# JuliaMeshless/WhatsThePoint.jl

Hardware: AMD Instinct MI355X
Metric: Mpoints/sec per repel iter (k=21 KNN+force) (higher is better)
Workload: dtype f32

## Files before the change

whatsthepoint.jl_amd/csrc/wtp_api.hip:

```cpp
#include <cmath>
#include <cstdlib>
#include <cstring>
#include <type_traits>

#include "wtp_internal.hpp"

namespace wtp {

static thread_local std::string g_create_err;

int fail(wtp_ctx* ctx, int code, const std::string& msg) {
    if (ctx)
        ctx->err = msg;
    else
        g_create_err = msg;
    return code;
}

int ensure(wtp_ctx* ctx, DevBuf& b, size_t bytes) {
    if (bytes == 0) bytes = 16;
    if (b.cap >= bytes) return WTP_OK;
    if (b.p) {
        hipFree(b.p);
        b.p = nullptr;
        b.cap = 0;
    }
    size_t want = bytes + bytes / 16 + 256;
    hipError_t e = hipMalloc(&b.p, want);
    if (e != hipSuccess) {
        (void)hipGetLastError();
        e = hipMalloc(&b.p, bytes);
        want = bytes;
    }
    if (e != hipSuccess) {
        (void)hipGetLastError();
        b.p = nullptr;
        return fail(ctx, WTP_ERR_OOM, "hipMalloc of " + std::to_string(bytes) + " bytes failed");
    }
    b.cap = want;
    return WTP_OK;
}

int launch_occupancy_of(wtp_ctx* ctx, const void* fn, int threads, size_t smem) {
    const auto key = std::make_pair(fn, smem);
    auto it = ctx->launch_cache.find(key);
    if (it != ctx->launch_cache.end()) return it->second;
    (void)hipFuncSetAttribute(fn, hipFuncAttributeMaxDynamicSharedMemorySize, (int)smem);
    int occ = 0;
    hipError_t e = hipOccupancyMaxActiveBlocksPerMultiprocessor(&occ, fn, threads, smem);
    if (e != hipSuccess || occ < 1) occ = 1;
    ctx->launch_cache[key] = occ;
    return occ;
}

int ensure_pinned(wtp_ctx* ctx, size_t bytes) {
    if (ctx->host_pinned_cap >= bytes) return WTP_OK;
    if (ctx->host_pinned) hipHostFree(ctx->host_pinned);
    ctx->host_pinned = nullptr;
    ctx->host_pinned_cap = 0;
    WTP_HIP(ctx, hipHostMalloc(&ctx->host_pinned, bytes, hipHostMallocDefault));
    ctx->host_pinned_cap = bytes;
    return WTP_OK;
}

static int take_event(wtp_ctx* ctx) {
    if (ctx->ev_used == (int)ctx->ev_pool.size()) {
        hipEvent_t e;
        if (hipEventCreate(&e) != hipSuccess) return -1;
        ctx->ev_pool.push_back(e);
    }
    return ctx->ev_used++;
}

int span_begin(wtp_ctx* ctx, int kind) {
    if (!ctx->timing) return -1;
    if (ctx->spans.size() > 8192) spans_collect(ctx);
    int a = ctx->ev_last_end;
    if (a < 0) {
        a = take_event(ctx);
        if (a < 0) return -1;
        hipEventRecord(ctx->ev_pool[a], ctx->stream);
    }
    const int b = take_event(ctx);
    if (b < 0) return -1;
    ctx->spans.push_back({a, b, kind});
    return (int)ctx->spans.size() - 1;
}

void span_end(wtp_ctx* ctx, int span) {
    if (span < 0) return;
    hipEventRecord(ctx->ev_pool[ctx->spans[span].b], ctx->stream);
    ctx->ev_last_end = ctx->spans[span].b;
}

void spans_collect(wtp_ctx* ctx) {
    ctx->ev_last_end = -1;
    if (ctx->spans.empty()) return;
    hipStreamSynchronize(ctx->stream);
    for (auto& s : ctx->spans) {
        float ms = 0.f;
        if (hipEventElapsedTime(&ms, ctx->ev_pool[s.a], ctx->ev_pool[s.b]) == hipSuccess) {
            if (s.kind == 0) ctx->t_hash += ms;
            else if (s.kind == 1) ctx->t_sweep += ms;
            else ctx->t_other += ms;
        }
    }
    ctx->spans.clear();
    ctx->ev_used = 0;
}

static int sync(wtp_ctx* ctx) {
    ctx->ev_last_end = -1;
    ctx->n_syncs += 1;
    WTP_HIP(ctx, hipStreamSynchronize(ctx->stream));
    return WTP_OK;
}

static size_t tsize(int dtype) { return dtype == WTP_F64 ? 8 : 4; }
static size_t pt_size(int dtype) { return by_dtype(dtype, [](auto t) { return sizeof(Pt<decltype(t)>); }); }

int need_session(wtp_ctx* ctx, const char* entry) {
    if (!ctx) return WTP_ERR_ARG;
    if (!ctx->relax.active) return fail(ctx, WTP_ERR_STATE, std::string(entry) + " before wtp_relax_init");
    return WTP_OK;
}

static double host_max(const void* v, int64_t n, int dtype) {
    double m = 0;
    if (dtype == WTP_F64) {
        const double* p = (const double*)v;
        for (int64_t i = 0; i < n; ++i) m = p[i] > m ? p[i] : m;
    } else {
        const float* p = (const float*)v;
        for (int64_t i = 0; i < n; ++i) m = p[i] > m ? p[i] : m;
    }
    return m;
}

static int check_cloud(wtp_ctx* ctx, const void* xyz, int64_t n, int dim, int dtype) {
    if (!ctx) return WTP_ERR_ARG;
    if (!xyz) return fail(ctx, WTP_ERR_ARG, "xyz is NULL");
    if (n < 1) return fail(ctx, WTP_ERR_ARG, "n must be >= 1");
    if (n > 2000000000LL) return fail(ctx, WTP_ERR_ARG, "n exceeds the int32 index space");
    if (dim != 2 && dim != 3) return fail(ctx, WTP_ERR_ARG, "dim must be 2 or 3");
    if (dtype != WTP_F32 && dtype != WTP_F64) return fail(ctx, WTP_ERR_ARG, "dtype must be WTP_F32 or WTP_F64");
    return WTP_OK;
}

static double hash_target_rho(const wtp_ctx* ctx, int dim, int k, double rho_direct) {
    if (rho_direct > 0) return rho_direct < 1.0 ? 1.0 : rho_direct;
    const double r = (dim == 3 ? 0.381 : 0.436) * (double)(k > 0 ? k : 21) * (ctx->rho / 8.0);
    return r < 1.0 ? 1.0 : r;
}

template <typename T>
static int find_robust_box(wtp_ctx* ctx, const Pt<T>* in, int64_t n, int dim, const Grid<T>& hg) {
    int rc;
    const size_t hist_bytes = sizeof(unsigned int) * 3 * 1024;
    if ((rc = ensure(ctx, ctx->box_dev, 64 + hist_bytes))) return rc;
    if ((rc = ensure_pinned(ctx, 64 + hist_bytes))) return rc;
    double box[6];
    for (int a = 0; a < 3; ++a) {
        box[a] = (double)hg.org[a];
        box[3 + a] = (double)hg.org[a] + (double)hg.n[a] * (double)hg.c;
    }
    const uint64_t tail = (uint64_t)(n / 2000) + 1;
    for (int round = 0; round < 4; ++round) {
        memcpy(ctx->host_pinned, box, sizeof(box));
        WTP_HIP(ctx, hipMemcpyAsync(ctx->box_dev.p, ctx->host_pinned, sizeof(box), hipMemcpyHostToDevice, ctx->stream));
        unsigned int* d_hist = (unsigned int*)((char*)ctx->box_dev.p + 64);
        if ((rc = launch_axis_hist<T>(ctx, in, n, dim, (const double*)ctx->box_dev.p, d_hist))) return rc;
        WTP_HIP(ctx, hipMemcpyAsync((char*)ctx->host_pinned + 64, d_hist, hist_bytes, hipMemcpyDeviceToHost, ctx->stream));
        if ((rc = sync(ctx))) return rc;
        const unsigned int* h = (const unsigned int*)((const char*)ctx->host_pinned + 64);
        bool shrunk = false;
        for (int a = 0; a < dim; ++a) {
            const double w = (box[3 + a] - box[a]) / 1024.0;
            if (!(w > 0)) continue;
            uint64_t run = 0;
            int b_lo = 0, b_hi = 1023;
            for (int b = 0; b < 1024; ++b) {
                run += h[a * 1024 + b];
                if (run >= tail) { b_lo = b; break; }
            }
            run = 0;
            for (int b = 1023; b >= 0; --b) {
                run += h[a * 1024 + b];
                if (run >= tail) { b_hi = b; break; }
            }
            if (b_hi < b_lo) b_hi = b_lo;
            const double nlo = box[a] + w * b_lo, nhi = box[a] + w * (b_hi + 1);
            if ((nhi - nlo) < 0.5 * (box[3 + a] - box[a])) shrunk = true;
            box[a] = nlo;
            box[3 + a] = nhi;
        }
        if (!shrunk) break;
    }
    memcpy(ctx->host_pinned, box, sizeof(box));
    WTP_HIP(ctx, hipMemcpyAsync(ctx->box_dev.p, ctx->host_pinned, sizeof(box), hipMemcpyHostToDevice, ctx->stream));
    return sync(ctx);
}

template <typename T>
static int build_hash_tuned(wtp_ctx* ctx, GridTune& t, HashBuild<T> b, Grid<T>* hg_out, double* rho_eff_out) {
    const double target = hash_target_rho(ctx, b.dim, b.k, b.rho_direct);
    double scale = 1.0;
    double prev_c = -1;
    int rc;
    if ((rc = ensure(ctx, ctx->occ, 64))) return rc;
    if ((rc = ensure_pinned(ctx, 16384))) return rc;
    t.clipped = false;
    b.keep_grid = false;
    for (int round = 0; round < 3; ++round) {
        b.cell_scale = scale;
        b.box = t.clipped ? (const double*)ctx->box_dev.p : nullptr;
        if ((rc = build_hash<T>(ctx, b))) return rc;
        if ((rc = launch_occupancy<T>(ctx, (const Grid<T>*)ctx->grid.p, (unsigned long long*)ctx->occ.p))) return rc;
        char* hp = (char*)ctx->host_pinned;
        WTP_HIP(ctx, hipMemcpyAsync(hp, ctx->occ.p, 24, hipMemcpyDeviceToHost, ctx->stream));
        WTP_HIP(ctx, hipMemcpyAsync(hp + 64, ctx->grid.p, sizeof(Grid<T>), hipMemcpyDeviceToHost, ctx->stream));
        if ((rc = sync(ctx))) return rc;
        const unsigned long long* o = (const unsigned long long*)hp;
        const double rho_eff = o[1] ? (double)o[0] / (double)o[1] : 1.0;
        Grid<T> hg;
        memcpy(&hg, hp + 64, sizeof(hg));
        *rho_eff_out = rho_eff;
        *hg_out = hg;
        const double excess = (rho_eff - 1.0) / target;
        const bool capped = hg.n[0] >= kMaxAxisCells || hg.n[1] >= kMaxAxisCells || hg.n[2] >= kMaxAxisCells ||
                            (double)hg.ncells > 6.0 * (double)b.n;
        if (excess > 4.0 && capped && !t.clipped) {
            if ((rc = find_robust_box<T>(ctx, b.in, b.n, b.dim, hg))) return rc;
            t.clipped = true;
            scale = 1.0;
            prev_c = -1;
            round = -1;
            continue;
        }
        if (!(excess > 1.6) || round == 2) break;
        if (prev_c > 0 && !((double)hg.c < prev_c * 0.999)) break;
        prev_c = (double)hg.c;
        double f = std::cbrt(1.15 / excess);
        if (f < 0.3) f = 0.3;
        scale *= f;
        if (scale < 0.02) scale = 0.02;
    }
    t.scale = scale;
    t.rho = b.rho_direct;
    return WTP_OK;
}

static double ksel_brick_cost(int cols, double rho_cell, int* bx_out = nullptr) {
    int bx = ksel_max_bx();
    double best = 1e300;
    for (int nbx = 1; nbx <= cols; ++nbx) {
        const int b = (cols + nbx - 1) / nbx;
        if (b > ksel_max_bx()) continue;
        const double q = 4.0 * rho_cell * b;
        const double p2 = 0.5 * std::erfc((256.0 - q) / std::sqrt(2.0 * (q > 1 ? q : 1)));
        const double cost = (1.0 + p2 + (q > 512.0 ? 100.0 : 0.0)) / q;
        if (cost < best) {
            best = cost;
            bx = b;
        }
        if (b < 8) break;
    }
// ... 168 lines not shown
    span_end(ctx, sp);
    sp = span_begin(ctx, 1);
    init_search(b, ctx, sorted32, sorted32, n, kc, 1);
    b.idx_out = (int32_t*)ctx->cand_idx.p;
    b.dist_out = (float*)ctx->cand_dist.p;
    if (ksel) {
        b.ksel_bx = t.bx;
        b.brick_hcap = t.hcap;
        b.cap_count = (float)ksel_cap_count(kc);
    }
    return launch_topology<float>(ctx, b);
}

static int knn_dev_f64(wtp_ctx* ctx, const double* d_xyz, int64_t n, int dim, int k, int include_self, int32_t* d_idx,
                       double* d_dist, bool* done) {
    *done = false;
    const int kq = include_self ? k : k + 1;
    int kc = kq + 2;
    if ((int64_t)kc > n) kc = (int)n;
    if (ctx->force_generic || kc > 31) return WTP_OK;
    int rc;
    if ((rc = ensure(ctx, ctx->pts[0], sizeof(double4) * (size_t)n))) return rc;
    if ((rc = ensure(ctx, ctx->pts[1], sizeof(double4) * (size_t)n))) return rc;
    if ((rc = ensure(ctx, ctx->fb_list, sizeof(int32_t) * (size_t)n))) return rc;
    if ((rc = ensure(ctx, ctx->fb_count, 64))) return rc;
    ctx->counters_clean = false;
    if ((rc = ensure(ctx, ctx->fb2_list, sizeof(int32_t) * (size_t)n))) return rc;
    if ((rc = ensure(ctx, ctx->fb2_count, 64))) return rc;
    double4* raw64 = (double4*)ctx->pts[0].p;
    int sp = span_begin(ctx, 0);
    if ((rc = load_points<double>(ctx, d_xyz, raw64, n, dim))) return rc;
    const bool slots = kc == 24;
    double4* slot64 = (double4*)ctx->pts[1].p;
    SearchArgs<float> a{};
    a.fb_list = (int32_t*)ctx->fb_list.p;
    a.fb_count = (int32_t*)ctx->fb_count.p;
    a.fb2_list = (int32_t*)ctx->fb2_list.p;
    a.fb2_count = (int32_t*)ctx->fb2_count.p;
    const double* org4 = nullptr;
    rc = f64_candidates(ctx, raw64, n, dim, kc, ctx->knn64_tune, a, sp, &org4, [&](float4* sorted32) {
        return slots ? launch_relabel_slots(ctx, raw64, sorted32, slot64, nullptr, n) : WTP_OK;
    });
    if (rc) return rc;
    ctx->knn_tune.valid = false;
    if (slots)
        rc = launch_refine_f64_slots(ctx, slot64, a.idx_out, a.dist_out, n, kc, k, include_self, org4, d_idx, d_dist,
                                     (int32_t*)ctx->fb_list.p, (int32_t*)ctx->fb_count.p);
    else
        rc = launch_refine_f64(ctx, raw64, a.idx_out, a.dist_out, n, kc, k, include_self, org4, d_idx, d_dist,
                               (int32_t*)ctx->fb_list.p, (int32_t*)ctx->fb_count.p);
    span_end(ctx, sp);
    if (rc) return rc;
    ctx->n_sweep_launches += 1;
    ctx->relax.have_tree = false;
    ctx->rad_valid = false;
    if ((rc = ensure_pinned(ctx, 64))) return rc;
    WTP_HIP(ctx, hipMemcpyAsync(ctx->host_pinned, ctx->fb_count.p, sizeof(int32_t), hipMemcpyDeviceToHost, ctx->stream));
    if ((rc = sync(ctx))) return rc;
    const int32_t n_fail = *(const int32_t*)ctx->host_pinned;
    if (n_fail > 0) {
        double4* sorted64 = (double4*)ctx->pts[1].p;
        HashBuild<double> hb(raw64, sorted64, n, dim, kq);
        hb.canonical = false;
        if ((rc = build_hash<double>(ctx, hb))) return rc;
        SearchArgs<double> b{};
        init_search(b, ctx, sorted64, raw64, n, k, include_self);
        b.idx_out = d_idx;
        b.dist_out = d_dist;
        b.fb_list = (int32_t*)ctx->fb_list.p;
        b.fb_count = (int32_t*)ctx->fb_count.p;
        b.fb2_list = (int32_t*)ctx->fb2_list.p;
        b.fb2_count = (int32_t*)ctx->fb2_count.p;
        if ((rc = launch_generic_topology<double>(ctx, b, false))) return rc;
    }
    *done = true;
    return WTP_OK;
}

static int check_idle(wtp_ctx* ctx) {
    if (ctx->relax.active)
        return fail(ctx, WTP_ERR_STATE,
                    "context holds a relax session (its buffers are live): call wtp_relax_end or use another context");
    return WTP_OK;
}

static int check_k(wtp_ctx* ctx, int64_t n, int k, int include_self) {
    if (k < 1) return fail(ctx, WTP_ERR_ARG, "k must be >= 1");
    if ((int64_t)k > n - (include_self ? 0 : 1))
        return fail(ctx, WTP_ERR_ARG, "k exceeds the number of available neighbours (k+1 > n)");
    if (k > kGenericKMax) return fail(ctx, WTP_ERR_ARG, "k > 128 is not supported");
    return WTP_OK;
}

}

using namespace wtp;

#define WTP_API extern "C"

WTP_API const char* wtp_version(void) { return "wtp-mi355x 0.1.0 (gfx950)"; }

WTP_API const char* wtp_last_error(const wtp_ctx* ctx) { return ctx ? ctx->err.c_str() : g_create_err.c_str(); }

WTP_API int wtp_create(const int* device_ordinals, int n_dev, wtp_ctx** out) {
    if (!out) return fail(nullptr, WTP_ERR_ARG, "out is NULL");
    *out = nullptr;
    if (n_dev != 1)
        return fail(nullptr, WTP_ERR_ARG, "one context drives one GPU: create one context per process/GPU");
    int count = 0;
    if (hipGetDeviceCount(&count) != hipSuccess || count < 1) {
        (void)hipGetLastError();
        return fail(nullptr, WTP_ERR_NO_DEVICE, "no HIP device visible (libwtp has no CPU path)");
    }
    int dev = device_ordinals ? device_ordinals[0] : 0;
    if (dev < 0 || dev >= count) return fail(nullptr, WTP_ERR_ARG, "device ordinal out of range");
    hipDeviceProp_t prop;
    if (hipGetDeviceProperties(&prop, dev) != hipSuccess)
        return fail(nullptr, WTP_ERR_HIP, "hipGetDeviceProperties failed");
    if (std::string(prop.gcnArchName).rfind("gfx950", 0) != 0)
        return fail(nullptr, WTP_ERR_NO_DEVICE,
                    std::string("device is ") + prop.gcnArchName + ", libwtp is built for gfx950 only");
    if (hipSetDevice(dev) != hipSuccess) return fail(nullptr, WTP_ERR_HIP, "hipSetDevice failed");
    wtp_ctx* ctx = new wtp_ctx();
    ctx->device = dev;
    ctx->sm_count = prop.multiProcessorCount > 0 ? prop.multiProcessorCount : 256;
    if (hipStreamCreateWithFlags(&ctx->own_stream, hipStreamNonBlocking) != hipSuccess) {
        delete ctx;
        return fail(nullptr, WTP_ERR_HIP, "hipStreamCreate failed");
    }
    ctx->stream = ctx->own_stream;
    if (const char* e = getenv("WTP_RHO")) ctx->rho = atof(e) > 0 ? atof(e) : ctx->rho;
    if (const char* e = getenv("WTP_FORCE_GENERIC")) ctx->force_generic = atoi(e);
    if (const char* e = getenv("WTP_FULL_SELECT")) ctx->full_select = atoi(e);
    if (const char* e = getenv("WTP_KSEL")) ctx->ksel = atoi(e);
    if (const char* e = getenv("WTP_BALL64")) ctx->ball64 = atoi(e);
    if (const char* e = getenv("WTP_F64_KSEL")) ctx->f64_ksel = atoi(e);
    if (const char* e = getenv("WTP_RADIUS_DENSE")) ctx->radius_dense = atoi(e);
    if (const char* e = getenv("WTP_BLOCK_OVERLAP")) ctx->block_overlap = atoi(e);
    ctx->debug = getenv("WTP_DEBUG") != nullptr;
    ctx->debug_kd = getenv("WTP_DEBUG_KD") != nullptr;
    if (const char* e = getenv("WTP_TIMING")) {
        ctx->timing = atoi(e) != 0;
        ctx->timing_forced = true;
    }
    *out = ctx;
    return WTP_OK;
}

WTP_API int wtp_destroy(wtp_ctx* ctx) {
    if (ctx) block_destroy(ctx);
    if (ctx) block_topo_destroy(ctx);
    if (!ctx) return WTP_OK;
    hipSetDevice(ctx->device);
    hipStreamSynchronize(ctx->stream);
    wtp_comm_finalize(ctx);
    if (ctx->host_pinned) hipHostFree(ctx->host_pinned);
    for (auto e : ctx->ev_pool) hipEventDestroy(e);
    if (ctx->ev_comm_a) hipEventDestroy(ctx->ev_comm_a);
    if (ctx->ev_comm_b) hipEventDestroy(ctx->ev_comm_b);
    if (ctx->comm_stream) hipStreamDestroy(ctx->comm_stream);
    hipStreamDestroy(ctx->own_stream);
    delete ctx;
    return WTP_OK;
}

static int knn_on_device(wtp_ctx* ctx, const void* d_xyz, int64_t n, int dim, int dtype, int k, int include_self,
                         int32_t* d_idx, void* d_dist) {
    bool done = false;
    int rc = dtype == WTP_F64 ? knn_dev_f64(ctx, (const double*)d_xyz, n, dim, k, include_self, d_idx, (double*)d_dist, &done)
                              : WTP_OK;
    if (rc || done) return rc;
    return by_dtype(dtype, [&](auto t) {
        using T = decltype(t);
        return knn_dev_t<T>(ctx, (const T*)d_xyz, n, dim, k, include_self, d_idx, (T*)d_dist);
    });
}

static int knn_rows_on_device(wtp_ctx* ctx, const void* xyz, int64_t n, int dim, int dtype, int k, int include_self,
                              bool want_dist) {
    const size_t ts = tsize(dtype);
    int rc;
    if ((rc = ensure(ctx, ctx->raw_in, ts * (size_t)n * dim))) return rc;
    if ((rc = ensure(ctx, ctx->idx_out, sizeof(int32_t) * (size_t)n * k))) return rc;
    if (want_dist && (rc = ensure(ctx, ctx->dist_out, ts * (size_t)n * k))) return rc;
    WTP_HIP(ctx, hipMemcpyAsync(ctx->raw_in.p, xyz, ts * (size_t)n * dim, hipMemcpyHostToDevice, ctx->stream));
    return knn_on_device(ctx, ctx->raw_in.p, n, dim, dtype, k, include_self, (int32_t*)ctx->idx_out.p,
                         want_dist ? ctx->dist_out.p : nullptr);
}

WTP_API int wtp_knn_dev(wtp_ctx* ctx, const void* d_xyz, int64_t n, int dim, int dtype, int k, int include_self,
                int32_t* d_idx_out, void* d_dist_out) {
    int rc = check_cloud(ctx, d_xyz, n, dim, dtype);
    if (rc) return rc;
    if ((rc = check_k(ctx, n, k, include_self))) return rc;
    if ((rc = check_idle(ctx))) return rc;
    if (!d_idx_out) return fail(ctx, WTP_ERR_ARG, "idx_out is NULL");
    WTP_HIP(ctx, hipSetDevice(ctx->device));
    if ((rc = knn_on_device(ctx, d_xyz, n, dim, dtype, k, include_self, d_idx_out, d_dist_out))) return rc;
    return sync(ctx);
}

WTP_API int wtp_knn(wtp_ctx* ctx, const void* xyz, int64_t n, int dim, int dtype, int k, int include_self,
            int32_t* idx_out, void* dist_out) {
    int rc = check_cloud(ctx, xyz, n, dim, dtype);
    if (rc) return rc;
    if ((rc = check_k(ctx, n, k, include_self))) return rc;
    if ((rc = check_idle(ctx))) return rc;
    if (!idx_out) return fail(ctx, WTP_ERR_ARG, "idx_out is NULL");
    WTP_HIP(ctx, hipSetDevice(ctx->device));
    const size_t ts = tsize(dtype);
    if ((rc = knn_rows_on_device(ctx, xyz, n, dim, dtype, k, include_self, dist_out != nullptr))) return rc;
    WTP_HIP(ctx, hipMemcpyAsync(idx_out, ctx->idx_out.p, sizeof(int32_t) * (size_t)n * k, hipMemcpyDeviceToHost,
                                ctx->stream));
    if (dist_out)
        WTP_HIP(ctx, hipMemcpyAsync(dist_out, ctx->dist_out.p, ts * (size_t)n * k, hipMemcpyDeviceToHost, ctx->stream));
    return sync(ctx);
}

WTP_API int wtp_pca_normals(wtp_ctx* ctx, const void* xyz, int64_t n, int dim, int dtype, int k, void* normals_out) {
    int rc = check_cloud(ctx, xyz, n, dim, dtype);
    if (rc) return rc;
    if (k < 2) return fail(ctx, WTP_ERR_ARG, "k must be >= 2 (a covariance needs two points)");
    if ((rc = check_k(ctx, n, k, 1))) return rc;
    if ((rc = check_idle(ctx))) return rc;
    if (!normals_out) return fail(ctx, WTP_ERR_ARG, "normals_out is NULL");
    WTP_HIP(ctx, hipSetDevice(ctx->device));
    const size_t ts = tsize(dtype);
    if ((rc = knn_rows_on_device(ctx, xyz, n, dim, dtype, k, 1, false))) return rc;
    if ((rc = ensure(ctx, ctx->scratch, ts * (size_t)n * dim))) return rc;
    int sp = span_begin(ctx, 2);
    rc = by_dtype(dtype, [&](auto t) {
        using T = decltype(t);
        return launch_pca_normals<T>(ctx, (const T*)ctx->raw_in.p, n, dim, (const int32_t*)ctx->idx_out.p, k, (T*)ctx->scratch.p);
    });
    span_end(ctx, sp);
    if (rc) return rc;
    WTP_HIP(ctx, hipMemcpyAsync(normals_out, ctx->scratch.p, ts * (size_t)n * dim, hipMemcpyDeviceToHost, ctx->stream));
    return sync(ctx);
}

WTP_API int wtp_gradient_limit(wtp_ctx* ctx, const void* centers, int64_t n, int dim, int dtype, int k, const void* h0,
                               double g, double tol, int max_sweeps, void* h_out, int* sweeps_out) {
    int rc = check_cloud(ctx, centers, n, dim, dtype);
    if (rc) return rc;
    if ((rc = check_k(ctx, n, k, 1))) return rc;
    if ((rc = check_idle(ctx))) return rc;
    if (!h0 || !h_out) return fail(ctx, WTP_ERR_ARG, "NULL array");
    if (max_sweeps < 0) return fail(ctx, WTP_ERR_ARG, "max_sweeps must be >= 0");
    WTP_HIP(ctx, hipSetDevice(ctx->device));
    const size_t ts = tsize(dtype);
    if ((rc = knn_rows_on_device(ctx, centers, n, dim, dtype, k, 1, true))) return rc;
    const size_t o1 = (ts * (size_t)n + 255) / 256 * 256;
    if ((rc = ensure(ctx, ctx->scratch, 2 * o1 + 64))) return rc;
    char* b = (char*)ctx->scratch.p;
    unsigned long long* st = (unsigned long long*)(b + 2 * o1);
    WTP_HIP(ctx, hipMemcpyAsync(b, h0, ts * (size_t)n, hipMemcpyHostToDevice, ctx->stream));
    WTP_HIP(ctx, hipMemsetAsync(st, 0, 64, ctx->stream));
    if ((rc = ensure_pinned(ctx, 64))) return rc;
    unsigned long long* hst = (unsigned long long*)ctx->host_pinned;
    hst[0] = hst[1] = 0;
    int sp = span_begin(ctx, 2);
    for (int first = 0; first < max_sweeps && !hst[0];) {
        const int batch = max_sweeps - first < 16 ? max_sweeps - first : 16;
        rc = by_dtype(dtype, [&](auto t) {
            using T = decltype(t);
            return launch_minplus_batch<T>(ctx, (const int32_t*)ctx->idx_out.p, (const T*)ctx->dist_out.p, n, k, g, tol, (T*)b,
                                           (T*)(b + o1), first, batch, st);
        });
        if (rc) return rc;
        WTP_HIP(ctx, hipMemcpyAsync(hst, st, 16, hipMemcpyDeviceToHost, ctx->stream));
        if ((rc = sync(ctx))) return rc;
        first += batch;
    }
    span_end(ctx, sp);
    const int applied = (int)hst[1];
    if (sweeps_out) *sweeps_out = applied;
    WTP_HIP(ctx, hipMemcpyAsync(h_out, b + ((applied & 1) ? o1 : 0), ts * (size_t)n, hipMemcpyDeviceToHost, ctx->stream));
    return sync(ctx);
}

template <typename T> static int radius_count_t(wtp_ctx* ctx, int64_t n, int dim, double r, int32_t* d_counts) {
    int rc;
    if ((rc = ensure(ctx, ctx->pts[0], sizeof(Pt<T>) * (size_t)n))) return rc;
    if ((rc = ensure(ctx, ctx->pts[1], sizeof(Pt<T>) * (size_t)n))) return rc;
    Pt<T>* raw = (Pt<T>*)ctx->pts[0].p;
    Pt<T>* sorted = (Pt<T>*)ctx->pts[1].p;
    int sp = span_begin(ctx, 0);
    if ((rc = load_points<T>(ctx, (const T*)ctx->raw_in.p, raw, n, dim))) return rc;
    HashBuild<T> b(raw, sorted, n, dim, 0);
    b.radius = r > 0 ? r : 1e-300;
    b.canonical = false;
    if ((rc = build_hash<T>(ctx, b))) return rc;
    span_end(ctx, sp);
    SearchArgs<T> a{};
    init_search(a, ctx, sorted, sorted, n, 0, 0);
    if ((rc = ensure(ctx, ctx->fb_list, sizeof(int32_t) * (size_t)n))) return rc;
    if ((rc = ensure(ctx, ctx->fb_count, 64))) return rc;
    ctx->counters_clean = false;
    a.fb_list = (int32_t*)ctx->fb_list.p;
    a.fb_count = (int32_t*)ctx->fb_count.p;
    if ((rc = ensure(ctx, ctx->rad_done, (size_t)n + 64))) return rc;
    WTP_HIP(ctx, hipMemsetAsync(ctx->rad_done.p, 0, (size_t)n, ctx->stream));
    a.rad_done = (uint8_t*)ctx->rad_done.p;
    if (sizeof(T) == 4 && !ctx->force_generic) {
        if ((rc = ensure(ctx, ctx->rad_tmp, sizeof(int32_t) * 32 * (size_t)n))) return rc;
        a.rad_tmp = (int32_t*)ctx->rad_tmp.p;
    }
    const int64_t arena_cap = (int64_t)kRadArenaPerPoint * n;
    if ((rc = ensure(ctx, ctx->rad_arena, sizeof(int32_t) * (size_t)arena_cap))) return rc;
    if ((rc = ensure(ctx, ctx->rad_arena_off, sizeof(int64_t) * (size_t)(n + 2)))) return rc;
    a.rad_arena = (int32_t*)ctx->rad_arena.p;
    a.rad_arena_off = (int64_t*)ctx->rad_arena_off.p;
// ... 340 lines not shown
    if ((rc = ensure(ctx, ctx->occ, 513 * sizeof(unsigned int)))) return rc;
    if ((rc = ensure_pinned(ctx, 16384))) return rc;
    const double cells = (double)hg.n[0] * hg.n[1] * hg.n[2];
    double rho_est = cells > 0 ? (double)r.n / cells : 1.0;
    if (rho_eff - 1.0 > rho_est) rho_est = rho_eff - 1.0;
    if (rho_est < 0.25) rho_est = 0.25;
    const int bx_max = hg.n[0] < cs2_max_bx() ? (hg.n[0] < 1 ? 1 : hg.n[0]) : cs2_max_bx();
    auto clampbx = [&](double v) {
        int b = (int)(v + 0.5);
        return b < 2 ? (bx_max < 2 ? bx_max : 2) : (b > bx_max ? bx_max : b);
    };
    r.cs2_rho = rho_est;
    int bx = clampbx(220.0 / (4.0 * rho_est));
    int q97 = 0, h999 = 0;
    for (int it = 0; it < 4; ++it) {
        if ((rc = launch_cs2_census(ctx, bx, (unsigned int*)ctx->occ.p))) return rc;
        WTP_HIP(ctx, hipMemcpyAsync(ctx->host_pinned, ctx->occ.p, 513 * sizeof(unsigned int), hipMemcpyDeviceToHost,
                                    ctx->stream));
        if ((rc = sync(ctx))) return rc;
        const unsigned int* h = (const unsigned int*)ctx->host_pinned;
        const double nb = (double)h[512];
        auto quant = [&](int base, double frac, int width) {
            double run = 0;
            for (int b = 0; b < 256; ++b) {
                run += h[base + b];
                if (run >= frac * nb) return (b + 1) * width;
            }
            return 256 * width;
        };
        q97 = nb > 0 ? quant(0, 0.97, 2) : 0;
        h999 = nb > 0 ? quant(256, 0.999, 8) : 0;
        if (nb <= 0) break;
        double f = 1.0;
        if (q97 > 248 || q97 < 216) f = 236.0 / (double)q97;
        if (h999 * f > 1060.0) f = 1060.0 / (double)h999;
        const int nbx = clampbx(bx * f);
        if (nbx == bx || it == 3) break;
        bx = nbx;
    }
    if (hg.n[0] > bx && q97 > 0) {
        int best = 0;
        for (int parts = hg.n[0] / bx > 1 ? hg.n[0] / bx : 1; parts <= (hg.n[0] + bx - 1) / bx; ++parts) {
            const int bxc = (hg.n[0] + parts - 1) / parts;
            if (bxc > bx_max) continue;
            const double grow = (double)bxc / (double)bx;
            if (q97 * grow <= 254.0 && h999 * grow <= 1100.0) {
                best = bxc;
                h999 = (int)(h999 * grow) + 1;
                break;
            }
        }
        if (!best) {
            const int parts = (hg.n[0] + bx - 1) / bx;
            best = (hg.n[0] + parts - 1) / parts;
        }
        bx = best;
    }
    int hc = (int)(h999 * 1.05) + 48;
    hc = (hc + 63) / 64 * 64;
    r.brick_hcap = hc < 256 ? 256 : (hc > 1920 ? 1920 : hc);
    r.cs2_bx = bx;
    if (ctx->debug)
        fprintf(stderr, "[wtp] cs2 geometry: BX=%d hcap=%d (q97=%d h999=%d rho_est=%.3f grid %dx%dx%d c=%g)\n", bx,
                r.brick_hcap, q97, h999, rho_est, hg.n[0], hg.n[1], hg.n[2], (double)hg.c);
    return WTP_OK;
}

static void swap_float_copy_grid(wtp_ctx* ctx) {
    std::swap(ctx->grid, ctx->grid_b);
    std::swap(ctx->cell_start, ctx->cell_start_b);
    std::swap(ctx->box_dev, ctx->box_b);
}

static int relax_f64_ksel_sweep(wtp_ctx* ctx, SearchArgs<double>& a, int* sp) {
    RelaxState& r = ctx->relax;
    const int64_t n = r.n;
    const int kc = 24;
    int rc;
    if ((rc = ensure(ctx, ctx->f64k_s64, sizeof(double4) * (size_t)n))) return rc;
    if ((rc = ensure(ctx, ctx->f64k_slot, sizeof(int32_t) * (size_t)n))) return rc;
    if ((rc = ensure(ctx, ctx->f64k_lists, sizeof(int32_t) * 2 * (size_t)n))) return rc;
    if ((rc = ensure(ctx, ctx->f64k_cnt, 64))) return rc;
    const double4* snap = (const double4*)a.snap;
    SearchArgs<float> b{};
    b.fb_list = (int32_t*)ctx->f64k_lists.p;
    b.fb_count = (int32_t*)ctx->f64k_cnt.p;
    b.fb2_list = (int32_t*)ctx->f64k_lists.p + n;
    b.fb2_count = (int32_t*)ctx->f64k_cnt.p + 4;
    b.stop = ctx->stop_dev;
    b.diag = a.diag;
    *sp = span_begin(ctx, 0);
    WTP_HIP(ctx, hipMemsetAsync(ctx->f64k_cnt.p, 0, 64, ctx->stream));
    b.counters_cleared = 1;
    swap_float_copy_grid(ctx);
    const double* org4 = nullptr;
    rc = f64_candidates(ctx, snap, n, 3, kc, r.f64k_tune, b, *sp, &org4, [&](float4* sorted32) {
        return launch_relabel_slots(ctx, snap, sorted32, (double4*)ctx->f64k_s64.p, (int32_t*)ctx->f64k_slot.p, n);
    });
    swap_float_copy_grid(ctx);
    if (rc) return rc;
    return launch_refine_sweep_f64(ctx, a, (const double4*)ctx->f64k_s64.p, (const int32_t*)ctx->f64k_slot.p,
                                   (const int32_t*)ctx->cand_idx.p, (const float*)ctx->cand_dist.p, org4);
}

static bool grid_reusable(const RelaxState& r, int64_t n_fixed_next, bool head_swapped) {
    const bool head_ok = !head_swapped || (r.shard_grid_reuse && r.grid_fixed > 0 &&
                                           std::llabs((long long)(n_fixed_next - r.grid_fixed)) * 10 <= (long long)r.grid_fixed + 640);
    return r.grid_age < kGridReuseMax && !r.moved_by_hand && head_ok && !r.tune.clipped;
}

static bool head_remeasures(const RelaxState& r, int64_t n_fixed_new) {
    const int64_t n_new = r.n - r.n_fixed + n_fixed_new;
    return r.cs2_bx > 0 && std::llabs((long long)(n_fixed_new - r.tuned_fixed)) * 20 > (long long)n_new;
}

template <typename T> static SweepRoute sweep_route(const wtp_ctx* ctx, const RelaxState& r) {
    if (ctx->force_generic) return SweepRoute::Exact;
    const bool clipped = r.force.kind == WTP_FORCE_CLIPPED_SPACING;
    if (clipped && r.k >= 2 && r.k < 32 && !ctx->full_select && !r.cs_disabled) {
        if (sizeof(T) == 8) return ctx->ball64 ? SweepRoute::Cs64 : SweepRoute::Cs64Wave;
        return r.dim == 3 ? SweepRoute::Cs2 : SweepRoute::Cs;
    }
    if (sizeof(T) == 8) {
        const bool f64k = r.dim == 3 && ctx->ksel && ctx->f64_ksel && !clipped && r.k >= 2 && r.k <= 22 && r.n >= 4096;
        return f64k ? SweepRoute::F64Ksel : SweepRoute::Exact;
    }
    if (r.k >= 32) return SweepRoute::Exact;
    const bool ksel = r.dim == 3 && ctx->ksel && r.k >= 2 && r.k <= ksel_kmax() && r.n >= 4096;
    return ksel ? SweepRoute::Ksel : SweepRoute::Select;
}

static bool route_cs(SweepRoute s) {
    return s == SweepRoute::Cs || s == SweepRoute::Cs2 || s == SweepRoute::Cs64 || s == SweepRoute::Cs64Wave;
}
static bool route_ball(SweepRoute s) { return s == SweepRoute::Cs || s == SweepRoute::Cs2 || s == SweepRoute::Cs64; }

struct RouteGrid { double rho, min_cell; };
static RouteGrid route_grid(const wtp_ctx* ctx, const RelaxState& r) {
    if (r.route == SweepRoute::Ksel) return {r.tune.valid && r.tune.bx > 0 ? r.tune.rho : ksel_rho_for(r.k), 0.0};
    if (!route_cs(r.route)) return {0.0, 0.0};
    const bool cs2 = r.route == SweepRoute::Cs2;
    const double cell_f = (cs2 && r.spacing_kind == WTP_SPACING_CONSTANT) ? 1.01 : 1.1;
    return {cs2 ? kRhoCs2 : 3.5 * (ctx->rho / 9.0),
            cell_f * r.force.u0 * (r.spacing_typ < r.spacing_max ? r.spacing_typ : r.spacing_max)};
}

static SweepRoute step_route(const RelaxState& r, bool fresh) {
    if (!fresh) return route_ball(r.route) ? SweepRoute::Ball : SweepRoute::Exact;
    const bool measured = r.route == SweepRoute::Ksel ? r.tune.bx > 0 : !route_cs(r.route) || r.brick_hcap > 0;
    if (measured) return r.route;
    return r.route == SweepRoute::Cs64 || r.route == SweepRoute::Cs64Wave ? SweepRoute::Exact : SweepRoute::Select;
}

static int ball_pass(wtp_ctx* ctx, SearchArgs<float>& a) { return launch_cs_ball(ctx, a, a.ball_list, a.ball_count); }
static int ball_pass(wtp_ctx* ctx, SearchArgs<double>& a) { return launch_cs_ball64(ctx, a, a.ball_list, a.ball_count); }

template <typename T> static int launch_sweep(wtp_ctx* ctx, SearchArgs<T>& a, SweepRoute route, bool ball) {
    constexpr bool f32 = sizeof(T) == 4;
    ctx->n_sweep_launches += 1;
    int rc = WTP_OK, sp = -1;
    switch (route) {
    case SweepRoute::Exact:
    case SweepRoute::Ball:
        sp = span_begin(ctx, 1);
        if (route == SweepRoute::Ball) {
            rc = launch_cs_all_slots(ctx, a.fb_list, a.n, a.fb_count);
            if (!rc) rc = ball_pass(ctx, a);
        }
        if (!rc) rc = launch_generic_sweep<T>(ctx, a, route == SweepRoute::Exact);
        span_end(ctx, sp);
        return rc;
    case SweepRoute::F64Ksel:
        if constexpr (!f32) rc = relax_f64_ksel_sweep(ctx, a, &sp);
        break;
    case SweepRoute::Ksel:
        sp = span_begin(ctx, 1);
        if constexpr (f32) rc = launch_ksel_sweep(ctx, a);
        a.fb_r0 = 3;
        break;
    case SweepRoute::Select:
    case SweepRoute::Cs:
    case SweepRoute::Cs2:
        sp = span_begin(ctx, 1);
        if constexpr (f32) {
            if (route == SweepRoute::Cs2 && ball) {
                const int dead_cap = (int)(ctx->cell_start.cap / sizeof(int32_t) / 4 + 4096);
                rc = ensure(ctx, ctx->brick_dead, (size_t)dead_cap);
                if (!rc) rc = launch_cs2_dead(ctx, a, (uint8_t*)ctx->brick_dead.p, dead_cap);
                a.brick_dead = (const uint8_t*)ctx->brick_dead.p;
                a.brick_dead_cap = dead_cap;
            }
            if (!rc) rc = route == SweepRoute::Cs2 ? launch_cs2(ctx, a) : launch_brick_sweep(ctx, a, route == SweepRoute::Cs);
        }
        break;
    case SweepRoute::Cs64:
    case SweepRoute::Cs64Wave:
        sp = span_begin(ctx, 1);
        if constexpr (!f32) {
            rc = launch_brick_cs<double>(ctx, a);
            if (!rc && ball) rc = ball_pass(ctx, a);
        }
        break;
    }
    span_end(ctx, sp);
    if (rc) return rc;
    sp = span_begin(ctx, 2);
    if constexpr (f32) {
        if (route == SweepRoute::Cs2) rc = launch_cs2_followup(ctx, a);
        if (!rc && ball) rc = ball_pass(ctx, a);
    }
    if (!rc) rc = launch_generic_sweep<T>(ctx, a, false);
    span_end(ctx, sp);
    return rc;
}

template <typename T>
static HashBuild<T> relax_request(const wtp_ctx* ctx, const RelaxState& r, const Pt<T>* in, Pt<T>* out, int64_t n, int k,
                                  const HashView& view, bool keep_grid) {
    const RouteGrid g = route_grid(ctx, r);
    HashBuild<T> b(in, out, n, r.dim, k);
    b.rho_direct = g.rho;
    b.min_cell = g.min_cell;
    b.cell_scale = r.tune.scale;
    b.view = view;
    b.keep_grid = keep_grid;
    b.canonical = !r.tune.valid || r.route != SweepRoute::F64Ksel;
    b.box = r.tune.clipped ? (const double*)ctx->box_dev.p : nullptr;
    return b;
}

template <typename T> static int relax_rebuild(wtp_ctx* ctx) {
    RelaxState& r = ctx->relax;
    int rc;
    const int t = pick_free(r, r.bufP, -1);
    if ((rc = ensure(ctx, ctx->pts[t], sizeof(Pt<T>) * (size_t)(r.n + r.shard_extra)))) return rc;
    int sp = span_begin(ctx, 0);
    r.route = sweep_route<T>(ctx, r);
    if (r.spacing_typ <= 0) {
        r.spacing_typ = r.spacing_const;
        if (r.spacing_kind != WTP_SPACING_CONSTANT) {
            if ((rc = ensure(ctx, ctx->occ, 64))) return rc;
            if ((rc = ensure_pinned(ctx, 1024))) return rc;
            if ((rc = launch_sum<T>(ctx, (const T*)ctx->spacing_pp.p, r.n, (double*)ctx->occ.p))) return rc;
            WTP_HIP(ctx, hipMemcpyAsync(ctx->host_pinned, ctx->occ.p, sizeof(double), hipMemcpyDeviceToHost, ctx->stream));
            if ((rc = sync(ctx))) return rc;
            r.spacing_typ = ((const double*)ctx->host_pinned)[0] / (double)r.n;
            if (!(r.spacing_typ > 0)) r.spacing_typ = r.spacing_max;
        }
    }
    const Pt<T>* in = pts_of<T>(ctx, r.bufP);
    Pt<T>* out = pts_of<T>(ctx, t);
    if (!r.tune.valid) {
        double rho_eff = 0;
        Grid<T> hg;
        HashBuild<T> b = relax_request<T>(ctx, r, in, out, r.n, r.k, r.pending, false);
        if ((rc = build_hash_tuned<T>(ctx, r.tune, b, &hg, &rho_eff))) return rc;
        if (route_cs(r.route) && rho_eff > (r.route == SweepRoute::Cs2 ? 5.0 : 4.0 * b.rho_direct) && 2 * r.n_fixed < r.n) {
            r.cs_disabled = true;
            r.route = sweep_route<T>(ctx, r);
            b = relax_request<T>(ctx, r, in, out, r.n, r.k, r.pending, false);
            if ((rc = build_hash_tuned<T>(ctx, r.tune, b, &hg, &rho_eff))) return rc;
        }
        r.cs2_bx = 0;
        if (r.route == SweepRoute::Cs2) {
            Grid<float> hgf;
            memcpy(&hgf, &hg, sizeof(hgf));
            if ((rc = cs2_tune(ctx, r, hgf, rho_eff))) return rc;
        } else if (route_cs(r.route)) {
            int hc = (int)(HCELLS * rho_eff * 1.15) + 128;
            hc = (hc + 63) / 64 * 64;
            r.brick_hcap = hc < 640 ? 640 : (hc > 2560 ? 2560 : hc);
        }
        if (r.route == SweepRoute::Ksel && (rc = ksel_tune<T>(ctx, r.tune, b, hg, rho_eff))) return rc;
        r.tune.valid = true;
        r.tuned_fixed = r.n_fixed;
        r.grid_fixed = r.n_fixed;
        r.grid_age = 0;
    } else {
        const bool reuse = grid_reusable(r, r.n_fixed, r.pending.active);
        r.grid_age = reuse ? r.grid_age + 1 : 0;
        if (!reuse) r.grid_fixed = r.n_fixed;
        rc = build_hash<T>(ctx, relax_request<T>(ctx, r, in, out, r.n, r.k, r.pending, reuse));
    }
    span_end(ctx, sp);
    if (rc) return rc;
    r.pending.active = false;
    r.bufS = t;
    r.bufP = t;
    r.have_tree = true;
    r.sweeps_since_rebuild = 0;
    r.moved_by_hand = false;
    return WTP_OK;
}

template <typename T> static int relax_step_t(wtp_ctx* ctx, int rebuild, wtp_step_stats* d_slot) {
    RelaxState& r = ctx->relax;
    int rc;
    if (!r.have_tree || r.pending.active) rebuild = 1;
    if (rebuild && (rc = relax_rebuild<T>(ctx))) return rc;
    if (spacing_on_device(r.spacing_kind)) {
        int sps = span_begin(ctx, 2);
        rc = launch_spacing_session<T>(ctx, (const Pt<T>*)ctx->pts[r.bufP].p, r.n, r.n_fixed, ctx->kd_nodes.p, ctx->kd_m,
                                       r.spacing_kind, r.sp_p0, r.sp_p1, r.sp_p2, (T*)ctx->spacing_pp.p,
                                       (int32_t*)ctx->sp_hint.p - r.aux_off, r.have_tree ? (const int32_t*)ctx->cell_start.p : nullptr,
                                       ctx->grid.p, (Pt<T>*)ctx->sp_cert.p - r.aux_off);
        span_end(ctx, sps);
        if (rc) return rc;
    }
    const bool fresh = (r.bufS == r.bufP);
    const int o = pick_free(r, r.bufS, r.bufP);
    if ((rc = ensure(ctx, ctx->pts[o], sizeof(Pt<T>) * (size_t)(r.n + r.shard_extra)))) return rc;
    SearchArgs<T> a{};
    init_search(a, ctx, (const Pt<T>*)ctx->pts[r.bufS].p, (const Pt<T>*)ctx->pts[r.bufP].p, r.n, r.k, 1);
    a.out = (Pt<T>*)ctx->pts[o].p;
    a.forces = (T*)ctx->forces.p;
    a.nn_dist = (T*)ctx->nn_dist.p;
    a.nn_id = (int32_t*)ctx->nn_id.p;
    a.spacing_pp = r.spacing_kind != WTP_SPACING_CONSTANT ? (const T*)ctx->spacing_pp.p : nullptr;
    a.spacing_const = (T)r.spacing_const;
    a.alpha_lo = (T)r.alpha_lo;
    a.alpha_max = (T)r.alpha_max;
    a.beta = (T)r.force.beta;
    a.u0 = (T)r.force.u0;
    a.gamma = (T)r.force.gamma;
    a.force_kind = r.force.kind;
    a.n_fixed = (int32_t)r.n_fixed;
    a.partials = (Partial*)ctx->partials.p;
    a.n_partials = total_partials();
    a.fb_list = (int32_t*)ctx->fb_list.p;
    a.fb_count = (int32_t*)ctx->fb_count.p;
    a.fb2_list = (int32_t*)ctx->fb2_list.p;
    a.fb2_count = (int32_t*)ctx->fb_count.p + 4;
    a.stop = ctx->stop_dev;
    a.nn_count = (int32_t*)ctx->fb_count.p + 2;
    const SweepRoute route = step_route(r, fresh);
    const bool ball = route_ball(r.route) && (!fresh || r.spacing_kind != WTP_SPACING_CONSTANT);
    if (ball || route == SweepRoute::Cs2) {
        if ((rc = ensure(ctx, ctx->nn_list, sizeof(int32_t) * (size_t)r.n))) return rc;
        if (sizeof(T) == 4) a.nn_list = (int32_t*)ctx->nn_list.p;
        if (ball) {
            a.ball_list = (int32_t*)ctx->nn_list.p;
            a.ball_count = (int32_t*)ctx->fb_count.p + 6;
        }
    }
    if ((rc = ensure(ctx, ctx->diag, 128))) return rc;
    a.diag = (unsigned long long*)ctx->diag.p;
    a.brick_hcap = route_cs(r.route) ? r.brick_hcap : (r.route == SweepRoute::Ksel ? r.tune.hcap : 0);
    a.cs2_bx = route_cs(r.route) ? r.cs2_bx : 0;
    a.cs2_chunked = (r.spacing_kind != WTP_SPACING_CONSTANT || r.cs2_rho > 1.6) ? 1 : 0;
    a.ksel_bx = r.route == SweepRoute::Ksel ? r.tune.bx : 0;
    if (r.route == SweepRoute::Ksel) a.cap_count = (float)ksel_cap_count(r.k);
    if (route == SweepRoute::Select || route == SweepRoute::Cs || route == SweepRoute::Cs2) {
        a.gamma_cap = (T)kGammaCapSweep;
        a.cap_count = (float)(4.18879 * kGammaCapSweep * kGammaCapSweep * kGammaCapSweep * ctx->rho * (a.k + 1) / 22.0);
    }
    if (route == SweepRoute::Cs64 || route == SweepRoute::Cs64Wave) a.gamma_cap = (T)kGammaCap;
    a.tnn_frac = (T)kTnnFrac;
    a.cover_axis = r.cover_axis;
    a.cover_lo = (T)r.cover_lo;
    a.cover_hi = (T)r.cover_hi;
    for (int ax = 0; ax < 3; ++ax) {
        a.cover_lo3[ax] = (T)r.cover_lo3[ax];
        a.cover_hi3[ax] = (T)r.cover_hi3[ax];
    }
    a.uncovered = (int32_t*)ctx->fb_count.p + 8;
    if (!ctx->counters_clean) WTP_HIP(ctx, hipMemsetAsync(ctx->fb_count.p, 0, 64, ctx->stream));
    ctx->counters_clean = false;
    a.used_brick = a.used_wave = a.used_generic = 0;
    if ((rc = launch_sweep<T>(ctx, a, route, ball && route_ball(route)))) return rc;
    int sp = span_begin(ctx, 2);
    if (r.wall_active) {
        char* wf = (char*)ctx->wall_flags.p;
        rc = launch_mesh_constrain<T>(ctx, a.query, a.out, r.n, r.n_fixed, r.wall_offset, (const uint8_t*)wf,
                                      (uint8_t*)wf + r.wall_nm, (int32_t*)ctx->wall_tri.p, (int32_t*)ctx->wall_hint.p,
                                      (int32_t*)ctx->fb_count.p + 12);
        if (rc) return rc;
    }
    rc = launch_reduce_partials(ctx, a.partials, a.n_partials, a.used_brick, a.used_wave, a.used_generic, a.fb_count,
                                a.uncovered, r.wall_active ? (const int32_t*)ctx->fb_count.p + 12 : nullptr, d_slot);
    span_end(ctx, sp);
    if (rc) return rc;
    r.bufOld = r.bufP;
    r.bufP = o;
    r.can_revert = true;
    r.have_point_data = true;
    r.sweeps_since_rebuild += 1;
    return WTP_OK;
}

static int relax_step_any(wtp_ctx* ctx, int rebuild, wtp_step_stats* d_slot) {
    return by_dtype(ctx->relax.dtype, [&](auto t) { return relax_step_t<decltype(t)>(ctx, rebuild, d_slot); });
}
int wtp::relax_step_enqueue(wtp_ctx* ctx, int rebuild, wtp_step_stats* d_slot) { return relax_step_any(ctx, rebuild, d_slot); }

int wtp::relax_prerank(wtp_ctx* ctx, int64_t n_fixed_new) {
    RelaxState& r = ctx->relax;
    ctx->prerank.valid = false;
    if (!r.active || !r.tune.valid || !r.have_tree || r.pending.active) return WTP_OK;
    if (!grid_reusable(r, n_fixed_new, true) || head_remeasures(r, n_fixed_new)) return WTP_OK;
    const int64_t n_new = r.n - r.n_fixed + n_fixed_new;
    if (ctx->pts[r.bufP].cap < pt_size(r.dtype) * (size_t)(r.n + n_fixed_new)) return WTP_OK;
    const int k = (int64_t)r.k_req < n_new ? r.k_req : (int)n_new;
    HashView view;
    view.active = true;
    view.n_in = r.n + n_fixed_new;
    view.n_old = r.n;
    view.fixed_old = (int32_t)r.n_fixed;
    view.id_shift = (int32_t)(n_fixed_new - r.n_fixed);
    return by_dtype(r.dtype, [&](auto t) {
        using T = decltype(t);
        return prerank_old_snapshot<T>(ctx, relax_request<T>(ctx, r, pts_of<T>(ctx, r.bufP), nullptr, n_new, k, view, true));
    });
}

int wtp::relax_swap_begin(wtp_ctx* ctx, int64_t n_move_new, void** d_buf_out) {
    RelaxState& r = ctx->relax;
    if (!r.active || r.pending.active) return fail(ctx, WTP_ERR_STATE, "relax_swap_begin: no session, or a pending fixed head");
    if (n_move_new < 1 || n_move_new > 2000000000LL) return fail(ctx, WTP_ERR_ARG, "relax_swap_begin: bad point count");
    const int t = pick_free(r, r.bufP, -1);
    int rc;
    if ((rc = ensure(ctx, ctx->pts[t], pt_size(r.dtype) * (size_t)(n_move_new + r.shard_extra)))) return rc;
    r.swap_target = t;
    *d_buf_out = ctx->pts[t].p;
    return WTP_OK;
}

int wtp::relax_swap_commit(wtp_ctx* ctx, int64_t n_move_new) {
    RelaxState& r = ctx->relax;
    if (!r.active || r.swap_target < 0) return fail(ctx, WTP_ERR_STATE, "relax_swap_commit without relax_swap_begin");
    const size_t ts = tsize(r.dtype);
    int rc;
    if (spacing_on_device(r.spacing_kind)) {
        if ((rc = ensure(ctx, ctx->spacing_pp, ts * (size_t)n_move_new))) return rc;
        if ((rc = ensure(ctx, ctx->sp_hint, sizeof(int32_t) * (size_t)n_move_new))) return rc;
        if ((rc = ensure(ctx, ctx->sp_cert, 4 * ts * (size_t)n_move_new))) return rc;
        WTP_HIP(ctx, hipMemsetAsync(ctx->sp_hint.p, 0xFF, sizeof(int32_t) * (size_t)n_move_new, ctx->stream));
        WTP_HIP(ctx, hipMemsetAsync(ctx->sp_cert.p, 0xFF, 4 * ts * (size_t)n_move_new, ctx->stream));
        r.aux_off = 0;
    }
    r.bufP = r.swap_target;
    r.swap_target = -1;
    r.n = n_move_new;
    r.n_fixed = 0;
    r.k = (int64_t)r.k_req < n_move_new ? r.k_req : (int)n_move_new;
    r.bufS = -1;
    r.bufOld = -1;
    r.have_tree = false;
    r.can_revert = false;
    r.have_point_data = false;
    r.moved_by_hand = true;
    return WTP_OK;
}

static int read_step(wtp_ctx* ctx, wtp_step_stats* stats, int n_axes = 0, int32_t* const* d_tot = nullptr,
                     int64_t* counts = nullptr) {
    if (!stats) return sync(ctx);
    const size_t off = (sizeof(wtp_step_stats) + 63) / 64 * 64;
    int rc;
    if ((rc = ensure_pinned(ctx, n_axes ? off + 64 * n_axes : sizeof(wtp_step_stats)))) return rc;
    char* h = (char*)ctx->host_pinned;
    WTP_HIP(ctx, hipMemcpyAsync(h, ctx->stats.p, sizeof(wtp_step_stats), hipMemcpyDeviceToHost, ctx->stream));
    for (int ax = 0; ax < n_axes; ++ax)
        if (d_tot[ax])
            WTP_HIP(ctx, hipMemcpyAsync(h + off + 64 * ax, d_tot[ax], 4 * sizeof(int32_t), hipMemcpyDeviceToHost, ctx->stream));
    if ((rc = sync(ctx))) return rc;
    memcpy(stats, h, sizeof(wtp_step_stats));
    for (int ax = 0; ax < n_axes; ++ax)
        for (int j = 0; j < 4; ++j) counts[4 * ax + j] = d_tot[ax] ? ((const int32_t*)(h + off + 64 * ax))[j] : 0;
    return WTP_OK;
}

WTP_API int wtp_relax_step(wtp_ctx* ctx, int rebuild, wtp_step_stats* stats) {
    int rc = need_session(ctx, __func__);
    if (rc) return rc;
    WTP_HIP(ctx, hipSetDevice(ctx->device));
    if ((rc = ensure(ctx, ctx->stats, sizeof(wtp_step_stats)))) return rc;
    if ((rc = relax_step_any(ctx, rebuild, (wtp_step_stats*)ctx->stats.p))) return rc;
    return read_step(ctx, stats);
}

WTP_API int wtp_relax_run(wtp_ctx* ctx, int n_iters, int rebuild_every, double* conv_out, wtp_step_stats* last) {
    int rc = need_session(ctx, __func__);
    if (rc) return rc;
    if (rebuild_every < 1) return fail(ctx, WTP_ERR_ARG, "rebuild_every must be >= 1");
    if (n_iters < 0) return fail(ctx, WTP_ERR_ARG, "n_iters must be >= 0");
    if (n_iters == 0) return WTP_OK;
    WTP_HIP(ctx, hipSetDevice(ctx->device));
    if ((rc = ensure(ctx, ctx->stats, sizeof(wtp_step_stats) * (size_t)n_iters))) return rc;
    wtp_step_stats* d = (wtp_step_stats*)ctx->stats.p;
    for (int i = 0; i < n_iters; ++i)
        if ((rc = relax_step_any(ctx, (i % rebuild_every) == 0, d + i))) return rc;
    if (conv_out || last) {
        if ((rc = ensure_pinned(ctx, sizeof(wtp_step_stats) * (size_t)n_iters))) return rc;
        WTP_HIP(ctx, hipMemcpyAsync(ctx->host_pinned, d, sizeof(wtp_step_stats) * (size_t)n_iters,
                                    hipMemcpyDeviceToHost, ctx->stream));
        if ((rc = sync(ctx))) return rc;
        const wtp_step_stats* h = (const wtp_step_stats*)ctx->host_pinned;
        if (conv_out)
            for (int i = 0; i < n_iters; ++i) conv_out[i] = h[i].max_force;
        if (last) *last = h[n_iters - 1];
        return WTP_OK;
    }
    return sync(ctx);
}

struct StopState {
    int32_t stopped, reason, n_done, last_impr;
    double best_cv;
};
__global__ void stop_rules_kernel(const wtp_step_stats* __restrict__ st, StopState* __restrict__ s, int iter1, double tol,
                                  int stall_after, double cv_target) {
    if (s->stopped) return;
    s->n_done = iter1;
    const double conv = st->max_force;
    if ((stall_after > 0 || cv_target > 0) && st->n_move > 0) {
        const double n = (double)st->n_move, mu = st->sum_u / n;
        const double var = st->sum_u2 / n - mu * mu;
        const double cv = sqrt(var > 0.0 ? var : 0.0) / mu;
        if (cv_target > 0 && cv <= cv_target) {
            s->stopped = 1;
            s->reason = 2;
            return;
        }
        if (stall_after > 0) {
            if (cv < s->best_cv * (1 - 1.0e-3)) {
                s->best_cv = cv;
                s->last_impr = iter1;
            } else if (iter1 - s->last_impr >= stall_after) {
                s->stopped = 1;
                s->reason = 3;
                return;
            }
        }
    }
    if (conv < tol) {
        s->stopped = 1;
        s->reason = 1;
    }
}

WTP_API int wtp_relax_run_until(wtp_ctx* ctx, int max_iters, int rebuild_every, double tol, int stall_after,
                                double cv_target, double* conv_out, int* n_done_out, int* reason_out,
                                wtp_step_stats* last) {
    int rc = need_session(ctx, __func__);
    if (rc) return rc;
    RelaxState& r = ctx->relax;
    if (rebuild_every < 1) return fail(ctx, WTP_ERR_ARG, "rebuild_every must be >= 1");
    if (max_iters < 0) return fail(ctx, WTP_ERR_ARG, "max_iters must be >= 0");
    if (r.wall_active) return fail(ctx, WTP_ERR_STATE, "wtp_relax_run_until: the octree wall rule steps through wtp_relax_step");
    if (n_done_out) *n_done_out = 0;
    if (reason_out) *reason_out = 0;
    if (max_iters == 0) return WTP_OK;
    WTP_HIP(ctx, hipSetDevice(ctx->device));
    if ((rc = ensure(ctx, ctx->stats, sizeof(wtp_step_stats) * (size_t)max_iters))) return rc;
    if ((rc = ensure(ctx, ctx->stop_state, 64))) return rc;
    if ((rc = ensure_pinned(ctx, 64 + sizeof(wtp_step_stats) * (size_t)max_iters))) return rc;
    StopState h0{};
    h0.best_cv = __builtin_huge_val();
    memcpy(ctx->host_pinned, &h0, sizeof(h0));
    WTP_HIP(ctx, hipMemcpyAsync(ctx->stop_state.p, ctx->host_pinned, sizeof(h0), hipMemcpyHostToDevice, ctx->stream));
    if ((rc = sync(ctx))) return rc;
    wtp_step_stats* d = (wtp_step_stats*)ctx->stats.p;
    StopState* ds = (StopState*)ctx->stop_state.p;
    const int kBatch = 16;
    std::vector<RelaxState> hist;
    hist.reserve((size_t)kBatch);
    int done = 0, reason = 0;
    ctx->stop_dev = &ds->stopped;
    for (int i0 = 0; i0 < max_iters && !reason; i0 += kBatch) {
        const int i1 = i0 + kBatch < max_iters ? i0 + kBatch : max_iters;
        hist.clear();
        for (int i = i0; i < i1; ++i) {
            if ((rc = relax_step_any(ctx, (i % rebuild_every) == 0, d + i))) {
                ctx->stop_dev = nullptr;
                return rc;
            }
            hist.push_back(r);
            hipLaunchKernelGGL(stop_rules_kernel, dim3(1), dim3(1), 0, ctx->stream, d + i, ds, i + 1, tol, stall_after, cv_target);
        }
        WTP_HIP(ctx, hipMemcpyAsync(ctx->host_pinned, ds, sizeof(StopState), hipMemcpyDeviceToHost, ctx->stream));
        if ((rc = sync(ctx))) {
            ctx->stop_dev = nullptr;
            return rc;
        }
        StopState hs;
        memcpy(&hs, ctx->host_pinned, sizeof(hs));
        done = hs.n_done;
        if (hs.stopped) {
            reason = hs.reason;
            r = hist[(size_t)(done - 1 - i0)];
        }
    }
    ctx->stop_dev = nullptr;
    if (reason == 2) {
        if ((rc = wtp_relax_revert(ctx))) return rc;
    }
    if (conv_out || last) {
        WTP_HIP(ctx, hipMemcpyAsync(ctx->host_pinned, d, sizeof(wtp_step_stats) * (size_t)done, hipMemcpyDeviceToHost,
                                    ctx->stream));
        if ((rc = sync(ctx))) return rc;
        const wtp_step_stats* hst = (const wtp_step_stats*)ctx->host_pinned;
        if (conv_out)
            for (int i = 0; i < done; ++i) conv_out[i] = hst[i].max_force;
        if (last && done > 0) *last = hst[done - 1];
    }
    if (n_done_out) *n_done_out = done;
    if (reason_out) *reason_out = reason;
    return WTP_OK;
}

static int unpermute_p(wtp_ctx* ctx, void* d_out) {
    const RelaxState& r = ctx->relax;
    return by_dtype(r.dtype, [&](auto t) {
        using T = decltype(t);
        return launch_unpermute<T>(ctx, pts_of<T>(ctx, r.bufP), r.n, r.n_fixed, r.dim, (T*)d_out);
    });
}

WTP_API int wtp_relax_get(wtp_ctx* ctx, void* xyz_out) {
    int rc = need_session(ctx, __func__);
    if (rc) return rc;
    RelaxState& r = ctx->relax;
    if (!xyz_out) return fail(ctx, WTP_ERR_ARG, "xyz_out is NULL");
    WTP_HIP(ctx, hipSetDevice(ctx->device));
    if ((rc = flush_pending(ctx))) return rc;
    const int64_t n_move = r.n - r.n_fixed;
    if (n_move == 0) return WTP_OK;
    const size_t bytes = tsize(r.dtype) * (size_t)n_move * r.dim;
    if ((rc = ensure(ctx, ctx->scratch, bytes))) return rc;
    if ((rc = unpermute_p(ctx, ctx->scratch.p))) return rc;
    WTP_HIP(ctx, hipMemcpyAsync(xyz_out, ctx->scratch.p, bytes, hipMemcpyDeviceToHost, ctx->stream));
    return sync(ctx);
}

WTP_API int wtp_relax_get_dev(wtp_ctx* ctx, void* d_xyz_out) {
    int rc = need_session(ctx, __func__);
    if (rc) return rc;
    RelaxState& r = ctx->relax;
    if (!d_xyz_out) return fail(ctx, WTP_ERR_ARG, "xyz_out is NULL");
    WTP_HIP(ctx, hipSetDevice(ctx->device));
    if ((rc = flush_pending(ctx))) return rc;
    if (r.n - r.n_fixed == 0) return WTP_OK;
    if ((rc = unpermute_p(ctx, d_xyz_out))) return rc;
    return sync(ctx);
}

WTP_API int wtp_relax_get_point_data(wtp_ctx* ctx, void* forces_out, void* nn_dist_out, int32_t* nn_id_out) {
    if (!ctx) return WTP_ERR_ARG;
    RelaxState& r = ctx->relax;
    if (!r.active || !r.have_point_data || r.bufOld < 0)
        return fail(ctx, WTP_ERR_STATE, "wtp_relax_get_point_data needs a completed wtp_relax_step");
    WTP_HIP(ctx, hipSetDevice(ctx->device));
    const int64_t n_move = r.n - r.n_fixed;
    if (n_move == 0) return WTP_OK;
    const size_t ts = tsize(r.dtype);
    int rc;
    if ((rc = ensure(ctx, ctx->scratch, (2 * ts + 4) * (size_t)n_move))) return rc;
    char* base = (char*)ctx->scratch.p;
    void* fo = base;
    void* no = base + ts * n_move;
    int32_t* io = (int32_t*)(base + 2 * ts * n_move);
    rc = by_dtype(r.dtype, [&](auto t) {
        using T = decltype(t);
        return launch_unpermute_point_data<T>(ctx, pts_of<T>(ctx, r.bufOld), r.n, r.n_fixed, (const T*)ctx->forces.p,
                                              (const T*)ctx->nn_dist.p, (const int32_t*)ctx->nn_id.p, (T*)fo, (T*)no, io);
    });
    if (rc) return rc;
    if (forces_out) WTP_HIP(ctx, hipMemcpyAsync(forces_out, fo, ts * n_move, hipMemcpyDeviceToHost, ctx->stream));
    if (nn_dist_out) WTP_HIP(ctx, hipMemcpyAsync(nn_dist_out, no, ts * n_move, hipMemcpyDeviceToHost, ctx->stream));
    if (nn_id_out) WTP_HIP(ctx, hipMemcpyAsync(nn_id_out, io, 4 * (size_t)n_move, hipMemcpyDeviceToHost, ctx->stream));
    return sync(ctx);
}

static int own_p(wtp_ctx* ctx, const char* entry) {
    RelaxState& r = ctx->relax;
    if (r.bufP != r.bufS) return WTP_OK;
    const int t = pick_free(r, r.bufS, r.can_revert ? r.bufOld : -1);
    if (t == r.bufS) return fail(ctx, WTP_ERR_STATE, std::string("no free buffer for ") + entry);
    const size_t bytes = pt_size(r.dtype) * (size_t)r.n;
    int rc;
    if ((rc = ensure(ctx, ctx->pts[t], bytes))) return rc;
    WTP_HIP(ctx, hipMemcpyAsync(ctx->pts[t].p, ctx->pts[r.bufP].p, bytes, hipMemcpyDeviceToDevice, ctx->stream));
    if (r.bufOld == t) r.can_revert = false;
    r.bufP = t;
    return WTP_OK;
}

WTP_API int wtp_relax_set(wtp_ctx* ctx, int64_t i, const void* xyz) {
    int rc = need_session(ctx, __func__);
    if (rc) return rc;
    RelaxState& r = ctx->relax;
    if (!xyz) return fail(ctx, WTP_ERR_ARG, "xyz is NULL");
    if (i < 0 || i >= r.n - r.n_fixed) return fail(ctx, WTP_ERR_ARG, "movable point index out of range");
    WTP_HIP(ctx, hipSetDevice(ctx->device));
    if ((rc = flush_pending(ctx))) return rc;
    const size_t ts = tsize(r.dtype);
    if ((rc = ensure(ctx, ctx->scratch, 64))) return rc;
    if ((rc = own_p(ctx, __func__))) return rc;
    WTP_HIP(ctx, hipMemcpyAsync(ctx->scratch.p, xyz, ts * r.dim, hipMemcpyHostToDevice, ctx->stream));
    const int32_t id = (int32_t)(i + r.n_fixed);
    r.moved_by_hand = true;
    rc = by_dtype(r.dtype, [&](auto t) {
        using T = decltype(t);
        return launch_set_point<T>(ctx, pts_of<T>(ctx, r.bufP), r.n, id, r.dim, (const T*)ctx->scratch.p);
    });
    if (rc) return rc;
    return sync(ctx);
}

WTP_API int wtp_relax_set_batch(wtp_ctx* ctx, const int64_t* idx, const void* xyz, int64_t m) {
    int rc = need_session(ctx, __func__);
    if (rc) return rc;
    RelaxState& r = ctx->relax;
    if (m < 0) return fail(ctx, WTP_ERR_ARG, "m must be >= 0");
    if (m == 0) return WTP_OK;
    if (!idx || !xyz) return fail(ctx, WTP_ERR_ARG, "NULL array");
    std::vector<int32_t> ids((size_t)m);
    for (int64_t j = 0; j < m; ++j) {
        if (idx[j] < 0 || idx[j] >= r.n - r.n_fixed) return fail(ctx, WTP_ERR_ARG, "movable point index out of range");
        if (j > 0 && idx[j] <= idx[j - 1]) return fail(ctx, WTP_ERR_ARG, "indices must be strictly increasing");
        ids[(size_t)j] = (int32_t)(idx[j] + r.n_fixed);
    }
    WTP_HIP(ctx, hipSetDevice(ctx->device));
    if ((rc = flush_pending(ctx))) return rc;
    const size_t ts = tsize(r.dtype);
    const size_t o_v = (sizeof(int32_t) * (size_t)m + 255) / 256 * 256;
// ... 98 lines not shown
    if ((rc = check_spacing_law(ctx, spacing))) return rc;
    WTP_HIP(ctx, hipSetDevice(ctx->device));
    const size_t ts = tsize(dtype);
    if ((rc = ensure_kd(ctx, spacing, dim, dtype))) return rc;
    if ((rc = ensure(ctx, ctx->ins_in, ts * (size_t)n * dim))) return rc;
    if ((rc = ensure(ctx, ctx->ins_out, ts * (size_t)n))) return rc;
    WTP_HIP(ctx, hipMemcpyAsync(ctx->ins_in.p, xyz, ts * (size_t)n * dim, hipMemcpyHostToDevice, ctx->stream));
    rc = by_dtype(dtype, [&](auto t) {
        using T = decltype(t);
        return launch_spacing_eval<T>(ctx, (const T*)ctx->ins_in.p, n, dim, ctx->kd_nodes.p, ctx->kd_m, spacing->kind,
                                      spacing->p0, spacing->p1, spacing->p2, (T*)ctx->ins_out.p);
    });
    if (rc) return rc;
    WTP_HIP(ctx, hipMemcpyAsync(out, ctx->ins_out.p, ts * (size_t)n, hipMemcpyDeviceToHost, ctx->stream));
    return sync(ctx);
}

WTP_API int wtp_relax_end(wtp_ctx* ctx) {
    if (!ctx) return WTP_ERR_ARG;
    ctx->relax = RelaxState{};
    return WTP_OK;
}

static size_t align256(size_t b) { return (b + 255) / 256 * 256; }

WTP_API int wtp_isinside_greens(wtp_ctx* ctx, const void* test_xyz, int64_t n, const void* elem_xyz,
                                const void* elem_normal, const void* elem_area, int64_t m, int dtype,
                                uint8_t* inside_out, void* g_out) {
    if (!ctx) return WTP_ERR_ARG;
    if (dtype != WTP_F32 && dtype != WTP_F64) return fail(ctx, WTP_ERR_ARG, "dtype must be WTP_F32 or WTP_F64");
    if (n < 0 || m < 1) return fail(ctx, WTP_ERR_ARG, "need n >= 0 test points and m >= 1 boundary elements");
    if (n > 2000000000LL || m > 2000000000LL) return fail(ctx, WTP_ERR_ARG, "n or m exceeds the int32 index space");
    if (n == 0) return WTP_OK;
    if (!test_xyz || !elem_xyz || !elem_normal || !elem_area || !inside_out)
        return fail(ctx, WTP_ERR_ARG, "NULL array");
    WTP_HIP(ctx, hipSetDevice(ctx->device));
    const size_t ts = tsize(dtype);
    const int chunks = isinside_chunks(ctx, n, m, isinside_greens_ppb());
    const size_t o_p = align256(ts * n * 3), o_n = o_p + align256(ts * m * 3), o_a = o_n + align256(ts * m * 3);
    int rc;
    if ((rc = ensure(ctx, ctx->ins_in, o_a + ts * m))) return rc;
    if ((rc = ensure(ctx, ctx->ins_elems, isinside_elem_bytes(dtype) * (size_t)m))) return rc;
    if ((rc = ensure(ctx, ctx->ins_partial, ts * (size_t)n * chunks))) return rc;
    if ((rc = ensure(ctx, ctx->ins_out, align256(ts * n) + (size_t)n))) return rc;
    char* in = (char*)ctx->ins_in.p;
    char* out = (char*)ctx->ins_out.p;
    WTP_HIP(ctx, hipMemcpyAsync(in, test_xyz, ts * n * 3, hipMemcpyHostToDevice, ctx->stream));
    WTP_HIP(ctx, hipMemcpyAsync(in + o_p, elem_xyz, ts * m * 3, hipMemcpyHostToDevice, ctx->stream));
    WTP_HIP(ctx, hipMemcpyAsync(in + o_n, elem_normal, ts * m * 3, hipMemcpyHostToDevice, ctx->stream));
    WTP_HIP(ctx, hipMemcpyAsync(in + o_a, elem_area, ts * m, hipMemcpyHostToDevice, ctx->stream));
    uint8_t* d_inside = (uint8_t*)(out + align256(ts * n));
    int sp = span_begin(ctx, 2);
    rc = by_dtype(dtype, [&](auto t) {
        using T = decltype(t);
        return launch_isinside_greens<T>(ctx, (const T*)in, n, (const T*)(in + o_p), (const T*)(in + o_n), (const T*)(in + o_a),
                                         m, ctx->ins_elems.p, chunks, (T*)ctx->ins_partial.p, (T*)out, d_inside);
    });
    span_end(ctx, sp);
    if (rc) return rc;
    WTP_HIP(ctx, hipMemcpyAsync(inside_out, d_inside, (size_t)n, hipMemcpyDeviceToHost, ctx->stream));
    if (g_out) WTP_HIP(ctx, hipMemcpyAsync(g_out, out, ts * n, hipMemcpyDeviceToHost, ctx->stream));
    return sync(ctx);
}

WTP_API int wtp_isinside_winding(wtp_ctx* ctx, const void* test_xy, int64_t n, const void* poly_xy, int64_t m,
                                 int dtype, uint8_t* inside_out, void* sum_out) {
    if (!ctx) return WTP_ERR_ARG;
    if (dtype != WTP_F32 && dtype != WTP_F64) return fail(ctx, WTP_ERR_ARG, "dtype must be WTP_F32 or WTP_F64");
    if (m < 3) return fail(ctx, WTP_ERR_ARG, "need at least 3 points to define a polygon");
    if (n < 0 || n > 2000000000LL || m > 2000000000LL) return fail(ctx, WTP_ERR_ARG, "bad n or m");
    if (n == 0) return WTP_OK;
    if (!test_xy || !poly_xy || !inside_out) return fail(ctx, WTP_ERR_ARG, "NULL array");
    WTP_HIP(ctx, hipSetDevice(ctx->device));
    const size_t ts = tsize(dtype);
    const int chunks = isinside_chunks(ctx, n, m, isinside_winding_ppb());
    const size_t o_p = align256(ts * n * 2);
    int rc;
    if ((rc = ensure(ctx, ctx->ins_in, o_p + ts * m * 2))) return rc;
    if ((rc = ensure(ctx, ctx->ins_partial, ts * (size_t)n * chunks))) return rc;
    if ((rc = ensure(ctx, ctx->ins_elems, sizeof(int32_t) * (size_t)n))) return rc;
    if ((rc = ensure(ctx, ctx->ins_out, align256(ts * n) + (size_t)n))) return rc;
    char* in = (char*)ctx->ins_in.p;
    char* out = (char*)ctx->ins_out.p;
    WTP_HIP(ctx, hipMemcpyAsync(in, test_xy, ts * n * 2, hipMemcpyHostToDevice, ctx->stream));
    WTP_HIP(ctx, hipMemcpyAsync(in + o_p, poly_xy, ts * m * 2, hipMemcpyHostToDevice, ctx->stream));
    uint8_t* d_inside = (uint8_t*)(out + align256(ts * n));
    rc = by_dtype(dtype, [&](auto t) {
        using T = decltype(t);
        return launch_isinside_winding<T>(ctx, (const T*)in, n, (const T*)(in + o_p), m, chunks, (T*)ctx->ins_partial.p,
                                          (int32_t*)ctx->ins_elems.p, (T*)out, d_inside);
    });
    if (rc) return rc;
    WTP_HIP(ctx, hipMemcpyAsync(inside_out, d_inside, (size_t)n, hipMemcpyDeviceToHost, ctx->stream));
    if (sum_out) WTP_HIP(ctx, hipMemcpyAsync(sum_out, out, ts * n, hipMemcpyDeviceToHost, ctx->stream));
    return sync(ctx);
}

WTP_API int wtp_set_stream(wtp_ctx* ctx, void* hip_stream, int external) {
    if (!ctx) return WTP_ERR_ARG;
    WTP_HIP(ctx, hipSetDevice(ctx->device));
    spans_collect(ctx);
    WTP_HIP(ctx, hipStreamSynchronize(ctx->stream));
    ctx->stream = external ? (hipStream_t)hip_stream : ctx->own_stream;
    return WTP_OK;
}

static int enqueue_layers(wtp_ctx* ctx, int axis, double lo_in, double hi_in, double lo_out, double hi_out, void* d_lo4,
                          void* d_hi4, int64_t cap, int32_t** d_tot_out, int slot = 0) {
    RelaxState& r = ctx->relax;
    if (axis < 0 || axis >= r.dim) return fail(ctx, WTP_ERR_ARG, "axis must be in [0, dim)");
    if (cap < 0 || (cap > 0 && (!d_lo4 || !d_hi4))) return fail(ctx, WTP_ERR_ARG, "layer buffers are NULL");
    if (int rcf = flush_pending(ctx)) return rcf;
    int rc;
    const int nblk = layer_blocks(r.n);
    const size_t region = (64 + sizeof(int2) * (size_t)nblk + 63) / 64 * 64;
    if ((rc = ensure(ctx, ctx->scratch, 3 * region))) return rc;
    int32_t* d_tot = (int32_t*)((char*)ctx->scratch.p + (size_t)slot * region);
    int2* d_blk = (int2*)((char*)d_tot + 64);
    const bool slot_ordered = r.have_tree && r.have_point_data && axis == r.dim - 1 && r.bufP != r.bufS &&
                              !r.moved_by_hand;
    const double reach = 1.001 * r.spacing_max * (double)(r.sweeps_since_rebuild > 0 ? r.sweeps_since_rebuild : 1);
    rc = by_dtype(r.dtype, [&](auto t) {
        using T = decltype(t);
        return launch_layers<T>(ctx, pts_of<T>(ctx, r.bufP), r.n, r.n_fixed, axis, lo_in, hi_in, lo_out, hi_out, (Pt<T>*)d_lo4,
                                (Pt<T>*)d_hi4, cap, d_blk, d_tot, slot_ordered, reach);
    });
    *d_tot_out = d_tot;
    return rc;
}

WTP_API int wtp_relax_layers_dev(wtp_ctx* ctx, int axis, double lo_in, double hi_in, double lo_out, double hi_out,
                                 void* d_lo4, void* d_hi4, int64_t cap, int64_t counts[4]) {
    int rc = need_session(ctx, __func__);
    if (rc) return rc;
    if (!counts) return fail(ctx, WTP_ERR_ARG, "counts is NULL");
    WTP_HIP(ctx, hipSetDevice(ctx->device));
    int32_t* d_tot = nullptr;
    if ((rc = enqueue_layers(ctx, axis, lo_in, hi_in, lo_out, hi_out, d_lo4, d_hi4, cap, &d_tot))) return rc;
    if ((rc = ensure_pinned(ctx, 64))) return rc;
    WTP_HIP(ctx, hipMemcpyAsync(ctx->host_pinned, d_tot, 4 * sizeof(int32_t), hipMemcpyDeviceToHost, ctx->stream));
    if ((rc = sync(ctx))) return rc;
    for (int j = 0; j < 4; ++j) counts[j] = ((const int32_t*)ctx->host_pinned)[j];
    return WTP_OK;
}

WTP_API int wtp_relax_step_layers(wtp_ctx* ctx, int rebuild, wtp_step_stats* stats, int axis, double lo_in, double hi_in,
                                  double lo_out, double hi_out, void* d_lo4, void* d_hi4, int64_t cap,
                                  int64_t counts[4]) {
    int rc = need_session(ctx, __func__);
    if (rc) return rc;
    if (!stats || !counts) return fail(ctx, WTP_ERR_ARG, "stats/counts is NULL");
    WTP_HIP(ctx, hipSetDevice(ctx->device));
    if ((rc = ensure(ctx, ctx->stats, sizeof(wtp_step_stats)))) return rc;
    if ((rc = relax_step_any(ctx, rebuild, (wtp_step_stats*)ctx->stats.p))) return rc;
    int32_t* d_tot = nullptr;
    if ((rc = enqueue_layers(ctx, axis, lo_in, hi_in, lo_out, hi_out, d_lo4, d_hi4, cap, &d_tot))) return rc;
    return read_step(ctx, stats, 1, &d_tot, counts);
}

static int flush_pending(wtp_ctx* ctx) {
    RelaxState& r = ctx->relax;
    if (!r.pending.active) return WTP_OK;
    int rc;
    const int t = pick_free(r, r.bufP, -1);
    if ((rc = ensure(ctx, ctx->pts[t], pt_size(r.dtype) * (size_t)(r.n + r.shard_extra)))) return rc;
    if ((rc = ensure(ctx, ctx->scratch, 64))) return rc;
    const HashView v = r.pending;
    rc = by_dtype(r.dtype, [&](auto tt) {
        using T = decltype(tt);
        const Pt<T>* P = pts_of<T>(ctx, r.bufP);
        return launch_refix<T>(ctx, P, v.n_old, v.fixed_old, r.n_fixed, P + v.n_old, pts_of<T>(ctx, t), (int32_t*)ctx->scratch.p);
    });
    if (rc) return rc;
    r.bufP = t;
    r.pending.active = false;
    return WTP_OK;
}

int wtp::relax_set_fixed_dev_impl(wtp_ctx* ctx, const void* d_fixed4, int64_t n_fixed_new, bool keep_alive) {
    int rc = need_session(ctx, "wtp_relax_set_fixed_dev");
    if (rc) return rc;
    RelaxState& r = ctx->relax;
    if (r.spacing_kind == WTP_SPACING_PER_POINT)
        return fail(ctx, WTP_ERR_STATE, "wtp_relax_set_fixed_dev: not with a caller-evaluated (PER_POINT) spacing array");
    if (n_fixed_new < 0 || (n_fixed_new > 0 && !d_fixed4)) return fail(ctx, WTP_ERR_ARG, "bad fixed-point array");
    WTP_HIP(ctx, hipSetDevice(ctx->device));
    if ((rc = flush_pending(ctx))) return rc;
    const int64_t n_move = r.n - r.n_fixed, n_new = n_move + n_fixed_new;
    if (n_new < 1) return fail(ctx, WTP_ERR_ARG, "the snapshot would be empty");
    if (n_new > 2000000000LL) return fail(ctx, WTP_ERR_ARG, "n exceeds the int32 index space");
    const size_t ts = tsize(r.dtype);
    const size_t ptsz = pt_size(r.dtype);
    const int64_t extra = n_fixed_new + n_fixed_new / 4 + 4096;
    if (extra > r.shard_extra) r.shard_extra = extra;
    if ((rc = ensure(ctx, ctx->forces, ts * (size_t)n_new))) return rc;
    if ((rc = ensure(ctx, ctx->nn_dist, ts * (size_t)n_new))) return rc;
    if ((rc = ensure(ctx, ctx->nn_id, sizeof(int32_t) * (size_t)n_new))) return rc;
    if ((rc = ensure(ctx, ctx->fb_list, sizeof(int32_t) * (size_t)n_new))) return rc;
    if ((rc = ensure(ctx, ctx->fb2_list, sizeof(int32_t) * (size_t)n_new))) return rc;
    if ((rc = ensure(ctx, ctx->scratch, 64))) return rc;
    if (spacing_on_device(r.spacing_kind)) {
        if ((rc = ensure(ctx, ctx->spacing_pp, ts * (size_t)n_new))) return rc;
        r.aux_off += n_fixed_new - r.n_fixed;
    }
    const bool fits = ctx->pts[r.bufP].cap >= ptsz * (size_t)(r.n + n_fixed_new);
    if (fits) {
        if (n_fixed_new > 0) {
            rc = by_dtype(r.dtype, [&](auto t) {
                using T = decltype(t);
                return launch_append_fixed<T>(ctx, (const Pt<T>*)d_fixed4, n_fixed_new, pts_of<T>(ctx, r.bufP) + r.n);
            });
            if (rc) return rc;
        }
        r.pending.active = true;
        r.pending.n_old = r.n;
        r.pending.n_in = r.n + n_fixed_new;
        r.pending.fixed_old = (int32_t)r.n_fixed;
        r.pending.id_shift = (int32_t)(n_fixed_new - r.n_fixed);
    } else {
        const int t = pick_free(r, r.bufP, -1);
        if ((rc = ensure(ctx, ctx->pts[t], ptsz * (size_t)(n_new + r.shard_extra)))) return rc;
        rc = by_dtype(r.dtype, [&](auto tt) {
            using T = decltype(tt);
            return launch_refix<T>(ctx, pts_of<T>(ctx, r.bufP), r.n, r.n_fixed, n_fixed_new, (const Pt<T>*)d_fixed4,
                                   pts_of<T>(ctx, t), (int32_t*)ctx->scratch.p);
        });
        if (rc) return rc;
        r.bufP = t;
    }
    if (head_remeasures(r, n_fixed_new)) r.tune.valid = false;
    r.n = n_new;
    r.n_fixed = n_fixed_new;
    r.k = (int64_t)r.k_req < n_new ? r.k_req : (int)n_new;
    r.bufS = -1;
    r.bufOld = -1;
    r.have_tree = false;
    r.can_revert = false;
    r.have_point_data = false;
    return (ctx->stream == ctx->own_stream && !keep_alive) ? sync(ctx) : WTP_OK;
}

WTP_API int wtp_relax_set_fixed_dev(wtp_ctx* ctx, const void* d_fixed4, int64_t n_fixed_new) {
    return relax_set_fixed_dev_impl(ctx, d_fixed4, n_fixed_new, false);
}

WTP_API int wtp_relax_set_coverage(wtp_ctx* ctx, int axis, double lo, double hi) {
    if (int rc = need_session(ctx, __func__)) return rc;
    RelaxState& r = ctx->relax;
    if (axis >= r.dim) return fail(ctx, WTP_ERR_ARG, "axis must be < dim (negative: unlimited)");
    if (axis >= 0 && !(lo <= hi)) return fail(ctx, WTP_ERR_ARG, "need lo <= hi");
    r.cover_axis = axis < 0 ? -1 : axis;
    r.cover_lo = lo;
    r.cover_hi = hi;
    return WTP_OK;
}

WTP_API int wtp_relax_step_layers3(wtp_ctx* ctx, int rebuild, wtp_step_stats* stats, int axes_mask, const double lo_in[3],
                                   const double hi_in[3], const double lo_out[3], const double hi_out[3], void* const d_lo4[3],
                                   void* const d_hi4[3], int64_t cap, int64_t counts[12]) {
    int rc = need_session(ctx, __func__);
    if (rc) return rc;
    if (!stats || !counts || !lo_in || !hi_in || !lo_out || !hi_out || !d_lo4 || !d_hi4)
        return fail(ctx, WTP_ERR_ARG, "NULL argument");
    WTP_HIP(ctx, hipSetDevice(ctx->device));
    if ((rc = ensure(ctx, ctx->stats, sizeof(wtp_step_stats)))) return rc;
    if ((rc = relax_step_any(ctx, rebuild, (wtp_step_stats*)ctx->stats.p))) return rc;
    int32_t* d_tot[3] = {nullptr, nullptr, nullptr};
    for (int ax = 0; ax < 3; ++ax)
        if (axes_mask & (1 << ax))
            if ((rc = enqueue_layers(ctx, ax, lo_in[ax], hi_in[ax], lo_out[ax], hi_out[ax], d_lo4[ax], d_hi4[ax], cap,
                                     &d_tot[ax], ax)))
                return rc;
    return read_step(ctx, stats, 3, d_tot, counts);
}

WTP_API int wtp_relax_set_coverage_box(wtp_ctx* ctx, const double lo[3], const double hi[3]) {
    if (!ctx || !lo || !hi) return WTP_ERR_ARG;
    if (int rc = need_session(ctx, __func__)) return rc;
    RelaxState& r = ctx->relax;
    for (int ax = 0; ax < 3; ++ax) {
        if (!(lo[ax] <= hi[ax])) return fail(ctx, WTP_ERR_ARG, "need lo <= hi on every axis");
        r.cover_lo3[ax] = lo[ax];
        r.cover_hi3[ax] = hi[ax];
    }
    r.cover_axis = 3;
    return WTP_OK;
}

WTP_API int wtp_timers_get(wtp_ctx* ctx, double out[4]) {
    if (!ctx || !out) return WTP_ERR_ARG;
    hipSetDevice(ctx->device);
    spans_collect(ctx);
    out[0] = ctx->t_hash;
    out[1] = ctx->t_sweep;
    out[2] = ctx->t_other;
    out[3] = (double)ctx->n_sweep_launches;
    return WTP_OK;
}

WTP_API int wtp_timers_reset(wtp_ctx* ctx) {
    if (!ctx) return WTP_ERR_ARG;
    hipSetDevice(ctx->device);
    spans_collect(ctx);
    ctx->t_hash = ctx->t_sweep = ctx->t_other = 0;
    ctx->n_sweep_launches = 0;
    if (!ctx->timing_forced) ctx->timing = true;
    return WTP_OK;
}

WTP_API int wtp_debug_diag(wtp_ctx* ctx, unsigned long long out[16]) {
    if (!ctx || !out) return WTP_ERR_ARG;
    WTP_HIP(ctx, hipSetDevice(ctx->device));
    int rc;
    if ((rc = ensure(ctx, ctx->diag, 128))) return rc;
    WTP_HIP(ctx, hipMemcpyAsync(out, ctx->diag.p, 128, hipMemcpyDeviceToHost, ctx->stream));
    WTP_HIP(ctx, hipMemsetAsync(ctx->diag.p, 0, 128, ctx->stream));
    if ((rc = sync(ctx))) return rc;
    if (ctx->debug_kd) {
        unsigned long long kd[2] = {0, 0};
        wtp::debug_kd_steps(kd);
        fprintf(stderr, "[wtp] kd walk: %llu node visits by %llu wave-walks (%.1f per walk)\n", kd[0], kd[1], kd[1] ? (double)kd[0] / (double)kd[1] : 0.0);
    }
    return WTP_OK;
}

WTP_API int wtp_gen_uniform_dev(wtp_ctx* ctx, uint64_t seed, int64_t first, int64_t n, int dim, int dtype, void* d_out) {
    if (!ctx || !d_out || n < 0) return WTP_ERR_ARG;
    WTP_HIP(ctx, hipSetDevice(ctx->device));
    int rc = dtype == WTP_F32 ? launch_gen_uniform<float>(ctx, seed, first, n, dim, (float*)d_out)
                              : launch_gen_uniform<double>(ctx, seed, first, n, dim, (double*)d_out);
    if (rc) return rc;
    return sync(ctx);
}
```

whatsthepoint.jl_amd/csrc/wtp_cs2.hip:

```cpp
#include "wtp_device.hpp"

namespace wtp {

#ifndef WTP_DIAG
#define WTP_DIAG 0
#endif
#define CS_STAMP(i)                                                 \
    if (WTP_DIAG) {                                                 \
        const unsigned long long t_ = __builtin_amdgcn_s_memtime(); \
        dt[i] += t_ - t_last;                                       \
        t_last = t_;                                                \
    }

constexpr int kCsThreads = 256;
constexpr int kCsSlab = 16;
constexpr int kCsMaxBX = 61;
constexpr int kCsMaxCells = (kCsMaxBX + 2) * kCsSlab;
constexpr int kCsMaskSteps = 12;
constexpr int kCsSU = 8;
constexpr int kCsPadBytes = 2 * kCsSU * 16;
constexpr int kCsMaxQ = 512;
constexpr int kCsMiss = 16;
constexpr int kCsRun = 2 * kCsSlab + 2 * 4 + 3;

// ... 561 lines not shown
                    if (bi != 0x7FFFFFFF && bd <= e.g2) {
                        const float nd = wsqrt(bd);
                        if (reaches_past_cover<float>(a, qp.x, qp.y, qp.z, bd)) atomicAdd(a.uncovered, 1);
                        a.nn_dist[e.gslot] = nd;
                        a.nn_id[e.gslot] = bi;
                        cs_acc_point(acc, e.f, nd, e.s, e.qid, bi);
                    } else {
                        a.nn_dist[e.gslot] = bd;
                        a.nn_id[e.gslot] = bi == 0x7FFFFFFF ? -1 : bi;
                        const int pos = atomicAdd(a.nn_count, 1);
                        a.nn_list[pos] = e.gslot;
                    }
                }
            }
            if (WTP_DIAG) dt[14] += (unsigned long long)nm;
        }
        CS_STAMP(5)
    }
    if (WTP_DIAG && a.diag && lane == 0) {
        for (int i = 0; i < 15; ++i) atomicAdd(&a.diag[i], dt[i]);
        atomicAdd(&a.diag[15], 1ull);
    }
    __syncthreads();
    Acc full = acc_empty();
    full.max_force = (double)acc.max_force;
    full.sum_u = acc.sum_u;
    full.sum_u2 = acc.sum_u2;
    full.n_move = acc.n_move;
    if (acc.argmin_i >= 0) {
        full.argmin_r = (double)acc.argmin_r;
        full.argmin_i = acc.argmin_i;
        full.argmin_j = acc.argmin_j;
    }
    acc_block_reduce(full, sm->acc);
    if (tid == 0) acc_store(&a.partials[blockIdx.x], full);
}

__global__ void cs2_census_kernel(const int32_t* __restrict__ cell_start, const Grid<float>* __restrict__ gp, int BX,
                                  unsigned int* __restrict__ out ) {
    const Grid<float> g = *gp;
    const int nbx = (g.n[0] + BX - 1) / BX, nby = (g.n[1] + 1) / 2, nbz = (g.n[2] + 1) / 2;
    const int nbricks = nbx * nby * nbz;
    for (int brick = blockIdx.x * blockDim.x + threadIdx.x; brick < nbricks; brick += gridDim.x * blockDim.x) {
        const int bx = brick % nbx, by = (brick / nbx) % nby, bz = brick / (nbx * nby);
        const int gx0 = bx * BX, gx1 = (gx0 + BX - 1) < g.n[0] - 1 ? (gx0 + BX - 1) : g.n[0] - 1;
        const int hx0 = gx0 > 0 ? gx0 - 1 : 0, hx1 = gx1 + 1 < g.n[0] - 1 ? gx1 + 1 : g.n[0] - 1;
        int Q = 0, H = 0;
        for (int r = 0; r < 16; ++r) {
            const int gy = by * 2 - 1 + (r & 3), gz = bz * 2 - 1 + (r >> 2);
            if (gy < 0 || gy >= g.n[1] || gz < 0 || gz >= g.n[2]) continue;
            const int base = (gz * g.n[1] + gy) * g.n[0];
            H += cell_start[base + hx1 + 1] - cell_start[base + hx0];
            const bool own = ((r & 3) == 1 || (r & 3) == 2) && ((r >> 2) == 1 || (r >> 2) == 2);
            if (own) Q += cell_start[base + gx1 + 1] - cell_start[base + gx0];
        }
        if (Q == 0) continue;
        atomicAdd(&out[Q / 2 < 255 ? Q / 2 : 255], 1u);
        atomicAdd(&out[256 + (H / 8 < 255 ? H / 8 : 255)], 1u);
        atomicAdd(&out[512], 1u);
    }
}

int launch_cs2_census(wtp_ctx* ctx, int BX, unsigned int* d_out513) {
    WTP_HIP(ctx, hipMemsetAsync(d_out513, 0, 513 * sizeof(unsigned int), ctx->stream));
    hipLaunchKernelGGL(cs2_census_kernel, dim3(512), dim3(256), 0, ctx->stream, (const int32_t*)ctx->cell_start.p,
                       (const Grid<float>*)ctx->grid.p, BX, d_out513);
    WTP_HIP(ctx, hipGetLastError());
    return WTP_OK;
}

int cs2_max_bx() { return kCsMaxBX; }

constexpr int kNnFixBlocks = 512;
constexpr int kNnFixThreads = 1024;
__global__ __launch_bounds__(kNnFixThreads, 8) void cs2_nnfix_kernel(SearchArgs<float> a, int part_base) {
    if (a.stop && *a.stop) return;
    __shared__ Acc sacc[kNnFixThreads / 64];
    const Grid<float> g = *a.grid;
    const int n = *a.nn_count;
    const int lane = threadIdx.x & 63;
    const int wave_g = (blockIdx.x * kNnFixThreads + threadIdx.x) >> 6, nwaves = (gridDim.x * kNnFixThreads) >> 6;
    Acc acc = acc_empty();
    const int grp = lane >> 4, l16 = lane & 15;
    for (int i0 = wave_g * 4; i0 < n; i0 += nwaves * 4) {
        const int i = i0 + grp;
        const bool on = i < n;
        const int gslot = a.nn_list[on ? i : i0];
        const float4 qp = a.snap[gslot];
        const int32_t qid = w_to_id(qp.w);
        const int cx = cell_coord(g, qp.x, 0), cy = cell_coord(g, qp.y, 1), cz = cell_coord(g, qp.z, 2);
        float bd = a.nn_dist[gslot];
        int32_t bi = a.nn_id[gslot];
        bi = bi < 0 ? 0x7FFFFFFF : bi;
        auto gap = [&](float v, int axis, int c, int lo, int hi) {
            const float a0 = g.org[axis] + (float)(c + lo) * g.c, a1 = g.org[axis] + (float)(c + hi + 1) * g.c;
            float d = v < a0 ? a0 - v : (v > a1 ? v - a1 : 0.f);
            d -= g.margin;
            return d > 0.f ? d : 0.f;
        };
        for (int piece = l16; piece < 75; piece += 16) {
            const int r = piece / 3, seg = piece % 3;
            const int dz = r / 5 - 2, dy = r % 5 - 2;
            const bool inner = dz >= -1 && dz <= 1 && dy >= -1 && dy <= 1;
            if (inner && seg == 1) continue;
            const int gz = cz + dz, gy = cy + dy;
            if (gz < 0 || gz >= g.n[2] || gy < 0 || gy >= g.n[1]) continue;
            int xa = seg == 0 ? cx - 2 : (seg == 1 ? cx - 1 : cx + 2), xb = seg == 1 ? cx + 1 : xa;
            xa = xa < 0 ? 0 : xa;
            xb = xb > g.n[0] - 1 ? g.n[0] - 1 : xb;
            if (xa > xb) continue;
            const bool edge = xa == 0 || xb == g.n[0] - 1 || gy == 0 || gy == g.n[1] - 1 || gz == 0 || gz == g.n[2] - 1;
            if (!edge) {
                const float gx2 = gap(qp.x, 0, 0, xa, xb), gy2 = gap(qp.y, 1, gy, 0, 0), gz2 = gap(qp.z, 2, gz, 0, 0);
                if ((gx2 * gx2 + gy2 * gy2) + gz2 * gz2 > bd) continue;
            }
            const int base = (gz * g.n[1] + gy) * g.n[0];
            const int p1 = a.cell_start[base + xb + 1];
            for (int p = a.cell_start[base + xa]; p < p1; p += 4) {
                float4 c[4];
#pragma unroll
                for (int u = 0; u < 4; ++u) c[u] = a.snap[p + u < p1 ? p + u : p];
#pragma unroll
                for (int u = 0; u < 4; ++u) {
                    const int32_t cid = w_to_id(c[u].w);
                    const float d = dist2<float>(qp.x, qp.y, qp.z, c[u].x, c[u].y, c[u].z);
                    if (p + u < p1 && cid != qid && lex_lt(d, cid, bd, bi)) {
                        bd = d;
                        bi = cid;
                    }
                }
            }
        }
#pragma unroll
        for (int dlt = 8; dlt >= 1; dlt >>= 1) {
            const float od = __shfl_xor(bd, dlt, 64);
            const int32_t oi = __shfl_xor(bi, dlt, 64);
            if (lex_lt(od, oi, bd, bi)) {
                bd = od;
                bi = oi;
            }
        }
        if (l16 == 0 && on) {
            const float g2 = safe_radius2(g, qp.x, qp.y, qp.z, cx, cy, cz, 2);
            if (bi != 0x7FFFFFFF && bd <= g2) {
                const float s = a.spacing_pp ? a.spacing_pp[qid] : a.spacing_const;
                const float nd = wsqrt(bd);
                if (reaches_past_cover<float>(a, qp.x, qp.y, qp.z, bd)) atomicAdd(a.uncovered, 1);
                a.nn_dist[gslot] = nd;
                a.nn_id[gslot] = bi;
                acc_point<float>(acc, a.forces[gslot], nd, s, qid, bi);
            } else {
                const int pos = atomicAdd(a.fb_count, 1);
                a.fb_list[pos] = gslot;
            }
        }
    }
    acc_block_reduce(acc, sacc);
    if (threadIdx.x == 0) acc_store(&a.partials[part_base + blockIdx.x], acc);
}

constexpr int kBallThreads = 256;
constexpr int kBallBlocksMax = 3072;
constexpr int kBallRMax = 4;
#ifndef WTP_BALL_LANES
#define WTP_BALL_LANES 8
#endif
constexpr int kBallLanes = WTP_BALL_LANES;
constexpr int kBallPerWave = 64 / kBallLanes;
__global__ __launch_bounds__(kBallThreads, 6) void cs_ball_kernel(SearchArgs<float> a, const int32_t* __restrict__ list,
                                                               const int32_t* __restrict__ list_count,
                                                               int32_t* __restrict__ out_list, int32_t* __restrict__ out_count,
                                                               int part_base) {
    if (a.stop && *a.stop) return;
    __shared__ Acc sacc[kBallThreads / 64];
    const Grid<float> g = *a.grid;
    const int n = *list_count;
    const int K = a.k;
    const int lane = threadIdx.x & 63;
    const int grp = lane / kBallLanes, l16 = lane % kBallLanes;
    const int wave_g = (blockIdx.x * kBallThreads + threadIdx.x) >> 6, nwaves = (gridDim.x * kBallThreads) >> 6;
    const ForceCoef fc = force_coef(WTP_FORCE_CLIPPED_SPACING, a.beta, a.u0, 0.f);
    Acc acc = acc_empty();
    for (int i0 = wave_g * kBallPerWave; i0 < n; i0 += nwaves * kBallPerWave) {
        const int i = i0 + grp;
        const bool on = i < n;
        const int gslot = list[on ? i : i0];
        const float4 qp = a.query[gslot];
        const int32_t qid = w_to_id(qp.w);
        const float s = a.spacing_pp ? a.spacing_pp[qid] : a.spacing_const;
        const float inv_s2 = 1.f / (s * s);
        const float lim = (a.u0 * a.u0) * (s * s);
        const int cx = cell_coord(g, qp.x, 0), cy = cell_coord(g, qp.y, 1), cz = cell_coord(g, qp.z, 2);
        int R = 0;
        float g2 = 0.f;
#pragma unroll
        for (int r = 1; r <= kBallRMax; ++r) {
            const float t = safe_radius2(g, qp.x, qp.y, qp.z, cx, cy, cz, r);
            const bool take = R == 0 && lim <= t;
            g2 = take ? t : g2;
            R = take ? r : R;
        }
        const bool ok = on && R > 0;
        const int side = 2 * R + 1, nrows = ok ? side * side : 0;
        const int x0 = cx - R < 0 ? 0 : cx - R, x1 = cx + R > g.n[0] - 1 ? g.n[0] - 1 : cx + R;
        int n_lim = 0;
        bool coincident = false;
        float Fx = 0.f, Fy = 0.f, Fz = 0.f;
        int32_t nid = 0x7FFFFFFF;
        float nd2 = Lim<float>::inf();
        constexpr int kRowsPerLane = ((2 * kBallRMax + 1) * (2 * kBallRMax + 1) + kBallLanes - 1) / kBallLanes;
        int ps[kRowsPerLane], pe[kRowsPerLane];
#pragma unroll
        for (int j = 0; j < kRowsPerLane; ++j) {
            const int row = l16 + kBallLanes * j;
            const int y = cy + row % side - R, z = cz + row / side - R;
            const bool in = row < nrows && y >= 0 && y < g.n[1] && z >= 0 && z < g.n[2];
            const int base = in ? (z * g.n[1] + y) * g.n[0] : 0;
            ps[j] = a.cell_start[base + (in ? x0 : 0)];
            pe[j] = in ? a.cell_start[base + x1 + 1] : ps[j];
        }
        auto visit = [&](const float4& c, bool valid) {
            const float dx = qp.x - c.x, dy = qp.y - c.y, dz = qp.z - c.z;
            const float d = (dx * dx + dy * dy) + dz * dz;
            const int32_t cid = w_to_id(c.w);
            const bool inl = valid && d <= lim;
            n_lim += inl ? 1 : 0;
            const bool other = valid && cid != qid;
            const bool nearer = other && lex_lt(d, cid, nd2, nid);
            nd2 = nearer ? d : nd2;
            nid = nearer ? cid : nid;
            const bool act = inl && other;
            const float f = force_fast(fc, d * inv_s2);
            const float coef = (act && d > 0.f) ? f * __builtin_amdgcn_rsqf(d) : 0.f;
            Fx = __builtin_fmaf(coef, dx, Fx);
            Fy = __builtin_fmaf(coef, dy, Fy);
            Fz = __builtin_fmaf(coef, dz, Fz);
            coincident = coincident || (act && !(d > 0.f));
        };
#pragma unroll
        for (int j = 0; j < kRowsPerLane; ++j) {
            for (int p = ps[j]; p < pe[j]; p += 4) {
                float4 c[4];
#pragma unroll
                for (int u = 0; u < 4; ++u) c[u] = a.snap[p + u < pe[j] ? p + u : p];
#pragma unroll
                for (int u = 0; u < 4; ++u) visit(c[u], p + u < pe[j]);
            }
        }
#pragma unroll
        for (int dlt = kBallLanes / 2; dlt >= 1; dlt >>= 1) {
            Fx += __shfl_xor(Fx, dlt, 64);
            Fy += __shfl_xor(Fy, dlt, 64);
            Fz += __shfl_xor(Fz, dlt, 64);
            n_lim += __shfl_xor(n_lim, dlt, 64);
            coincident = coincident || (__shfl_xor((int)coincident, dlt, 64) != 0);
            const float od = __shfl_xor(nd2, dlt, 64);
            const int32_t oi = __shfl_xor(nid, dlt, 64);
            if (lex_lt(od, oi, nd2, nid)) {
                nd2 = od;
                nid = oi;
            }
        }
        if (l16 == 0 && on) {
            const bool nn_ok = nid != 0x7FFFFFFF && (nd2 <= lim || nd2 <= g2);
            if (!ok || n_lim > K || coincident || !nn_ok || qid < a.n_fixed) {
                const int pos = atomicAdd(out_count, 1);
                out_list[pos] = gslot;
            } else {
                float4 o;
                const float f = cs_step_point(a, s, qp.x, qp.y, qp.z, Fx, Fy, Fz, o.x, o.y, o.z);
                o.w = qp.w;
                a.out[gslot] = o;
                a.forces[gslot] = f;
                const float nd = wsqrt(nd2);
                if (reaches_past_cover<float>(a, qp.x, qp.y, qp.z, nd2 > lim ? nd2 : lim)) atomicAdd(a.uncovered, 1);
                a.nn_dist[gslot] = nd;
                a.nn_id[gslot] = nid;
                acc_point<float>(acc, f, nd, s, qid, nid);
            }
        }
    }
    acc_block_reduce(acc, sacc);
    if (threadIdx.x == 0) acc_store(&a.partials[part_base + blockIdx.x], acc);
}

__global__ void cs_all_slots_kernel(int32_t* __restrict__ list, int32_t n, int32_t* __restrict__ count) {
    for (int i = blockIdx.x * blockDim.x + threadIdx.x; i < n; i += gridDim.x * blockDim.x) list[i] = i;
    if (blockIdx.x == 0 && threadIdx.x == 0) *count = n;
}

int launch_cs_all_slots(wtp_ctx* ctx, int32_t* list, int32_t n, int32_t* count) {
    hipLaunchKernelGGL(cs_all_slots_kernel, dim3(1024), dim3(256), 0, ctx->stream, list, n, count);
    WTP_HIP(ctx, hipGetLastError());
    return WTP_OK;
}

int launch_cs_ball(wtp_ctx* ctx, SearchArgs<float>& a, int32_t* rest_list, int32_t* rest_count) {
    int blocks = (int)((a.n + 1023) / 1024);
    blocks = blocks < 8 ? 8 : (blocks > kBallBlocksMax ? kBallBlocksMax : blocks);
    hipLaunchKernelGGL(cs_ball_kernel, dim3(blocks), dim3(kBallThreads), 0, ctx->stream, a, (const int32_t*)a.fb_list,
                       (const int32_t*)a.fb_count, rest_list, rest_count, a.used_brick);
    a.used_brick += blocks;
    a.fb_list = rest_list;
    a.fb_count = rest_count;
    WTP_HIP(ctx, hipGetLastError());
    return WTP_OK;
// ... 89 lines not shown
```

whatsthepoint.jl_amd/csrc/wtp_generic.hip:

```cpp
#include "wtp_device.hpp"

namespace wtp {

static constexpr int kThreads = 128;

template <typename T, int MODE>
__global__ __launch_bounds__(kThreads) void generic_kernel(SearchArgs<T> a, const int32_t* __restrict__ list,
                                                           const int32_t* __restrict__ list_count,
                                                           int all, int part_base) {
    if (a.stop && *a.stop) return;
    __shared__ Acc sm_acc[kThreads / 64];
    const Grid<T> g = *a.grid;
    const int nq = all ? a.n : *list_count;
    const int K = a.k;
    const bool skip_self = (MODE == 0) && !a.include_self;
    T bd[kGenericKMax];
    int32_t bi[kGenericKMax];
    int32_t bp[kGenericKMax];
    Acc acc = acc_empty();

    for (int qi = blockIdx.x * blockDim.x + threadIdx.x; qi < nq; qi += gridDim.x * blockDim.x) {
        const int slot = all ? qi : list[qi];
        const Pt<T> q = a.query[slot];
        const int32_t id = w_to_id(q.w);
        if (MODE == 1 && id < a.n_fixed) {
            a.out[slot] = q;
            a.forces[slot] = (T)0;
            a.nn_dist[slot] = Lim<T>::inf();
            a.nn_id[slot] = -1;
            continue;
        }
        const int cx = cell_coord(g, q.x, 0), cy = cell_coord(g, q.y, 1), cz = cell_coord(g, q.z, 2);
        int m = 0;
        for (int r = 1;; r *= 2) {
            m = 0;
            const int z0 = cz - r < 0 ? 0 : cz - r, z1 = cz + r > g.n[2] - 1 ? g.n[2] - 1 : cz + r;
            const int y0 = cy - r < 0 ? 0 : cy - r, y1 = cy + r > g.n[1] - 1 ? g.n[1] - 1 : cy + r;
            const int x0 = cx - r < 0 ? 0 : cx - r, x1 = cx + r > g.n[0] - 1 ? g.n[0] - 1 : cx + r;
            for (int z = z0; z <= z1; ++z)
                for (int y = y0; y <= y1; ++y) {
                    const int row = (z * g.n[1] + y) * g.n[0];
                    const int ps = a.cell_start[row + x0], pe = a.cell_start[row + x1 + 1];
                    for (int p = ps; p < pe; ++p) {
                        const Pt<T> c = a.snap[p];
                        const int32_t cid = w_to_id(c.w);
                        if (skip_self && cid == id) continue;
                        const T d = dist2<T>(q.x, q.y, q.z, c.x, c.y, c.z);
                        if (m == K && !lex_lt(d, cid, bd[K - 1], bi[K - 1])) continue;
                        int pos = (m < K) ? m++ : K - 1;
                        while (pos > 0 && lex_lt(d, cid, bd[pos - 1], bi[pos - 1])) {
                            bd[pos] = bd[pos - 1];
                            bi[pos] = bi[pos - 1];
                            bp[pos] = bp[pos - 1];
                            --pos;
                        }
                        bd[pos] = d;
                        bi[pos] = cid;
                        bp[pos] = p;
                    }
                }
            const T g2 = safe_radius2(g, q.x, q.y, q.z, cx, cy, cz, r);
            if (g2 == Lim<T>::inf()) break;
            if (m == K && bd[K - 1] <= g2) break;
        }

        if (MODE == 0) {
            int32_t* row = a.idx_out + (int64_t)id * K;
            for (int j = 0; j < K; ++j) row[j] = j < m ? bi[j] : -1;
            if (a.dist_out) {
                T* drow = a.dist_out + (int64_t)id * K;
                for (int j = 0; j < K; ++j) drow[j] = j < m ? wsqrt(bd[j]) : Lim<T>::inf();
            }
        } else {
            const T s = a.spacing_pp ? a.spacing_pp[id] : a.spacing_const;
            T Fx = 0, Fy = 0, Fz = 0;
            int32_t nid = -1;
            T nd = Lim<T>::inf();
            for (int j = 0; j < m; ++j) {
                if (bi[j] == id) continue;
                if (nid < 0) {
                    nid = bi[j];
                    nd = wsqrt(bd[j]);
                }
                const Pt<T> c = a.snap[bp[j]];
                add_force<T>(a, g.dim, s, q.x, q.y, q.z, id, c.x, c.y, c.z, bi[j], bd[j], Fx, Fy, Fz);
            }
            Pt<T> o;
            const T f = step_point<T>(a, s, q.x, q.y, q.z, Fx, Fy, Fz, o.x, o.y, o.z);
            o.w = q.w;
            a.out[slot] = o;
            a.forces[slot] = f;
            a.nn_dist[slot] = nd;
            a.nn_id[slot] = nid;
            acc_point<T>(acc, f, nd, s, id, nid);
            const T need = m == K ? bd[K - 1] : Lim<T>::inf();
            if (reaches_past_cover<T>(a, q.x, q.y, q.z, need)) atomicAdd(a.uncovered, 1);
        }
    }
    if (MODE == 1) {
        acc_block_reduce(acc, sm_acc);
        if (threadIdx.x == 0) acc_store(&a.partials[part_base + blockIdx.x], acc);
    }
}

template <typename T>
__global__ void pack_queries_kernel(const T* __restrict__ xyz, int64_t nq, int dim, Pt<T>* __restrict__ out) {
    const int64_t i = (int64_t)blockIdx.x * blockDim.x + threadIdx.x;
    if (i >= nq) return;
    Pt<T> p;
    p.x = xyz[i * dim];
    p.y = xyz[i * dim + 1];
    p.z = dim == 3 ? xyz[i * dim + 2] : (T)0;
    p.w = id_to_w((T)0, (int32_t)i);
    out[i] = p;
}

template <typename T> int launch_query_knn(wtp_ctx* ctx, SearchArgs<T>& a, const T* d_xyz, int dim, Pt<T>* d_packed) {
    hipLaunchKernelGGL(pack_queries_kernel<T>, dim3((unsigned)((a.n + 255) / 256)), dim3(256), 0, ctx->stream, d_xyz,
                       (int64_t)a.n, dim, d_packed);
    a.query = d_packed;
    a.include_self = 1;
    hipLaunchKernelGGL((generic_kernel<T, 0>), dim3(grid_for(a.n, kThreads, 4096)), dim3(kThreads), 0, ctx->stream, a,
                       (const int32_t*)nullptr, (const int32_t*)nullptr, 1, 0);
    WTP_HIP(ctx, hipGetLastError());
    return WTP_OK;
}

template <typename T>
__global__ __launch_bounds__(kThreads) void radius_kernel(SearchArgs<T> a, T r, const int64_t* __restrict__ offsets,
                                                          int32_t* __restrict__ idx_out, T* __restrict__ d2_tmp,
                                                          const int32_t* __restrict__ list,
                                                          const int32_t* __restrict__ list_count) {
    const Grid<T> g = *a.grid;
    const T r2 = r * r;
    const int nq = list ? *list_count : a.n;
    for (int qi = blockIdx.x * blockDim.x + threadIdx.x; qi < nq; qi += gridDim.x * blockDim.x) {
        const int slot = list ? list[qi] : qi;
        const Pt<T> q = a.snap[slot];
        const int32_t id = w_to_id(q.w);
        const int cx = cell_coord(g, q.x, 0), cy = cell_coord(g, q.y, 1), cz = cell_coord(g, q.z, 2);
        const int z0 = cz - 1 < 0 ? 0 : cz - 1, z1 = cz + 1 > g.n[2] - 1 ? g.n[2] - 1 : cz + 1;
        const int y0 = cy - 1 < 0 ? 0 : cy - 1, y1 = cy + 1 > g.n[1] - 1 ? g.n[1] - 1 : cy + 1;
        const int x0 = cx - 1 < 0 ? 0 : cx - 1, x1 = cx + 1 > g.n[0] - 1 ? g.n[0] - 1 : cx + 1;
        const int64_t base = offsets[id];
        const int64_t cap = offsets[id + 1] - base;
        int32_t m = 0;
        for (int z = z0; z <= z1; ++z)
            for (int y = y0; y <= y1; ++y) {
                const int row = (z * g.n[1] + y) * g.n[0];
                const int ps = a.cell_start[row + x0], pe = a.cell_start[row + x1 + 1];
                for (int p = ps; p < pe; ++p) {
                    const Pt<T> c = a.snap[p];
                    const int32_t cid = w_to_id(c.w);
                    if (cid == id) continue;
                    const T d = dist2<T>(q.x, q.y, q.z, c.x, c.y, c.z);
                    if (!(d <= r2)) continue;
                    if (m >= cap) continue;
                    int64_t pos = m;
                    while (pos > 0 && lex_lt(d, cid, d2_tmp[base + pos - 1], idx_out[base + pos - 1])) {
                        d2_tmp[base + pos] = d2_tmp[base + pos - 1];
                        idx_out[base + pos] = idx_out[base + pos - 1];
                        --pos;
                    }
                    d2_tmp[base + pos] = d;
                    idx_out[base + pos] = cid;
                    ++m;
                }
            }
    }
}


template <typename T> int launch_generic_topology(wtp_ctx* ctx, SearchArgs<T>& a, bool all) {
    if (!a.counters_cleared) WTP_HIP(ctx, hipMemsetAsync(a.fb2_count, 0, sizeof(int32_t), ctx->stream));
    int rc = launch_wave_topology<T>(ctx, a, all);
    if (rc) return rc;
    hipLaunchKernelGGL((generic_kernel<T, 0>), dim3(256), dim3(kThreads), 0, ctx->stream, a, a.fb2_list,
                       a.fb2_count, 0, 0);
    WTP_HIP(ctx, hipGetLastError());
    return WTP_OK;
}


template <typename T> int launch_generic_sweep(wtp_ctx* ctx, SearchArgs<T>& a, bool all) {
    const int part_base = a.n_partials - kGenericPartials;
    int rc = launch_wave_sweep<T>(ctx, a, all);
    if (rc) return rc;
    a.used_generic = grid_for(a.n / 16, kThreads, 256);
    hipLaunchKernelGGL((generic_kernel<T, 1>), dim3(a.used_generic), dim3(kThreads), 0, ctx->stream, a, a.fb2_list,
                       a.fb2_count, 0, part_base);
    WTP_HIP(ctx, hipGetLastError());
    return WTP_OK;
}

template <typename T> static bool brick_radius_usable(wtp_ctx*, SearchArgs<T>&) { return false; }
template <> bool brick_radius_usable<float>(wtp_ctx* ctx, SearchArgs<float>& a) {
    return !ctx->force_generic && a.fb_list != nullptr && a.fb_count != nullptr;
}
template <typename T> static int brick_radius(wtp_ctx*, SearchArgs<T>&) { return WTP_OK; }
template <> int brick_radius<float>(wtp_ctx* ctx, SearchArgs<float>& a) { return launch_brick_radius(ctx, a); }

__global__ void radius_copy_rows_kernel(int64_t n, const int32_t* __restrict__ tmp, const uint8_t* __restrict__ done,
                                        const int32_t* __restrict__ arena, const int64_t* __restrict__ arena_off,
                                        const int64_t* __restrict__ offsets, int32_t* __restrict__ idx) {
    const int64_t grp = ((int64_t)blockIdx.x * blockDim.x + threadIdx.x) >> 4, ngrp = ((int64_t)gridDim.x * blockDim.x) >> 4;
    const int l = threadIdx.x & 15;
    auto meta = [&](int64_t q, uint8_t& d, int64_t& o, int64_t& len, int64_t& ao) {
        d = 0;
        o = len = ao = 0;
        if (q < n) {
            d = done[q];
            o = offsets[q];
            len = offsets[q + 1] - o;
            ao = arena_off ? arena_off[q] : 0;
        }
    };
    uint8_t d, dn;
    int64_t o, len, ao, on, lenn, aon;
    meta(grp, d, o, len, ao);
    for (int64_t q = grp; q < n; q += ngrp) {
        meta(q + ngrp, dn, on, lenn, aon);
        if (d) {
            const int32_t* row;
            int64_t cnt = len;
            if (d == 1) {
                row = tmp + q * 32;
                cnt = cnt > 32 ? 32 : cnt;
            } else {
                row = arena + ao;
            }
            for (int64_t j0 = l; j0 < cnt; j0 += 64) {
                int32_t v[4];
#pragma unroll
                for (int u = 0; u < 4; ++u) v[u] = j0 + 16 * u < cnt ? row[j0 + 16 * u] : 0;
#pragma unroll
                for (int u = 0; u < 4; ++u)
                    if (j0 + 16 * u < cnt) idx[o + j0 + 16 * u] = v[u];
            }
        }
        d = dn;
        o = on;
        len = lenn;
        ao = aon;
    }
}

template <typename T>
int launch_radius_count(wtp_ctx* ctx, SearchArgs<T>& a, T r, int32_t* d_counts) {
    const bool dense = ctx->radius_dense && !ctx->force_generic && a.rad_done && a.rad_arena && a.rad_arena_pos && a.rad_bricks && a.fb_list && a.fb_count;
    a.rad_dense = dense ? radius_dense_hcap<T>() : 0;
    if (brick_radius_usable<T>(ctx, a) || dense) {
        WTP_HIP(ctx, hipMemsetAsync(a.fb_count, 0, sizeof(int32_t), ctx->stream));
        int rc;
        if (brick_radius_usable<T>(ctx, a)) {
            a.radius2 = r * r;
            a.rad_counts = d_counts;
            a.rad_offsets = nullptr;
            a.rad_fill = 0;
            if ((rc = brick_radius<T>(ctx, a))) return rc;
        }
        if (dense && (rc = launch_radius_dense<T>(ctx, a, r, d_counts))) return rc;
        return launch_wave_radius_count<T>(ctx, a, r, d_counts, a.fb_list, a.fb_count);
    }
    return launch_wave_radius_count<T>(ctx, a, r, d_counts, nullptr, nullptr);
}

template <typename T>
int launch_radius_fill(wtp_ctx* ctx, SearchArgs<T>& a, T r, const int64_t* d_offsets, int32_t* d_idx) {
    WTP_HIP(ctx, hipMemsetAsync(a.fb2_count, 0, sizeof(int32_t), ctx->stream));
    hipLaunchKernelGGL(radius_copy_rows_kernel, dim3(grid_for((int64_t)a.n * 16, kThreads, 16384)), dim3(kThreads), 0, ctx->stream,
                       (int64_t)a.n, (const int32_t*)a.rad_tmp, (const uint8_t*)a.rad_done, (const int32_t*)a.rad_arena,
                       (const int64_t*)a.rad_arena_off, d_offsets, d_idx);
    int rc;
    if ((brick_radius_usable<T>(ctx, a) && a.rad_tmp) || a.rad_dense)
        rc = launch_wave_radius_fill<T>(ctx, a, r, d_offsets, d_idx, a.fb_list, a.fb_count);
    else
        rc = launch_wave_radius_fill<T>(ctx, a, r, d_offsets, d_idx, nullptr, nullptr);
    if (rc) return rc;
    hipLaunchKernelGGL((radius_kernel<T>), dim3(256), dim3(kThreads), 0, ctx->stream, a, r, d_offsets, d_idx,
                       (T*)ctx->scratch.p, (const int32_t*)a.fb2_list, (const int32_t*)a.fb2_count);
    WTP_HIP(ctx, hipGetLastError());
    return WTP_OK;
}

#define INST(T)                                                                              \
    template int launch_generic_topology<T>(wtp_ctx*, SearchArgs<T>&, bool);                 \
    template int launch_query_knn<T>(wtp_ctx*, SearchArgs<T>&, const T*, int, Pt<T>*);         \
    template int launch_generic_sweep<T>(wtp_ctx*, SearchArgs<T>&, bool);                    \
    template int launch_radius_count<T>(wtp_ctx*, SearchArgs<T>&, T, int32_t*);              \
    template int launch_radius_fill<T>(wtp_ctx*, SearchArgs<T>&, T, const int64_t*, int32_t*);
INST(float)
INST(double)
#undef INST

}
```

whatsthepoint.jl_amd/csrc/wtp_hash.hip:

```cpp
#include "wtp_device.hpp"

namespace wtp {

static constexpr int kThreads = 256;

template <typename T>
__global__ void load_points_kernel(const T* __restrict__ xyz, Pt<T>* __restrict__ out, int64_t n, int dim) {
    int64_t i = (int64_t)blockIdx.x * blockDim.x + threadIdx.x;
    int64_t stride = (int64_t)gridDim.x * blockDim.x;
    for (; i < n; i += stride) {
        Pt<T> p;
        p.x = xyz[i * dim + 0];
        p.y = xyz[i * dim + 1];
        p.z = dim == 3 ? xyz[i * dim + 2] : (T)0;
        p.w = id_to_w((T)0, (int32_t)i);
        out[i] = p;
    }
}

template <typename T>
__global__ void bbox_kernel(const Pt<T>* __restrict__ pts, int64_t n, T* __restrict__ part, int64_t v_old = 0,
                            int32_t v_fixed_old = 0) {
    __shared__ T sm[6][kThreads / 64];
    T mn[3] = {Lim<T>::inf(), Lim<T>::inf(), Lim<T>::inf()};
// ... 436 lines not shown
    WTP_HIP(ctx, hipMemsetAsync(d_out, 0, 2 * sizeof(double), ctx->stream));
    hipLaunchKernelGGL(sum_kernel<T>, dim3(grid_for(n, kThreads, 1024)), dim3(kThreads), 0, ctx->stream, d_v, n, d_out);
    WTP_HIP(ctx, hipGetLastError());
    return WTP_OK;
}

int launch_bbox64(wtp_ctx* ctx, const double4* pts, int64_t n, int* nparts) {
    *nparts = grid_for(n, kThreads, 1024);
    int rc;
    if ((rc = ensure(ctx, ctx->bbox_part, sizeof(double) * 6 * 1024))) return rc;
    hipLaunchKernelGGL(bbox_kernel<double>, dim3(*nparts), dim3(kThreads), 0, ctx->stream, pts, n, (double*)ctx->bbox_part.p);
    WTP_HIP(ctx, hipGetLastError());
    return WTP_OK;
}

static constexpr int kHistBins = 1024;

template <typename T>
__global__ void axis_hist_kernel(const Pt<T>* __restrict__ pts, int64_t n, int dim, const double* __restrict__ range,
                                 unsigned int* __restrict__ hist) {
    __shared__ unsigned int sh[3 * kHistBins];
    for (int i = threadIdx.x; i < 3 * kHistBins; i += blockDim.x) sh[i] = 0;
    __syncthreads();
    double lo[3], scale[3];
    for (int a = 0; a < 3; ++a) {
        lo[a] = range[a];
        const double w = range[3 + a] - range[a];
        scale[a] = w > 0 ? (double)kHistBins / w : 0.0;
    }
    for (int64_t i = (int64_t)blockIdx.x * blockDim.x + threadIdx.x; i < n; i += (int64_t)gridDim.x * blockDim.x) {
        const Pt<T> p = pts[i];
        const double v[3] = {(double)p.x, (double)p.y, (double)p.z};
        for (int a = 0; a < dim; ++a) {
            double f = (v[a] - lo[a]) * scale[a];
            int b = f > 0 ? (f < (double)(kHistBins - 1) ? (int)f : kHistBins - 1) : 0;
            atomicAdd(&sh[a * kHistBins + b], 1u);
        }
    }
    __syncthreads();
    for (int i = threadIdx.x; i < 3 * kHistBins; i += blockDim.x)
        if (sh[i]) atomicAdd(&hist[i], sh[i]);
}

template <typename T>
int launch_axis_hist(wtp_ctx* ctx, const Pt<T>* pts, int64_t n, int dim, const double* d_range, unsigned int* d_hist) {
    WTP_HIP(ctx, hipMemsetAsync(d_hist, 0, sizeof(unsigned int) * 3 * kHistBins, ctx->stream));
    hipLaunchKernelGGL(axis_hist_kernel<T>, dim3(grid_for(n, kThreads, 512)), dim3(kThreads), 0, ctx->stream, pts, n, dim,
                       d_range, d_hist);
    WTP_HIP(ctx, hipGetLastError());
    return WTP_OK;
}

template <typename T> int launch_occupancy(wtp_ctx* ctx, const Grid<T>* g, unsigned long long* d_out3) {
    WTP_HIP(ctx, hipMemsetAsync(d_out3, 0, 3 * sizeof(unsigned long long), ctx->stream));
    hipLaunchKernelGGL(occupancy_kernel, dim3(1024), dim3(kThreads), 0, ctx->stream, (const int32_t*)ctx->cell_start.p,
                       (const int32_t*)&g->ncells, d_out3);
    WTP_HIP(ctx, hipGetLastError());
    return WTP_OK;
}

template <typename T> static int hash_scratch(wtp_ctx* ctx, const HashBuild<T>& b, int* cap_out, bool* fresh) {
    const int k_cap = b.rho_direct > 0 ? (int)(b.rho_direct * 21.0 / ctx->rho) : (b.radius > 0 ? 6 : b.k);
    const int cap = cell_capacity(ctx, b.n, k_cap > 0 ? k_cap : 1, b.cell_scale > 0 ? b.cell_scale : 1.0);
    int rc;
    if ((rc = ensure(ctx, ctx->grid, sizeof(Grid<double>)))) return rc;
    if ((rc = ensure(ctx, ctx->bbox_part, sizeof(double) * 6 * 1024))) return rc;
    const void* cnt_before = ctx->cell_cnt.p;
    const void* dirty_before = ctx->rank_of.p;
    if ((rc = ensure(ctx, ctx->cell_cnt, sizeof(int32_t) * (size_t)(cap + 1)))) return rc;
    if ((rc = ensure(ctx, ctx->cell_start, sizeof(int32_t) * (size_t)(cap + 2)))) return rc;
    if ((rc = ensure(ctx, ctx->cell_of, sizeof(int32_t) * (size_t)b.n_in()))) return rc;
    if ((rc = ensure(ctx, ctx->rank_of, (size_t)cap + 64))) return rc;
    const int nscan = (cap + kScanTile - 1) / kScanTile;
    if ((rc = ensure(ctx, ctx->scan_tmp, sizeof(int32_t) * (size_t)(nscan + 1)))) return rc;
    *cap_out = cap;
    *fresh = cnt_before != ctx->cell_cnt.p || dirty_before != ctx->rank_of.p;
    return WTP_OK;
}

template <typename T> int prerank_old_snapshot(wtp_ctx* ctx, const HashBuild<T>& next) {
    int cap = 0, rc;
    bool fresh = false;
    ctx->prerank.valid = false;
    if ((rc = hash_scratch(ctx, next, &cap, &fresh))) return rc;
    int32_t* cnt = (int32_t*)ctx->cell_cnt.p;
    uint8_t* dirty = (uint8_t*)ctx->rank_of.p;
    if (!ctx->hash_scratch_clean || fresh) {
        WTP_HIP(ctx, hipMemsetAsync(cnt, 0, ctx->cell_cnt.cap, ctx->stream));
        WTP_HIP(ctx, hipMemsetAsync(dirty, 0, ctx->rank_of.cap, ctx->stream));
    }
    ctx->hash_scratch_clean = false;
    const int64_t n_old = next.view.n_old;
    const int nb = grid_for(n_old, kThreads, 16384);
    hipLaunchKernelGGL(cell_rank_kernel<T>, dim3(nb), dim3(kThreads), 0, ctx->stream, next.in, n_old, (const Grid<T>*)ctx->grid.p,
                       cnt, (int32_t*)ctx->cell_of.p, next.canonical ? dirty : (uint8_t*)nullptr, n_old, next.view.fixed_old,
                       ctx->stop_dev);
    WTP_HIP(ctx, hipGetLastError());
    Prerank& p = ctx->prerank;
    p.valid = true;
    p.in = next.in;
    p.n_old = n_old;
    p.fixed_old = next.view.fixed_old;
    p.canonical = next.canonical;
    p.cnt = cnt;
    p.cr = ctx->cell_of.p;
    p.dirty = dirty;
    return WTP_OK;
}

template <typename T> static bool prerank_matches(const wtp_ctx* ctx, const HashBuild<T>& b, bool fresh) {
    const Prerank& p = ctx->prerank;
    const bool same_request = b.keep_grid && b.view.active && p.in == (const void*)b.in && p.n_old == b.view.n_old &&
                              p.fixed_old == b.view.fixed_old && p.canonical == b.canonical;
    const bool same_scratch = !fresh && p.cnt == ctx->cell_cnt.p && p.cr == ctx->cell_of.p && p.dirty == ctx->rank_of.p;
    return p.valid && same_request && same_scratch;
}

template <typename T> int build_hash(wtp_ctx* ctx, const HashBuild<T>& b) {
    const double cell_scale = b.cell_scale > 0 ? b.cell_scale : 1.0;
    const HashView& hv = b.view;
    const int64_t n = b.n, n_in = b.n_in();
    const int64_t v_old = hv.active ? hv.n_old : 0;
    const int32_t v_fixed_old = hv.active ? hv.fixed_old : 0, v_shift = hv.active ? hv.id_shift : 0;
    const int nbb = grid_for(n_in, kThreads, 1024);
    int cap = 0, rc;
    bool fresh = false;
    if ((rc = hash_scratch(ctx, b, &cap, &fresh))) return rc;
    const int nscan = (cap + kScanTile - 1) / kScanTile;

    const Pt<T>* in = b.in;
    Pt<T>* out = b.out;
    Grid<T>* g = (Grid<T>*)ctx->grid.p;
    T* part = (T*)ctx->bbox_part.p;
    int32_t* cnt = (int32_t*)ctx->cell_cnt.p;
    int32_t* start = (int32_t*)ctx->cell_start.p;
    int32_t* cr = (int32_t*)ctx->cell_of.p;
    uint8_t* dirty = (uint8_t*)ctx->rank_of.p;
    uint8_t* marks = b.canonical ? dirty : nullptr;
    int32_t* bs = (int32_t*)ctx->scan_tmp.p;
    hipStream_t st = ctx->stream;

    double rho_k = (b.dim == 3 ? 0.381 : 0.436) * (double)(b.k > 0 ? b.k : 21) * (ctx->rho / 8.0);
    if (b.rho_direct > 0) rho_k = b.rho_direct;
    if (rho_k < 1.0) rho_k = 1.0;

    const bool half_done = prerank_matches(ctx, b, fresh);
    ctx->prerank.valid = false;
    if (!half_done && (!ctx->hash_scratch_clean || fresh)) {
        WTP_HIP(ctx, hipMemsetAsync(cnt, 0, ctx->cell_cnt.cap, st));
        WTP_HIP(ctx, hipMemsetAsync(dirty, 0, ctx->rank_of.cap, st));
    }
    ctx->hash_scratch_clean = false;
    ctx->preranked_builds += half_done ? 1 : 0;
    if (!b.keep_grid) {
        hipLaunchKernelGGL(bbox_kernel<T>, dim3(nbb), dim3(kThreads), 0, st, in, n_in, part, v_old, v_fixed_old);
        hipLaunchKernelGGL(grid_setup_kernel<T>, dim3(1), dim3(64), 0, st, part, nbb, g, n, b.dim, rho_k, b.radius, b.min_cell,
                           cap, cell_scale, b.box, ctx->stop_dev);
    }
    const int nb = grid_for(n_in, kThreads, 16384);
    if (half_done) {
        if (n_in > v_old)
            hipLaunchKernelGGL(cell_rank_kernel<T>, dim3(grid_for(n_in - v_old, kThreads, 16384)), dim3(kThreads), 0, st, in + v_old,
                               n_in - v_old, g, cnt, cr + v_old, marks, (int64_t)0, 0, ctx->stop_dev);
    } else {
        hipLaunchKernelGGL(cell_rank_kernel<T>, dim3(nb), dim3(kThreads), 0, st, in, n_in, g, cnt, cr, marks, v_old, v_fixed_old,
                           ctx->stop_dev);
    }
    hipLaunchKernelGGL(scan_reduce_kernel<T>, dim3(nscan), dim3(kThreads), 0, st, cnt, g, bs);
    hipLaunchKernelGGL(scan_apply_kernel<T>, dim3(nscan), dim3(kThreads), 0, st, cnt, bs, g, start, ctx->stop_dev);
    hipLaunchKernelGGL(scatter_kernel<T>, dim3(nb), dim3(kThreads), 0, st, in, n_in, cr, g, start, out, v_old, v_fixed_old,
                       v_shift, ctx->stop_dev);
    if (b.canonical) {
        hipLaunchKernelGGL(canon_kernel<T>, dim3(grid_for((cap + 15) / 16, kThreads, 4096)), dim3(kThreads), 0, st, out, start,
                           dirty, g, ctx->stop_dev);
    }
    WTP_HIP(ctx, hipGetLastError());
    ctx->hash_scratch_clean = true;
    return WTP_OK;
}

template <typename T>
__global__ void unpermute_kernel(const Pt<T>* __restrict__ pts, int64_t n, int64_t n_fixed, int dim,
                                 T* __restrict__ out) {
    int64_t i = (int64_t)blockIdx.x * blockDim.x + threadIdx.x;
    int64_t stride = (int64_t)gridDim.x * blockDim.x;
    for (; i < n; i += stride) {
        Pt<T> p = pts[i];
        int64_t id = w_to_id(p.w);
        if (id < n_fixed) continue;
        T* o = out + (id - n_fixed) * dim;
        o[0] = p.x;
        o[1] = p.y;
        if (dim == 3) o[2] = p.z;
    }
}

template <typename T>
__global__ void unpermute_pd_kernel(const Pt<T>* __restrict__ pts, int64_t n, int64_t n_fixed,
                                    const T* __restrict__ forces, const T* __restrict__ nn_dist,
                                    const int32_t* __restrict__ nn_id, T* __restrict__ fo,
                                    T* __restrict__ no, int32_t* __restrict__ io) {
    int64_t i = (int64_t)blockIdx.x * blockDim.x + threadIdx.x;
    int64_t stride = (int64_t)gridDim.x * blockDim.x;
    for (; i < n; i += stride) {
        int64_t id = w_to_id(pts[i].w);
        if (id < n_fixed) continue;
        int64_t o = id - n_fixed;
        if (fo) fo[o] = forces[i];
        if (no) no[o] = nn_dist[i];
        if (io) io[o] = nn_id[i];
    }
}

template <typename T>
__global__ void set_point_kernel(Pt<T>* __restrict__ pts, int64_t n, int32_t id, int dim, const T* __restrict__ v) {
    int64_t i = (int64_t)blockIdx.x * blockDim.x + threadIdx.x;
    int64_t stride = (int64_t)gridDim.x * blockDim.x;
    for (; i < n; i += stride) {
        if (w_to_id(pts[i].w) == id) {
            pts[i].x = v[0];
            pts[i].y = v[1];
            pts[i].z = dim == 3 ? v[2] : (T)0;
        }
    }
}

static constexpr int kOffTile = 2048;
__global__ __launch_bounds__(kThreads) void offsets_tile_sum_kernel(const int32_t* __restrict__ cnt, int64_t n,
                                                                   int64_t* __restrict__ tile_sum) {
    __shared__ int64_t sm[kThreads / 64];
    const int64_t base = (int64_t)blockIdx.x * kOffTile;
    int64_t s = 0;
    for (int i = threadIdx.x; i < kOffTile; i += kThreads)
        if (base + i < n) s += cnt[base + i];
    for (int o = 32; o > 0; o >>= 1) s += __shfl_xor(s, o);
    if ((threadIdx.x & 63) == 0) sm[threadIdx.x >> 6] = s;
    __syncthreads();
    if (threadIdx.x == 0) {
        int64_t t = 0;
        for (int w = 0; w < kThreads / 64; ++w) t += sm[w];
        tile_sum[blockIdx.x] = t;
    }
}
__global__ void offsets_tile_scan_kernel(int64_t* __restrict__ tile_sum, int64_t ntiles) {
    int64_t run = 0;
    for (int64_t i = 0; i < ntiles; ++i) {
        const int64_t t = tile_sum[i];
        tile_sum[i] = run;
        run += t;
    }
    tile_sum[ntiles] = run;
}
__global__ __launch_bounds__(kThreads) void offsets_apply_kernel(const int32_t* __restrict__ cnt, int64_t n,
                                                                const int64_t* __restrict__ tile_sum,
                                                                int64_t* __restrict__ off) {
    constexpr int kRun = kOffTile / kThreads;
    __shared__ int64_t sm[kThreads];
    const int64_t base = (int64_t)blockIdx.x * kOffTile + (int64_t)threadIdx.x * kRun;
    int32_t v[kRun];
    int64_t s = 0;
#pragma unroll
    for (int i = 0; i < kRun; ++i) {
        v[i] = base + i < n ? cnt[base + i] : 0;
        s += v[i];
    }
    sm[threadIdx.x] = s;
    __syncthreads();
    if (threadIdx.x == 0) {
        int64_t run = tile_sum[blockIdx.x];
        for (int t = 0; t < kThreads; ++t) {
            const int64_t x = sm[t];
            sm[t] = run;
            run += x;
        }
    }
    __syncthreads();
    int64_t run = sm[threadIdx.x];
#pragma unroll
    for (int i = 0; i < kRun; ++i) {
        if (base + i < n) off[base + i] = run;
        run += v[i];
    }
    if (blockIdx.x == gridDim.x - 1 && threadIdx.x == 0) off[n] = tile_sum[gridDim.x];
}

int launch_offsets_scan(wtp_ctx* ctx, const int32_t* d_cnt, int64_t n, int64_t* d_tmp, int64_t* d_off) {
    const int64_t ntiles = (n + kOffTile - 1) / kOffTile;
    hipLaunchKernelGGL(offsets_tile_sum_kernel, dim3((unsigned)ntiles), dim3(kThreads), 0, ctx->stream, d_cnt, n, d_tmp);
    hipLaunchKernelGGL(offsets_tile_scan_kernel, dim3(1), dim3(1), 0, ctx->stream, d_tmp, ntiles);
    hipLaunchKernelGGL(offsets_apply_kernel, dim3((unsigned)ntiles), dim3(kThreads), 0, ctx->stream, d_cnt, n,
                       (const int64_t*)d_tmp, d_off);
    WTP_HIP(ctx, hipGetLastError());
    return WTP_OK;
}
size_t offsets_scan_tmp_bytes(int64_t n) { return sizeof(int64_t) * (size_t)((n + kOffTile - 1) / kOffTile + 2); }

template <typename T>
int launch_unpermute(wtp_ctx* ctx, const Pt<T>* pts, int64_t n, int64_t n_fixed, int dim, T* d_out) {
    hipLaunchKernelGGL(unpermute_kernel<T>, dim3(grid_for(n, kThreads, 8192)), dim3(kThreads), 0,
                       ctx->stream, pts, n, n_fixed, dim, d_out);
    WTP_HIP(ctx, hipGetLastError());
    return WTP_OK;
}

template <typename T>
int launch_unpermute_point_data(wtp_ctx* ctx, const Pt<T>* pts, int64_t n, int64_t n_fixed,
                                const T* forces, const T* nn_dist, const int32_t* nn_id, T* fo, T* no,
                                int32_t* io) {
    hipLaunchKernelGGL(unpermute_pd_kernel<T>, dim3(grid_for(n, kThreads, 8192)), dim3(kThreads), 0,
                       ctx->stream, pts, n, n_fixed, forces, nn_dist, nn_id, fo, no, io);
    WTP_HIP(ctx, hipGetLastError());
    return WTP_OK;
}

template <typename T>
__global__ void set_points_kernel(Pt<T>* __restrict__ pts, int64_t n, const int32_t* __restrict__ ids, int64_t m, int dim,
                                  const T* __restrict__ v) {
    int64_t i = (int64_t)blockIdx.x * blockDim.x + threadIdx.x;
    const int64_t stride = (int64_t)gridDim.x * blockDim.x;
    for (; i < n; i += stride) {
        const int32_t id = w_to_id(pts[i].w);
// ... 339 lines not shown
```

whatsthepoint.jl_amd/csrc/wtp_internal.hpp:

```cpp
#pragma once
#include <hip/hip_runtime.h>
#include <stdint.h>
#include <map>
#include <string>
#include <utility>
#include <vector>

#include "../../include/wtp.h"

namespace wtp {

template <typename T> struct PtOf;
template <> struct PtOf<float> { using type = float4; };
template <> struct PtOf<double> { using type = double4; };
template <typename T> using Pt = typename PtOf<T>::type;

template <typename F> inline auto by_dtype(int dtype, F&& f) { return dtype == WTP_F32 ? f(float{}) : f(double{}); }

__host__ __device__ inline float id_to_w(float, int32_t id) { return __builtin_bit_cast(float, id); }
__host__ __device__ inline double id_to_w(double, int32_t id) {
    return __builtin_bit_cast(double, (int64_t)id);
}
__host__ __device__ inline int32_t w_to_id(float w) { return __builtin_bit_cast(int32_t, w); }
__host__ __device__ inline int32_t w_to_id(double w) {
    return (int32_t)__builtin_bit_cast(int64_t, w);
}

template <typename T> struct Grid {
    T org[3];
    T c;
    T inv_c;
    T margin;
    int32_t n[3];
    int32_t ncells;
    int32_t nb[3];
    int32_t nbricks;
    int32_t dim;
    int32_t npts;
    int32_t rad_wave_only;
    int32_t pad_;
};

constexpr int kMaxAxisCells = 4096;

constexpr int BX = 4, BY = 4, BZ = 4;
constexpr int HX = BX + 2, HY = BY + 2, HZ = BZ + 2;
constexpr int HCELLS = HX * HY * HZ;
constexpr int kRadDenseMin = 1600;
constexpr int kBrickThreads = 256;
constexpr int kRadArenaPerPoint = 48;
constexpr int kWavePartials = 4096;
constexpr int kGenericPartials = 1024;
int brick_partials();
constexpr int kGenericKMax = 128;

constexpr double kGammaCap = 1.0;
constexpr double kGammaCapSweep = 0.96;
constexpr double kTnnFrac = 0.8;
constexpr double kRhoCs2 = 1.0;
constexpr double kRhoKsel = 1.2;
constexpr double kCapKsel = 40.0;
constexpr int kGridReuseMax = 7;

struct Partial {
    double max_force;
    double sum_u;
    double sum_u2;
    double argmin_r;
    int64_t argmin_i;
    int64_t argmin_j;
    int64_t n_move;
};

struct ForceParams {
    int32_t kind;
    double beta, u0, gamma;
};

template <typename T> struct SearchArgs {
    const Grid<T>* grid;
    const Pt<T>* snap;
    const int32_t* cell_start;
    const Pt<T>* query;
    int32_t n;
    int32_t k;
    int32_t include_self;
    int32_t* idx_out;
    T* dist_out;
    Pt<T>* out;
    T* forces;
    T* nn_dist;
    int32_t* nn_id;
    const T* spacing_pp;
    T spacing_const;
    T alpha_lo, alpha_max;
    T beta, u0, gamma;
    int32_t force_kind;
    int32_t n_fixed;
    Partial* partials;
    int32_t n_partials;
    int32_t used_brick, used_wave, used_generic;
    T radius2;
    int32_t* rad_counts;
    const int64_t* rad_offsets;
    int32_t rad_fill;
    int32_t* rad_tmp;
    uint8_t* rad_done;
    int32_t* rad_arena;
    int64_t* rad_arena_off;
    unsigned long long* rad_arena_pos;
    int64_t rad_arena_cap;
    int32_t* rad_bricks;
    int32_t rad_dense;
    int32_t* fb_list;
    int32_t* fb_count;
    int32_t* fb2_list;
    int32_t* fb2_count;
    int32_t* nn_list;
    int32_t* nn_count;
    int32_t* ball_list;
    int32_t* ball_count;
    const int32_t* stop;
    int32_t cover_axis;
    T cover_lo, cover_hi;
    T cover_lo3[3], cover_hi3[3];
    int32_t* uncovered;
    T gamma_cap;
    float cap_count;
    T tnn_frac;
    int32_t brick_hcap;
    int32_t cs2_bx;
    const uint8_t* brick_dead;
    int32_t brick_dead_cap;
    int32_t cs2_chunked;
    int32_t counters_cleared;
    int32_t fb_r0;
    int32_t ksel_bx;
    unsigned long long* diag;
};

struct DevBuf {
    void* p = nullptr;
    size_t cap = 0;
    DevBuf() = default;
    DevBuf(const DevBuf&) = delete;
    DevBuf& operator=(const DevBuf&) = delete;
    DevBuf(DevBuf&& o) noexcept : p(o.p), cap(o.cap) {
        o.p = nullptr;
        o.cap = 0;
    }
    DevBuf& operator=(DevBuf&& o) noexcept {
        std::swap(p, o.p);
        std::swap(cap, o.cap);
        return *this;
    }
    ~DevBuf() {
        if (p) hipFree(p);
    }
};

struct HashView {
    bool active = false;
    int64_t n_in = 0;
    int64_t n_old = 0;
    int32_t fixed_old = 0;
    int32_t id_shift = 0;
};

template <typename T> struct HashBuild {
    const Pt<T>* in;
    Pt<T>* out;
    int64_t n;
    int dim;
    int k;
    double radius = 0.0;
    double rho_direct = 0.0;
    double min_cell = 0.0;
    double cell_scale = 1.0;
    HashView view;
    bool keep_grid = false;
    bool canonical = true;
    const double* box = nullptr;
    HashBuild(const Pt<T>* in_, Pt<T>* out_, int64_t n_, int dim_, int k_) : in(in_), out(out_), n(n_), dim(dim_), k(k_) {}
    int64_t n_in() const { return view.active ? view.n_in : n; }
};

struct Prerank {
    bool valid = false;
    const void* in = nullptr;
    int64_t n_old = 0;
    int32_t fixed_old = 0;
    bool canonical = true;
    const void *cnt = nullptr, *cr = nullptr, *dirty = nullptr;
};

struct GridTune {
    bool loose = false;
    bool valid = false;
    bool clipped = false;
    int64_t n = 0;
    int dim = 0, kq = 0;
    bool ksel = false;
    double scale = 1.0;
    double rho = 0;
    int bx = 0, hcap = 0;
};

enum class SweepRoute {
    Exact,
    Select,
    Ksel,
    Cs,
    Cs2,
    Cs64,
    Cs64Wave,
    Ball,
    F64Ksel,
};

struct RelaxState {
    bool active = false;
    int64_t n = 0, n_fixed = 0;
    int dim = 3, dtype = 0, k = 0;
    int k_req = 0;
    int spacing_kind = 0;
    double spacing_const = 0, alpha_lo = 0, alpha_max = 0;
    ForceParams force{};
    int bufS = -1, bufP = -1, bufOld = -1;
    bool have_tree = false;
    bool can_revert = false;
    bool have_point_data = false;
    double spacing_max = 0;
    int brick_hcap = 0;
    GridTune tune;
    int grid_age = 0;
    int sweeps_since_rebuild = 0;
    bool moved_by_hand = false;
    double spacing_typ = 0;
    SweepRoute route = SweepRoute::Exact;
    bool cs_disabled = false;
    double cs2_rho = 0;
    int cs2_bx = 0;
    int64_t tuned_fixed = 0;
    double sp_p0 = 0, sp_p1 = 0, sp_p2 = 0;
    HashView pending;
    int64_t shard_extra = 0;
    int64_t aux_off = 0;
    int swap_target = -1;
    bool shard_grid_reuse = false;
    int64_t grid_fixed = -1;
    GridTune f64k_tune{true};
    bool wall_active = false;
    double wall_offset = 0;
    int64_t wall_nm = 0;
    int cover_axis = -1;
    double cover_lo = 0, cover_hi = 0;
    double cover_lo3[3] = {0, 0, 0}, cover_hi3[3] = {0, 0, 0};
};

}

struct wtp_ctx {
    int device = 0;
    hipStream_t stream = nullptr;
    hipStream_t own_stream = nullptr;
    std::string err;
    int sm_count = 256;
    double rho = 9.0;
    int force_generic = 0;
    int full_select = 0;
    int ksel = 1;
    int ball64 = 1;
    int f64_ksel = 1;
    int radius_dense = 1;
    int block_overlap = 1;
    bool debug = false;
    bool debug_kd = false;
    size_t cs2_smem = 0;
    const void* cs2_fn = nullptr;
    int cs2_occ = 0;
    std::map<std::pair<const void*, size_t>, int> launch_cache;
    wtp::GridTune knn_tune, knn64_tune;
    wtp::DevBuf pts[3];
    wtp::DevBuf raw_in;
    wtp::DevBuf cell_of, rank_of, cell_cnt, cell_start, scan_tmp;
    wtp::DevBuf grid, bbox_part, occ;
    wtp::DevBuf box_dev;
    wtp::DevBuf idx_out, dist_out, counts_out;
    wtp::DevBuf cand_idx, cand_dist, f32_pts;
    wtp::DevBuf grid_b, cell_start_b, box_b, f64k_s64, f64k_slot, f64k_lists, f64k_cnt;
    wtp::DevBuf forces, nn_dist, nn_id, spacing_pp;
    wtp::DevBuf partials, stats, fb_list, fb_count, fb2_list, fb2_count, nn_list;
    wtp::DevBuf rad_pos;
    wtp::DevBuf rad_bricks;
    bool rad_dense_attr[2] = {false, false};
    bool rad_dense_used = false;
    wtp::DevBuf rad_tmp, rad_done;
    wtp::DevBuf rad_arena, rad_arena_off;
    wtp::DevBuf brick_dead;
    wtp::Prerank prerank;
    int64_t preranked_builds = 0;
    hipStream_t comm_stream = nullptr;
    hipEvent_t ev_comm_a = nullptr, ev_comm_b = nullptr;
    bool hash_scratch_clean = false;
    bool counters_clean = false;
    wtp::DevBuf stop_state;
    const int32_t* stop_dev = nullptr;
    wtp::DevBuf scratch;
    wtp::DevBuf diag;
    wtp::DevBuf ins_in, ins_elems, ins_partial, ins_out;
    wtp::DevBuf mesh_nodes, mesh_pn, mesh_io;
    int64_t mesh_nt = 0;
    int mesh_dtype = -1;
    double mesh_bbox[6] = {0, 0, 0, 0, 0, 0};
    double mesh_scale = 0;
    std::vector<double> mesh_face_host;
    wtp::DevBuf wall_flags, wall_tri;
    wtp::DevBuf wall_hint;
    wtp::DevBuf mesh_cls;
    bool mesh_cls_ready = false;
    int mesh_cls_dim[3] = {0, 0, 0};
    double mesh_cls_cell = 0;
    wtp::DevBuf sp_hint;
    wtp::DevBuf kd_nodes;
    int64_t kd_m = 0;
    uint64_t kd_key = 0;
    int kd_dim = 0, kd_dtype = -1;
    int64_t n_syncs = 0;
    void* block = nullptr;
    void* block_topo = nullptr;
    void* comm = nullptr;
    int comm_rank = 0, comm_size = 0;
    wtp::DevBuf comm_scratch;
    wtp::DevBuf sp_cert;
    void* host_pinned = nullptr;
    size_t host_pinned_cap = 0;
    int64_t rad_n = 0;
    int rad_dim = 0, rad_dtype = 0;
    double rad_r = 0;
    int64_t rad_nnz = 0;
    bool rad_valid = false;
    bool rad_offsets_dev = false;
    wtp::RelaxState relax;
    bool timing = false;
    bool timing_forced = false;
    double t_hash = 0, t_sweep = 0, t_other = 0;
    int64_t n_sweep_launches = 0;
    std::vector<hipEvent_t> ev_pool;
    struct Span { int a, b, kind; };
    std::vector<Span> spans;
    int ev_used = 0;
    int ev_last_end = -1;
};

namespace wtp {

int fail(wtp_ctx* ctx, int code, const std::string& msg);
int ensure_pinned(wtp_ctx* ctx, size_t bytes);
#define WTP_HIP(ctx, call)                                                                    \
    do {                                                                                      \
        hipError_t e_ = (call);                                                               \
        if (e_ != hipSuccess)                                                                 \
            return ::wtp::fail(ctx, e_ == hipErrorOutOfMemory ? WTP_ERR_OOM : WTP_ERR_HIP,    \
                               std::string(#call) + ": " + hipGetErrorString(e_));            \
    } while (0)

int ensure(wtp_ctx* ctx, DevBuf& b, size_t bytes);
template <typename T> Pt<T>* pts_of(wtp_ctx* ctx, int i) { return (Pt<T>*)ctx->pts[i].p; }
int need_session(wtp_ctx* ctx, const char* entry);
int launch_occupancy_of(wtp_ctx* ctx, const void* fn, int threads, size_t smem);

int span_begin(wtp_ctx* ctx, int kind);
void span_end(wtp_ctx* ctx, int span);
void spans_collect(wtp_ctx* ctx);

template <typename T> int build_hash(wtp_ctx* ctx, const HashBuild<T>& b);
template <typename T> int prerank_old_snapshot(wtp_ctx* ctx, const HashBuild<T>& next);
template <typename T> int launch_occupancy(wtp_ctx* ctx, const Grid<T>* g, unsigned long long* d_out3);
template <typename T> int launch_sum(wtp_ctx* ctx, const T* d_v, int64_t n, double* d_out);
int launch_offsets_scan(wtp_ctx* ctx, const int32_t* d_cnt, int64_t n, int64_t* d_tmp, int64_t* d_off);
size_t offsets_scan_tmp_bytes(int64_t n);
template <typename T>
int launch_axis_hist(wtp_ctx* ctx, const Pt<T>* pts, int64_t n, int dim, const double* d_range, unsigned int* d_hist);

template <typename T>
int load_points(wtp_ctx* ctx, const T* d_xyz, Pt<T>* out, int64_t n, int dim);

inline int grid_for(int64_t n, int threads, int cap) {
    int64_t b = (n + threads - 1) / threads;
    if (b < 1) b = 1;
    return (int)(b > cap ? cap : b);
}
template <typename T> int launch_topology(wtp_ctx* ctx, SearchArgs<T>& a);
int launch_brick_sweep(wtp_ctx* ctx, SearchArgs<float>& a, bool cs);
template <typename T> int launch_brick_cs(wtp_ctx* ctx, SearchArgs<T>& a);
template <typename T> int launch_wave_topology(wtp_ctx* ctx, SearchArgs<T>& a, bool all);
template <typename T> int launch_wave_sweep(wtp_ctx* ctx, SearchArgs<T>& a, bool all);
template <typename T>
int launch_wave_radius_count(wtp_ctx* ctx, SearchArgs<T>& a, T r, int32_t* d_counts, const int32_t* list,
                             const int32_t* list_count);
template <typename T>
int launch_wave_radius_fill(wtp_ctx* ctx, SearchArgs<T>& a, T r, const int64_t* d_offsets, int32_t* d_idx,
                            const int32_t* list, const int32_t* list_count);
template <typename T> int launch_generic_topology(wtp_ctx* ctx, SearchArgs<T>& a, bool all);
template <typename T> int launch_query_knn(wtp_ctx* ctx, SearchArgs<T>& a, const T* d_xyz, int dim, Pt<T>* d_packed);
template <typename T> int launch_generic_sweep(wtp_ctx* ctx, SearchArgs<T>& a, bool all);
inline int total_partials() { return brick_partials() + kWavePartials + kGenericPartials; }
int launch_brick_radius(wtp_ctx* ctx, SearchArgs<float>& a);
int launch_cs2(wtp_ctx* ctx, SearchArgs<float>& a);
int launch_cs2_followup(wtp_ctx* ctx, SearchArgs<float>& a);
int debug_kd_steps(unsigned long long out[2]);
int launch_cs_ball(wtp_ctx* ctx, SearchArgs<float>& a, int32_t* rest_list, int32_t* rest_count);
int launch_cs2_census(wtp_ctx* ctx, int BX, unsigned int* d_out513);
int launch_cs2_dead(wtp_ctx* ctx, SearchArgs<float>& a, uint8_t* d_dead, int dead_cap);
int cs2_max_bx();
int launch_ksel_topology(wtp_ctx* ctx, SearchArgs<float>& a);
int launch_ksel_sweep(wtp_ctx* ctx, SearchArgs<float>& a);
int ksel_max_bx();
int ksel_kmax();
template <typename T>
int launch_radius_count(wtp_ctx* ctx, SearchArgs<T>& a, T r, int32_t* d_counts);
template <typename T>
int launch_radius_fill(wtp_ctx* ctx, SearchArgs<T>& a, T r, const int64_t* d_offsets,
                       int32_t* d_idx);
int launch_reduce_partials(wtp_ctx* ctx, const Partial* parts, int n_parts, int used_brick, int used_wave,
                           int used_generic, const int32_t* fb_count, const int32_t* uncovered,
                           const int32_t* escaped, wtp_step_stats* d_stats_slot);
template <typename T>
int launch_pca_normals(wtp_ctx* ctx, const T* d_xyz, int64_t n, int dim, const int32_t* d_rows, int k, T* d_out);
template <typename T>
int launch_minplus_batch(wtp_ctx* ctx, const int32_t* d_rows, const T* d_dist, int64_t n, int k, double g, double tol,
                         T* d_h0, T* d_h1, int first, int sweeps, unsigned long long* d_state);
template <typename TP>
int launch_mesh_constrain(wtp_ctx* ctx, const Pt<TP>* old, Pt<TP>* cur, int64_t n, int64_t n_fixed, double offset,
                          const uint8_t* is_bnd, uint8_t* escaped, int32_t* tri_idx, int32_t* hint, int32_t* n_escaped);
template <typename T>
int launch_unpermute(wtp_ctx* ctx, const Pt<T>* pts, int64_t n, int64_t n_fixed, int dim, T* d_xyz_out);
template <typename T>
int launch_unpermute_point_data(wtp_ctx* ctx, const Pt<T>* pts, int64_t n, int64_t n_fixed,
                                const T* forces, const T* nn_dist, const int32_t* nn_id,
                                T* forces_o, T* nn_dist_o, int32_t* nn_id_o);
template <typename T>
int launch_set_points(wtp_ctx* ctx, Pt<T>* pts, int64_t n, const int32_t* d_ids, int64_t m, int dim, const T* d_v);
template <typename T>
int launch_set_point(wtp_ctx* ctx, Pt<T>* pts, int64_t n, int32_t id, int dim, const T* d_xyz3);
template <typename T>
int launch_gen_uniform(wtp_ctx* ctx, uint64_t seed, int64_t first, int64_t n, int dim, T* d_out);
template <typename T> size_t kd_bytes(int64_t m);
template <typename T> void kd_build_host(const T* xyz, int64_t m, int dim, void* out);
template <typename T>
int launch_spacing_eval(wtp_ctx* ctx, const T* d_xyz, int64_t n, int dim, const void* d_nodes, int64_t m, int kind,
                        double p0, double p1, double p2, T* d_out);
template <typename T>
int launch_spacing_session(wtp_ctx* ctx, const Pt<T>* pts, int64_t n, int64_t first_id, const void* d_nodes, int64_t m,
                           int kind, double p0, double p1, double p2, T* d_spacing_pp, int32_t* d_hint,
                           const int32_t* d_cell_start = nullptr, const void* d_grid = nullptr, void* d_cert = nullptr);
int launch_bbox64(wtp_ctx* ctx, const double4* pts, int64_t n, int* nparts);
int launch_origin(wtp_ctx* ctx, const double4* pts, int64_t n, double* d_org4);
int launch_to_local_f32(wtp_ctx* ctx, const double4* in, int64_t n, const double* d_org4, float4* out);
int launch_relabel_slots(wtp_ctx* ctx, const double4* raw, float4* sorted32, double4* sorted64, int32_t* sslot, int64_t n);
int launch_refine_f64(wtp_ctx* ctx, const double4* raw, const int32_t* cand, const float* cdist, int64_t n, int kc, int k,
                      int include_self, const double* d_org4, int32_t* idx_out, double* dist_out, int32_t* fail_list,
                      int32_t* fail_count);
int launch_refine_f64_slots(wtp_ctx* ctx, const double4* sorted, const int32_t* cand, const float* cdist, int64_t n, int kc, int k,
                            int include_self, const double* d_org4, int32_t* idx_out, double* dist_out, int32_t* fail_list,
                            int32_t* fail_count);
int launch_refine_sweep_f64(wtp_ctx* ctx, SearchArgs<double>& a, const double4* s64, const int32_t* sslot, const int32_t* cand,
                            const float* cdist, const double* d_org4);
int isinside_chunks(wtp_ctx* ctx, int64_t n, int64_t m, int points_per_block);
int isinside_greens_ppb();
int isinside_winding_ppb();
size_t isinside_elem_bytes(int dtype);
template <typename T>
int launch_isinside_greens(wtp_ctx* ctx, const T* d_test, int64_t n, const T* d_p, const T* d_nrm, const T* d_area,
                           int64_t m, void* d_elems, int chunks, T* d_partial, T* d_g, uint8_t* d_inside);
template <typename T>
int launch_isinside_winding(wtp_ctx* ctx, const T* d_test, int64_t n, const T* d_poly, int64_t m, int chunks,
                            T* d_partial, int32_t* d_coincident, T* d_sum, uint8_t* d_inside);
int layer_blocks(int64_t n);
template <typename T>
int launch_layers(wtp_ctx* ctx, const Pt<T>* pts, int64_t n, int64_t n_fixed, int axis, double lo_in, double hi_in,
                  double lo_out, double hi_out, Pt<T>* d_lo, Pt<T>* d_hi, int64_t cap, int2* d_blk, int32_t* d_totals,
                  bool slot_ordered, double reach);
template <typename T> int launch_append_fixed(wtp_ctx* ctx, const Pt<T>* d_src, int64_t n, Pt<T>* d_dst);
int relax_step_enqueue(wtp_ctx* ctx, int rebuild, wtp_step_stats* d_slot);
int relax_swap_begin(wtp_ctx* ctx, int64_t n_move_new, void** d_buf_out);
int relax_swap_commit(wtp_ctx* ctx, int64_t n_move_new);
int relax_set_fixed_dev_impl(wtp_ctx* ctx, const void* d_fixed4, int64_t n_fixed_new, bool keep_alive);
int comm_exchange_peers_on(wtp_ctx* ctx, hipStream_t stream, int n_msgs, const int* peers, const void* const* d_send,
                           const int64_t* n_send, void* const* d_recv, const int64_t* n_recv);
template <typename T> int launch_radius_dense(wtp_ctx* ctx, SearchArgs<T>& a, T r, int32_t* d_counts);
template <typename T> int radius_dense_hcap();
int launch_cs_all_slots(wtp_ctx* ctx, int32_t* list, int32_t n, int32_t* count);
int launch_cs_ball64(wtp_ctx* ctx, SearchArgs<double>& a, int32_t* rest_list, int32_t* rest_count);
int relax_prerank(wtp_ctx* ctx, int64_t n_fixed_new);
void block_destroy(wtp_ctx* ctx);
void block_topo_destroy(wtp_ctx* ctx);
bool block_session_open(wtp_ctx* ctx);
const wtp_transport* block_host_transport(wtp_ctx* ctx);
int launch_blk_scan(wtp_ctx* ctx, int32_t* span_counts, int64_t nspans, int ncol, int32_t* totals);
int topo_knn_local(wtp_ctx* ctx, const float* d_xyz, int64_t n, int k, int include_self, int32_t* d_idx, float* d_dist);
int topo_radius_local(wtp_ctx* ctx, const float* d_xyz, int64_t n, double r, int32_t* d_counts, int64_t* d_off, DevBuf& d_idx,
                      int64_t* nnz);
template <typename T>
int launch_refix(wtp_ctx* ctx, const Pt<T>* in, int64_t n_old, int64_t n_fixed_old, int64_t n_fixed_new,
                 const Pt<T>* d_fixed_new, Pt<T>* out, int32_t* d_counter);

}
```

whatsthepoint.jl_amd/csrc/wtp_wave.hip:

```cpp
#include "wtp_device.hpp"

namespace wtp {

static constexpr int kWaves = 4;
static constexpr int kThreads = kWaves * 64;
static constexpr int kCap = 512;
static constexpr int kKeyRegs = kCap / 64;
static constexpr int kSurv = 256;

template <typename T> struct Bits;
template <> struct Bits<float> {
    using U = uint32_t;
    static __device__ U of(float v) { return __builtin_bit_cast(uint32_t, v); }
    static __device__ float back(U u) { return __builtin_bit_cast(float, u); }
    static constexpr U kInf = 0x7F800000u;
};
template <> struct Bits<double> {
    using U = uint64_t;
    static __device__ U of(double v) { return __builtin_bit_cast(uint64_t, v); }
    static __device__ double back(U u) { return __builtin_bit_cast(double, u); }
    static constexpr U kInf = 0x7FF0000000000000ull;
};

template <typename T, bool SWEEP> struct WaveSmem;
template <typename T> struct WaveSmem<T, true> {
    T d2[kCap];
    int32_t id[kCap];
    int32_t slot[kCap];
    T sd2[kSurv];
    int32_t sid[kSurv];
    int32_t sslot[kSurv];
    T od2[kGenericKMax];
    int32_t oid[kGenericKMax];
    int32_t oslot[kGenericKMax];
};
static_assert(3 * kGenericKMax <= kCap, "the force terms reuse the candidate list");
template <typename T> struct WaveSmem<T, false> {
    T d2[kCap];
    int32_t id[kCap];
    T sd2[kSurv];
    int32_t sid[kSurv];
    T od2[kGenericKMax];
    int32_t oid[kGenericKMax];
};

__device__ inline int lane_id() { return __builtin_amdgcn_mbcnt_hi(~0u, __builtin_amdgcn_mbcnt_lo(~0u, 0)); }

template <typename T, int MODE>
__global__ __launch_bounds__(kThreads) void wave_kernel(SearchArgs<T> a, const int32_t* __restrict__ list,
                                                        const int32_t* __restrict__ list_count, int all,
                                                        int part_base) {
    if (a.stop && *a.stop) return;
    extern __shared__ __attribute__((aligned(16))) unsigned char smem_raw[];
    using U = typename Bits<T>::U;
    const int wave = threadIdx.x >> 6;
    const int lane = threadIdx.x & 63;
    using Smem = WaveSmem<T, MODE == 1>;
    Smem* sm = reinterpret_cast<Smem*>(smem_raw) + wave;
    Acc* sm_acc = reinterpret_cast<Acc*>(smem_raw + sizeof(Smem) * kWaves);
    const Grid<T> g = *a.grid;
    const int nq = all ? a.n : *list_count;
    const int K = a.k;
    const bool skip_self = (MODE == 0) && !a.include_self;
    Acc acc = acc_empty();
    const int wave_global = blockIdx.x * kWaves + wave;
    const int wave_stride = gridDim.x * kWaves;

    for (int qi = wave_global; qi < nq; qi += wave_stride) {
        const int slot = all ? qi : list[qi];
        const Pt<T> q = a.query[slot];
        const int32_t id = w_to_id(q.w);
        if (MODE == 1 && id < a.n_fixed) {
            if (lane == 0) {
                a.out[slot] = q;
                a.forces[slot] = (T)0;
                a.nn_dist[slot] = Lim<T>::inf();
                a.nn_id[slot] = -1;
            }
            continue;
        }
        const int cx = cell_coord(g, q.x, 0), cy = cell_coord(g, q.y, 1), cz = cell_coord(g, q.z, 2);
        int m = 0;
        bool overflow = false;
        int Kq = K;
        T cs_lim = (T)0;
        int cs_r = 0;
        if (MODE == 1 && a.force_kind == WTP_FORCE_CLIPPED_SPACING && K >= 2) {
            const T s = a.spacing_pp ? a.spacing_pp[id] : a.spacing_const;
            cs_lim = (a.u0 * a.u0) * (s * s);
            for (int r = 1; r <= 6 && !cs_r; ++r)
                if (safe_radius2(g, q.x, q.y, q.z, cx, cy, cz, r) >= cs_lim) cs_r = r;
        }
        bool cs_try = cs_r > 0, cs_done = false;
        for (int r2 = all ? 1 : (a.fb_r0 > 0 ? a.fb_r0 : 2);;) {
            const int r = cs_try ? cs_r : r2;
            m = 0;
            const T g2 = safe_radius2(g, q.x, q.y, q.z, cx, cy, cz, r);
            const int z0 = cz - r < 0 ? 0 : cz - r, z1 = cz + r > g.n[2] - 1 ? g.n[2] - 1 : cz + r;
            const int y0 = cy - r < 0 ? 0 : cy - r, y1 = cy + r > g.n[1] - 1 ? g.n[1] - 1 : cy + r;
            const int x0 = cx - r < 0 ? 0 : cx - r, x1 = cx + r > g.n[0] - 1 ? g.n[0] - 1 : cx + r;
            auto consume = [&](int p, bool valid, const Pt<T>& c) {
                bool take = false;
                T d = 0;
                int32_t cid = 0;
                if (valid) {
                    cid = w_to_id(c.w);
                    d = dist2<T>(q.x, q.y, q.z, c.x, c.y, c.z);
                    take = (d <= g2) && !(skip_self && cid == id);
                }
                const unsigned long long mask = __ballot(take);
                const int pos = m + __popcll(mask & ((1ull << lane) - 1ull));
                if (take && pos < kCap) {
                    sm->d2[pos] = d;
                    sm->id[pos] = cid;
                    if constexpr (MODE == 1) sm->slot[pos] = p;
                }
                m += __popcll(mask);
                if (m > kCap) overflow = true;
            };
            const int ny_rows = y1 - y0 + 1;
            const int nrows = ny_rows * (z1 - z0 + 1);
            for (int rb = 0; rb < nrows && !overflow; rb += 64) {
                int my_ps = 0, my_pe = 0;
                if (rb + lane < nrows) {
                    const int i = rb + lane;
                    const int row = ((z0 + i / ny_rows) * g.n[1] + (y0 + i % ny_rows)) * g.n[0];
                    my_ps = a.cell_start[row + x0];
                    my_pe = a.cell_start[row + x1 + 1];
                }
                const int my_len = my_pe - my_ps;
                int incl = my_len;
#pragma unroll
                for (int d = 1; d < 64; d <<= 1) {
                    const int o = __shfl_up(incl, d, 64);
                    if (lane >= d) incl += o;
                }
                const int total = __shfl(incl, 63, 64);
                const int excl = incl - my_len;
                for (int base = 0; base < total && !overflow; base += 2 * 64) {
                    Pt<T> c[2];
                    int pp[2];
                    bool vv[2];
#pragma unroll
                    for (int u = 0; u < 2; ++u) {
                        const int f = base + u * 64 + lane;
                        vv[u] = f < total;
                        int lo = 0, hi = 63;
#pragma unroll
                        for (int it = 0; it < 6; ++it) {
                            const int mid = (lo + hi + 1) >> 1;
                            const bool ge = __shfl(excl, mid, 64) <= f;
                            lo = ge ? mid : lo;
                            hi = ge ? hi : mid - 1;
                        }
                        pp[u] = __shfl(my_ps, lo, 64) + (f - __shfl(excl, lo, 64));
                        c[u] = a.snap[vv[u] ? pp[u] : 0];
                    }
                    consume(pp[0], vv[0], c[0]);
                    if (base + 64 < total && !overflow) consume(pp[1], vv[1], c[1]);
                }
            }
            if (cs_try) {
                cs_try = false;
                int m_lim = 0;
                if (!overflow) {
                    for (int i0 = 0; i0 < m; i0 += 64) {
                        const int i = i0 + lane;
                        m_lim += __popcll(__ballot(i < m && sm->d2[i] <= cs_lim));
                    }
                }
                if (!overflow && m_lim >= 2 && m_lim <= K) {
                    Kq = m_lim;
                    cs_done = true;
                    break;
                }
                if (!overflow && m_lim == 1) {
                    Kq = 2;
                    if (m >= 2) break;
                    r2 = r + 1;
                }
                overflow = false;
                continue;
            }
            if (overflow) break;
            if (m >= Kq) break;
            if (g2 == Lim<T>::inf()) break;
            r2 *= 2;
        }
        if (overflow || m < Kq) {
            if (lane == 0) {
                const int pos = atomicAdd(a.fb2_count, 1);
                a.fb2_list[pos] = slot;
            }
            continue;
        }
        __builtin_amdgcn_wave_barrier();

        U key[kKeyRegs];
#pragma unroll
        for (int j = 0; j < kKeyRegs; ++j) {
            const int i = j * 64 + lane;
            key[j] = i < m ? Bits<T>::of(sm->d2[i]) : ~(U)0;
        }
        U lo = 0, hi = cs_done ? Bits<T>::of(cs_lim) : Bits<T>::kInf;
        bool lo_valid = false;
        while (!cs_done) {
            bool found = false;
            U pivot = 0;
#pragma unroll
            for (int j = 0; j < kKeyRegs; ++j) {
                if (!found && j * 64 < m) {
                    const unsigned long long mask = __ballot((!lo_valid || key[j] > lo) && key[j] < hi);
                    if (mask) {
                        const unsigned long long upper = mask & (~0ull << 31);
                        const int src = __builtin_ctzll(upper ? upper : mask);
                        pivot = __shfl(key[j], src, 64);
                        found = true;
                    }
                }
            }
            if (!found) break;
            int cnt = 0;
#pragma unroll
            for (int j = 0; j < kKeyRegs; ++j)
                if (j * 64 < m) cnt += __popcll(__ballot(key[j] <= pivot));
            if (cnt >= Kq) {
                hi = pivot;
            } else {
                lo = pivot;
                lo_valid = true;
            }
        }
        lo = hi;
        const U cut = lo;
        int ns = 0;
#pragma unroll
        for (int j = 0; j < kKeyRegs; ++j) {
            if (j * 64 < m) {
                const int i = j * 64 + lane;
                const bool take = key[j] <= cut;
                const unsigned long long mask = __ballot(take);
                const int pos = ns + __popcll(mask & ((1ull << lane) - 1ull));
                if (take && pos < kSurv) {
                    sm->sd2[pos] = sm->d2[i];
                    sm->sid[pos] = sm->id[i];
                    if constexpr (MODE == 1) sm->sslot[pos] = sm->slot[i];
                }
                ns += __popcll(mask);
            }
        }
        if (ns > kSurv) {
            if (lane == 0) {
                const int pos = atomicAdd(a.fb2_count, 1);
                a.fb2_list[pos] = slot;
            }
            continue;
        }
        __builtin_amdgcn_wave_barrier();
        for (int i = lane; i < ns; i += 64) {
            const T md = sm->sd2[i];
            const int32_t mi = sm->sid[i];
            int rank = 0;
            for (int j = 0; j < ns; ++j) rank += lex_lt(sm->sd2[j], sm->sid[j], md, mi) ? 1 : 0;
            if (rank < Kq) {
                sm->od2[rank] = md;
                sm->oid[rank] = mi;
                if constexpr (MODE == 1) sm->oslot[rank] = sm->sslot[i];
            }
        }
        __builtin_amdgcn_wave_barrier();

        if constexpr (MODE == 0) {
            for (int j = lane; j < K; j += 64) {
                a.idx_out[(int64_t)id * K + j] = sm->oid[j];
                if (a.dist_out) a.dist_out[(int64_t)id * K + j] = wsqrt(sm->od2[j]);
            }
        } else {
            const T s = a.spacing_pp ? a.spacing_pp[id] : a.spacing_const;
            T* const sfx = sm->d2;
            T* const sfy = sm->d2 + kGenericKMax;
            T* const sfz = sm->d2 + 2 * kGenericKMax;
            for (int j = lane; j < Kq; j += 64) {
                T fx = 0, fy = 0, fz = 0;
                if (sm->oid[j] != id) {
                    const Pt<T> c = a.snap[sm->oslot[j]];
                    add_force<T>(a, g.dim, s, q.x, q.y, q.z, id, c.x, c.y, c.z, sm->oid[j], sm->od2[j], fx, fy, fz);
                }
                sfx[j] = fx;
                sfy[j] = fy;
                sfz[j] = fz;
            }
            __builtin_amdgcn_wave_barrier();
            if (lane == 0) {
                T Fx = 0, Fy = 0, Fz = 0;
                int32_t nid = -1;
                T nd = Lim<T>::inf();
                for (int j = 0; j < Kq; ++j) {
                    if (sm->oid[j] == id) continue;
                    if (nid < 0) {
                        nid = sm->oid[j];
                        nd = wsqrt(sm->od2[j]);
                    }
                    Fx = Fx + sfx[j];
                    Fy = Fy + sfy[j];
                    Fz = Fz + sfz[j];
                }
                Pt<T> o;
                const T f = step_point<T>(a, s, q.x, q.y, q.z, Fx, Fy, Fz, o.x, o.y, o.z);
                o.w = q.w;
                a.out[slot] = o;
                a.forces[slot] = f;
                a.nn_dist[slot] = nd;
                a.nn_id[slot] = nid;
                acc_point<T>(acc, f, nd, s, id, nid);
                const T last = sm->od2[Kq - 1];
                const T need = cs_done ? cs_lim : (Kq < K ? (last > cs_lim ? last : cs_lim) : last);
                if (reaches_past_cover<T>(a, q.x, q.y, q.z, need)) atomicAdd(a.uncovered, 1);
            }
        }
        __builtin_amdgcn_wave_barrier();
    }
    if (MODE == 1) {
        __syncthreads();
        acc_block_reduce(acc, sm_acc);
        if (threadIdx.x == 0) acc_store(&a.partials[part_base + blockIdx.x], acc);
    }
}

constexpr int kRadCap = 512;
template <typename T> struct RadSmem;
template <> struct RadSmem<float> {
    unsigned long long key[kRadCap + 2];
};
template <> struct RadSmem<double> {
    double d2[kRadCap + 2];
    int32_t id[kRadCap + 2];
};

template <typename T, bool FILL>
__global__ __launch_bounds__(kThreads, sizeof(T) == 4 ? 8 : 5) void wave_radius_kernel(SearchArgs<T> a, T r, int32_t* __restrict__ counts,
                                                               const int64_t* __restrict__ offsets,
                                                               int32_t* __restrict__ idx_out,
                                                               const int32_t* __restrict__ list,
                                                               const int32_t* __restrict__ list_count) {
    __shared__ RadSmem<T> sm_all[FILL ? kWaves : 1];
    const int wave = __builtin_amdgcn_readfirstlane((int)(threadIdx.x >> 6));
    const int lane = threadIdx.x & 63;
    RadSmem<T>* sm = &sm_all[FILL ? wave : 0];
    const Grid<T> g = *a.grid;
    const T r2 = r * r;
    const int wave_global = blockIdx.x * kWaves + wave;
    const int wave_stride = gridDim.x * kWaves;
    const bool all = !list || (g.rad_wave_only && !a.rad_dense);
    const int nq = all ? a.n : *list_count;
    const unsigned long long below = lane == 0 ? 0ull : (~0ull >> (64 - lane));
    int64_t arena_used = 0;
    auto slot_of = [&](int qi) { return qi < nq ? (all ? qi : list[qi]) : 0; };
    auto row_bounds = [&](const Pt<T>& p, bool on, int& b_ps, int& b_pe) {
        const int cx = cell_coord(g, p.x, 0), cy = cell_coord(g, p.y, 1), cz = cell_coord(g, p.z, 2);
        const int z0 = cz - 1 < 0 ? 0 : cz - 1, z1 = cz + 1 > g.n[2] - 1 ? g.n[2] - 1 : cz + 1;
        const int y0 = cy - 1 < 0 ? 0 : cy - 1, y1 = cy + 1 > g.n[1] - 1 ? g.n[1] - 1 : cy + 1;
        const int x0 = cx - 1 < 0 ? 0 : cx - 1, x1 = cx + 1 > g.n[0] - 1 ? g.n[0] - 1 : cx + 1;
        const int ny = y1 - y0 + 1, nrows = ny * (z1 - z0 + 1);
        b_ps = 0;
        b_pe = 0;
        if (on && lane < nrows) {
            const int row = ((z0 + lane / ny) * g.n[1] + (y0 + lane % ny)) * g.n[0];
            b_ps = a.cell_start[row + x0];
            b_pe = a.cell_start[row + x1 + 1];
        }
    };
    int qi = wave_global;
    int slot0 = slot_of(qi), slot1 = slot_of(qi + wave_stride), slot2 = slot_of(qi + 2 * wave_stride);
    Pt<T> q0 = a.snap[slot0], q1 = a.snap[slot1];
    int b0_ps, b0_pe;
    row_bounds(q0, qi < nq, b0_ps, b0_pe);
    for (; qi < nq; qi += wave_stride) {
        const int slot = slot0;
        const Pt<T> q = q0;
        asm volatile("" : "+v"(b0_ps), "+v"(b0_pe));
        const int my_ps = b0_ps, my_pe = b0_pe;
        const int32_t id = w_to_id(q.w);
        int done = 0;
        if (FILL && !counts && all && a.rad_done) done = a.rad_done[id];
        int64_t off_lo = 0, off_hi = 0;
        if (FILL && !counts) {
            off_lo = offsets[id];
            off_hi = offsets[id + 1];
        }
        row_bounds(q1, qi + wave_stride < nq, b0_ps, b0_pe);
        slot0 = slot1;
        q0 = q1;
        slot1 = slot2;
        q1 = a.snap[slot2];
        slot2 = slot_of(qi + 3 * wave_stride);
        if (done == 2) continue;
        int ps[9], len[9];
        Pt<T> c[9];
#pragma unroll
        for (int rr = 0; rr < 9; ++rr) {
            ps[rr] = __builtin_amdgcn_readlane(my_ps, rr);
            len[rr] = __builtin_amdgcn_readlane(my_pe, rr) - ps[rr];
        }
#pragma unroll
        for (int rr = 0; rr < 9; ++rr) {
            const int last = len[rr] - 1;
            c[rr] = a.snap[ps[rr] + (len[rr] > 0 ? (lane < last ? lane : last) : 0)];
        }
        int m = 0;
        auto visit = [&](const Pt<T>& cc, bool on) {
            bool take = false;
            T d = 0;
            int32_t cid = 0;
            if (on) {
                cid = w_to_id(cc.w);
                d = dist2<T>(q.x, q.y, q.z, cc.x, cc.y, cc.z);
                take = (d <= r2) && (cid != id);
            }
            const unsigned long long mask = __ballot(take);
            if (FILL) {
                const int pos = m + __popcll(mask & below);
                if (take && pos < kRadCap) {
                    if constexpr (sizeof(T) == 4) {
                        sm->key[pos] = ((unsigned long long)__builtin_bit_cast(uint32_t, (float)d) << 32) | (uint32_t)cid;
                    } else {
                        reinterpret_cast<RadSmem<double>*>(sm)->d2[pos] = (double)d;
                        reinterpret_cast<RadSmem<double>*>(sm)->id[pos] = cid;
                    }
                }
            }
            m += __popcll(mask);
        };
#pragma unroll
        for (int rr = 0; rr < 9; ++rr) {
            if (len[rr] <= 0) continue;
            visit(c[rr], lane < len[rr]);
            for (int p0 = 64; p0 < len[rr]; p0 += 64) {
                const bool on = p0 + lane < len[rr];
                Pt<T> cc{};
                int first = ps[rr] + p0;
                asm volatile("" : "+s"(first));
                if (on) cc = a.snap[first + lane];
                visit(cc, on);
            }
        }
        if (!FILL) {
            if (lane == 0) counts[id] = m;
            continue;
        }
        const bool arena = counts != nullptr && all && a.rad_arena != nullptr;
        if (counts && lane == 0) counts[id] = m;
        if (counts && !arena) continue;
        if (m > kRadCap) {
            if (!arena && lane == 0) {
                const int pos = atomicAdd(a.fb2_count, 1);
                a.fb2_list[pos] = slot;
            }
            continue;
        }
        __builtin_amdgcn_wave_barrier();
        int64_t base, cap;
        if (arena) {
            const int64_t share = a.rad_arena_cap / wave_stride;
            if (arena_used + m > share) continue;
            base = (int64_t)wave_global * share + arena_used;
            arena_used += m;
            cap = m;
            idx_out = a.rad_arena;
            if (lane == 0) {
                a.rad_arena_off[id] = base;
                a.rad_done[id] = 2;
            }
        } else {
            base = off_lo;
            cap = off_hi - off_lo;
        }
        if constexpr (sizeof(T) == 4) {
            if (lane == 0) sm->key[m] = ~0ull;
            __builtin_amdgcn_wave_barrier();
#pragma unroll 1
            for (int o0 = 0; o0 < m; o0 += 128) {
                const int e0 = o0 + lane, e1 = o0 + 64 + lane;
                const unsigned long long mine0 = e0 < m ? sm->key[e0] : 0ull, mine1 = e1 < m ? sm->key[e1] : 0ull;
                int rank0 = 0, rank1 = 0;
                for (int j = 0; j < m; j += 2) {
                    const ulonglong2 kk = *reinterpret_cast<const ulonglong2*>(&sm->key[j]);
                    rank0 += (kk.x < mine0 ? 1 : 0) + (kk.y < mine0 ? 1 : 0);
                    rank1 += (kk.x < mine1 ? 1 : 0) + (kk.y < mine1 ? 1 : 0);
                }
                if (e0 < m && rank0 < cap) idx_out[base + rank0] = (int32_t)(uint32_t)mine0;
                if (e1 < m && rank1 < cap) idx_out[base + rank1] = (int32_t)(uint32_t)mine1;
            }
        } else {
            const RadSmem<double>* sd = reinterpret_cast<const RadSmem<double>*>(sm);
            for (int i = lane; i < m; i += 64) {
                const T md = (T)sd->d2[i];
                const int32_t mi = sd->id[i];
                int rank = 0;
                for (int j = 0; j < m; ++j) rank += lex_lt((T)sd->d2[j], sd->id[j], md, mi) ? 1 : 0;
                if (rank < cap) idx_out[base + rank] = mi;
            }
        }
        __builtin_amdgcn_wave_barrier();
    }
}

template <typename T, int MODE> static size_t wave_smem() { return sizeof(WaveSmem<T, MODE == 1>) * kWaves + sizeof(Acc) * kWaves; }

template <typename T>
int launch_wave_radius_count(wtp_ctx* ctx, SearchArgs<T>& a, T r, int32_t* d_counts, const int32_t* list,
                             const int32_t* list_count) {
    int64_t want = ((int64_t)a.n / (list ? 16 : 1) + kWaves - 1) / kWaves;
    int nb = (int)(want > 16384 ? 16384 : (want < 64 ? 64 : want));
    if (a.rad_arena && a.rad_done && !list)
        hipLaunchKernelGGL((wave_radius_kernel<T, true>), dim3(nb), dim3(kThreads), 0, ctx->stream, a, r, d_counts,
                           (const int64_t*)nullptr, (int32_t*)nullptr, list, list_count);
    else
        hipLaunchKernelGGL((wave_radius_kernel<T, false>), dim3(nb), dim3(kThreads), 0, ctx->stream, a, r,
                           d_counts, (const int64_t*)nullptr, (int32_t*)nullptr, list, list_count);
    WTP_HIP(ctx, hipGetLastError());
    return WTP_OK;
}

template <typename T>
int launch_wave_radius_fill(wtp_ctx* ctx, SearchArgs<T>& a, T r, const int64_t* d_offsets, int32_t* d_idx,
                            const int32_t* list, const int32_t* list_count) {
    int64_t want = ((int64_t)a.n / (list ? 16 : 1) + kWaves - 1) / kWaves;
    int nb = (int)(want > 16384 ? 16384 : (want < 64 ? 64 : want));
    hipLaunchKernelGGL((wave_radius_kernel<T, true>), dim3(nb), dim3(kThreads), 0, ctx->stream, a, r,
                       (int32_t*)nullptr, d_offsets, d_idx, list, list_count);
    WTP_HIP(ctx, hipGetLastError());
    return WTP_OK;
}

template <typename T, int MODE> static int launch_wave(wtp_ctx* ctx, SearchArgs<T>& a, bool all, int part_base) {
    (void)launch_occupancy_of(ctx, (const void*)wave_kernel<T, MODE>, kThreads, (wave_smem<T, MODE>()));
    int64_t want = all ? ((int64_t)a.n + kWaves - 1) / kWaves : (int64_t)a.n / 256;
    if (!all && want > 2048) want = 2048;
    if (!all && want < 64) want = 64;
    int nb = (int)(want > kWavePartials ? kWavePartials : (want < 1 ? 1 : want));
    if (MODE == 1) a.used_wave = nb;
    const size_t smem_bytes = wave_smem<T, MODE>();
    hipLaunchKernelGGL((wave_kernel<T, MODE>), dim3(nb), dim3(kThreads), smem_bytes, ctx->stream, a, a.fb_list,
                       a.fb_count, all ? 1 : 0, part_base);
    WTP_HIP(ctx, hipGetLastError());
    return WTP_OK;
}

template <typename T> int launch_wave_topology(wtp_ctx* ctx, SearchArgs<T>& a, bool all) {
    return launch_wave<T, 0>(ctx, a, all, 0);
}

template <typename T> int launch_wave_sweep(wtp_ctx* ctx, SearchArgs<T>& a, bool all) {
    return launch_wave<T, 1>(ctx, a, all, brick_partials());
}

#define INST(T)                                                                                  \
    template int launch_wave_topology<T>(wtp_ctx*, SearchArgs<T>&, bool);                        \
    template int launch_wave_radius_count<T>(wtp_ctx*, SearchArgs<T>&, T, int32_t*, const int32_t*, const int32_t*); \
    template int launch_wave_radius_fill<T>(wtp_ctx*, SearchArgs<T>&, T, const int64_t*, int32_t*, const int32_t*, const int32_t*); \
    template int launch_wave_sweep<T>(wtp_ctx*, SearchArgs<T>&, bool);
INST(float)
INST(double)
#undef INST

}
```

Baseline: 12630.

## Run Cs2 follow-up and reduction on a side stream overlapping the next step

```diff
diff --git a/whatsthepoint.jl_amd/csrc/wtp_api.hip b/whatsthepoint.jl_amd/csrc/wtp_api.hip
--- a/whatsthepoint.jl_amd/csrc/wtp_api.hip
+++ b/whatsthepoint.jl_amd/csrc/wtp_api.hip
@@ -93,9 +93,28 @@
     ctx->ev_last_end = ctx->spans[span].b;
 }
 
+static int tail_streams(wtp_ctx* ctx) {
+    if (!ctx->comm_stream) {
+        int lo = 0, hi = 0;
+        WTP_HIP(ctx, hipDeviceGetStreamPriorityRange(&lo, &hi));
+        WTP_HIP(ctx, hipStreamCreateWithPriority(&ctx->comm_stream, hipStreamNonBlocking, hi));
+    }
+    if (!ctx->ev_tail_pos) WTP_HIP(ctx, hipEventCreateWithFlags(&ctx->ev_tail_pos, hipEventDisableTiming));
+    if (!ctx->ev_tail_nn) WTP_HIP(ctx, hipEventCreateWithFlags(&ctx->ev_tail_nn, hipEventDisableTiming));
+    return WTP_OK;
+}
+
+int tail_join(wtp_ctx* ctx) {
+    if (!ctx->tail_pending) return WTP_OK;
+    ctx->tail_pending = false;
+    WTP_HIP(ctx, hipStreamWaitEvent(ctx->stream, ctx->ev_tail_nn, 0));
+    return WTP_OK;
+}
+
 void spans_collect(wtp_ctx* ctx) {
     ctx->ev_last_end = -1;
     if (ctx->spans.empty()) return;
+    tail_join(ctx);
     hipStreamSynchronize(ctx->stream);
     for (auto& s : ctx->spans) {
         float ms = 0.f;
@@ -112,6 +131,8 @@
 static int sync(wtp_ctx* ctx) {
     ctx->ev_last_end = -1;
     ctx->n_syncs += 1;
+    int rc = tail_join(ctx);
+    if (rc) return rc;
     WTP_HIP(ctx, hipStreamSynchronize(ctx->stream));
     return WTP_OK;
 }
@@ -586,12 +607,15 @@
     if (ctx) block_topo_destroy(ctx);
     if (!ctx) return WTP_OK;
     hipSetDevice(ctx->device);
+    tail_join(ctx);
     hipStreamSynchronize(ctx->stream);
     wtp_comm_finalize(ctx);
     if (ctx->host_pinned) hipHostFree(ctx->host_pinned);
     for (auto e : ctx->ev_pool) hipEventDestroy(e);
     if (ctx->ev_comm_a) hipEventDestroy(ctx->ev_comm_a);
     if (ctx->ev_comm_b) hipEventDestroy(ctx->ev_comm_b);
+    if (ctx->ev_tail_pos) hipEventDestroy(ctx->ev_tail_pos);
+    if (ctx->ev_tail_nn) hipEventDestroy(ctx->ev_tail_nn);
     if (ctx->comm_stream) hipStreamDestroy(ctx->comm_stream);
     hipStreamDestroy(ctx->own_stream);
     delete ctx;
@@ -1238,10 +1262,14 @@
     return r.route == SweepRoute::Cs64 || r.route == SweepRoute::Cs64Wave ? SweepRoute::Exact : SweepRoute::Select;
 }
 
+static bool tail_splits(const wtp_ctx* ctx, const RelaxState& r, SweepRoute route, bool ball) {
+    return route == SweepRoute::Cs2 && !ball && !r.wall_active && !ctx->stop_dev;
+}
+
 static int ball_pass(wtp_ctx* ctx, SearchArgs<float>& a) { return launch_cs_ball(ctx, a, a.ball_list, a.ball_count); }
 static int ball_pass(wtp_ctx* ctx, SearchArgs<double>& a) { return launch_cs_ball64(ctx, a, a.ball_list, a.ball_count); }
 
-template <typename T> static int launch_sweep(wtp_ctx* ctx, SearchArgs<T>& a, SweepRoute route, bool ball) {
+template <typename T> static int launch_sweep(wtp_ctx* ctx, SearchArgs<T>& a, SweepRoute route, bool ball, bool split) {
     constexpr bool f32 = sizeof(T) == 4;
     ctx->n_sweep_launches += 1;
     int rc = WTP_OK, sp = -1;
@@ -1292,7 +1320,7 @@
     if (rc) return rc;
     sp = span_begin(ctx, 2);
     if constexpr (f32) {
-        if (route == SweepRoute::Cs2) rc = launch_cs2_followup(ctx, a);
+        if (route == SweepRoute::Cs2 && !split) rc = launch_cs2_followup(ctx, a);
         if (!rc && ball) rc = ball_pass(ctx, a);
     }
     if (!rc) rc = launch_generic_sweep<T>(ctx, a, false);
@@ -1320,6 +1348,7 @@
     int rc;
     const int t = pick_free(r, r.bufP, -1);
     if ((rc = ensure(ctx, ctx->pts[t], sizeof(Pt<T>) * (size_t)(r.n + r.shard_extra)))) return rc;
+    if (!r.tune.valid && (rc = tail_join(ctx))) return rc;
     int sp = span_begin(ctx, 0);
     r.route = sweep_route<T>(ctx, r);
     if (r.spacing_typ <= 0) {
@@ -1366,7 +1395,10 @@
         const bool reuse = grid_reusable(r, r.n_fixed, r.pending.active);
         r.grid_age = reuse ? r.grid_age + 1 : 0;
         if (!reuse) r.grid_fixed = r.n_fixed;
-        rc = build_hash<T>(ctx, relax_request<T>(ctx, r, in, out, r.n, r.k, r.pending, reuse));
+        HashBuild<T> b = relax_request<T>(ctx, r, in, out, r.n, r.k, r.pending, reuse);
+        b.readers = ctx->tail_pending ? ctx->ev_tail_nn : nullptr;
+        rc = build_hash<T>(ctx, b);
+        ctx->tail_pending = false;
     }
     span_end(ctx, sp);
     if (rc) return rc;
@@ -1379,11 +1411,43 @@
     return WTP_OK;
 }
 
-template <typename T> static int relax_step_t(wtp_ctx* ctx, int rebuild, wtp_step_stats* d_slot) {
+static int launch_neighbour_chain(wtp_ctx* ctx, const SearchArgs<float>& a, wtp_step_stats* d_slot) {
+    if (ctx->timing && ctx->spans.size() > 8000) spans_collect(ctx);
+    WTP_HIP(ctx, hipEventRecord(ctx->ev_tail_pos, ctx->stream));
+    WTP_HIP(ctx, hipStreamWaitEvent(ctx->comm_stream, ctx->ev_tail_pos, 0));
+    SearchArgs<float> b = a;
+    b.fb_list = (int32_t*)ctx->nn_rest.p;
+    b.fb_count = (int32_t*)ctx->fb_count.p + 1;
+    b.fb_total = a.fb_count;
+    b.fb2_count = (int32_t*)ctx->fb_count.p + 5;
+    b.keep_out = 1;
+    hipStream_t main_stream = ctx->stream;
+    const int ev_main = ctx->ev_last_end;
+    ctx->stream = ctx->comm_stream;
+    ctx->ev_last_end = -1;
+    const int sp = span_begin(ctx, 2);
+    int rc = launch_cs2_followup(ctx, b);
+    if (!rc) rc = launch_generic_sweep<float>(ctx, b, false);
+    if (!rc)
+        rc = launch_reduce_partials(ctx, b.partials, b.n_partials, b.used_brick, b.used_wave, b.used_generic, a.fb_count,
+                                    a.uncovered, nullptr, d_slot);
+    span_end(ctx, sp);
+    hipEventRecord(ctx->ev_tail_nn, ctx->comm_stream);
+    ctx->stream = main_stream;
+    ctx->ev_last_end = ev_main;
+    ctx->tail_pending = true;
+    return rc;
+}
+static int launch_neighbour_chain(wtp_ctx* ctx, const SearchArgs<double>&, wtp_step_stats*) {
+    return fail(ctx, WTP_ERR_STATE, "split tail on a Float64 session");
+}
+
+template <typename T> static int relax_step_t(wtp_ctx* ctx, int rebuild, wtp_step_stats* d_slot, bool may_split) {
     RelaxState& r = ctx->relax;
     int rc;
     if (!r.have_tree || r.pending.active) rebuild = 1;
     if (rebuild && (rc = relax_rebuild<T>(ctx))) return rc;
+    if ((rc = tail_join(ctx))) return rc;
     if (spacing_on_device(r.spacing_kind)) {
         int sps = span_begin(ctx, 2);
         rc = launch_spacing_session<T>(ctx, (const Pt<T>*)ctx->pts[r.bufP].p, r.n, r.n_fixed, ctx->kd_nodes.p, ctx->kd_m,
@@ -1421,6 +1485,11 @@
     a.nn_count = (int32_t*)ctx->fb_count.p + 2;
     const SweepRoute route = step_route(r, fresh);
     const bool ball = route_ball(r.route) && (!fresh || r.spacing_kind != WTP_SPACING_CONSTANT);
+    const bool split = may_split && tail_splits(ctx, r, route, ball && route_ball(route));
+    if (split) {
+        if ((rc = tail_streams(ctx))) return rc;
+        if ((rc = ensure(ctx, ctx->nn_rest, sizeof(int32_t) * (size_t)r.n))) return rc;
+    }
     if (ball || route == SweepRoute::Cs2) {
         if ((rc = ensure(ctx, ctx->nn_list, sizeof(int32_t) * (size_t)r.n))) return rc;
         if (sizeof(T) == 4) a.nn_list = (int32_t*)ctx->nn_list.p;
@@ -1453,7 +1522,16 @@
     if (!ctx->counters_clean) WTP_HIP(ctx, hipMemsetAsync(ctx->fb_count.p, 0, 64, ctx->stream));
     ctx->counters_clean = false;
     a.used_brick = a.used_wave = a.used_generic = 0;
-    if ((rc = launch_sweep<T>(ctx, a, route, ball && route_ball(route)))) return rc;
+    if ((rc = launch_sweep<T>(ctx, a, route, ball && route_ball(route), split))) return rc;
+    if (split) {
+        if ((rc = launch_neighbour_chain(ctx, a, d_slot))) return rc;
+        r.bufOld = r.bufP;
+        r.bufP = o;
+        r.can_revert = true;
+        r.have_point_data = true;
+        r.sweeps_since_rebuild += 1;
+        return WTP_OK;
+    }
     int sp = span_begin(ctx, 2);
     if (r.wall_active) {
         char* wf = (char*)ctx->wall_flags.p;
@@ -1474,10 +1552,12 @@
     return WTP_OK;
 }
 
-static int relax_step_any(wtp_ctx* ctx, int rebuild, wtp_step_stats* d_slot) {
-    return by_dtype(ctx->relax.dtype, [&](auto t) { return relax_step_t<decltype(t)>(ctx, rebuild, d_slot); });
-}
-int wtp::relax_step_enqueue(wtp_ctx* ctx, int rebuild, wtp_step_stats* d_slot) { return relax_step_any(ctx, rebuild, d_slot); }
+static int relax_step_any(wtp_ctx* ctx, int rebuild, wtp_step_stats* d_slot, bool may_split) {
+    const int rc = by_dtype(ctx->relax.dtype, [&](auto t) { return relax_step_t<decltype(t)>(ctx, rebuild, d_slot, may_split); });
+    if (rc) tail_join(ctx);
+    return rc;
+}
+int wtp::relax_step_enqueue(wtp_ctx* ctx, int rebuild, wtp_step_stats* d_slot) { return relax_step_any(ctx, rebuild, d_slot, false); }
 
 int wtp::relax_prerank(wtp_ctx* ctx, int64_t n_fixed_new) {
     RelaxState& r = ctx->relax;
@@ -1543,6 +1623,7 @@
     if (!stats) return sync(ctx);
     const size_t off = (sizeof(wtp_step_stats) + 63) / 64 * 64;
     int rc;
+    if ((rc = tail_join(ctx))) return rc;
     if ((rc = ensure_pinned(ctx, n_axes ? off + 64 * n_axes : sizeof(wtp_step_stats)))) return rc;
     char* h = (char*)ctx->host_pinned;
     WTP_HIP(ctx, hipMemcpyAsync(h, ctx->stats.p, sizeof(wtp_step_stats), hipMemcpyDeviceToHost, ctx->stream));
@@ -1561,7 +1642,7 @@
     if (rc) return rc;
     WTP_HIP(ctx, hipSetDevice(ctx->device));
     if ((rc = ensure(ctx, ctx->stats, sizeof(wtp_step_stats)))) return rc;
-    if ((rc = relax_step_any(ctx, rebuild, (wtp_step_stats*)ctx->stats.p))) return rc;
+    if ((rc = relax_step_any(ctx, rebuild, (wtp_step_stats*)ctx->stats.p, true))) return rc;
     return read_step(ctx, stats);
 }
 
@@ -1575,7 +1656,8 @@
     if ((rc = ensure(ctx, ctx->stats, sizeof(wtp_step_stats) * (size_t)n_iters))) return rc;
     wtp_step_stats* d = (wtp_step_stats*)ctx->stats.p;
     for (int i = 0; i < n_iters; ++i)
-        if ((rc = relax_step_any(ctx, (i % rebuild_every) == 0, d + i))) return rc;
+        if ((rc = relax_step_any(ctx, (i % rebuild_every) == 0, d + i, true))) return rc;
+    if ((rc = tail_join(ctx))) return rc;
     if (conv_out || last) {
         if ((rc = ensure_pinned(ctx, sizeof(wtp_step_stats) * (size_t)n_iters))) return rc;
         WTP_HIP(ctx, hipMemcpyAsync(ctx->host_pinned, d, sizeof(wtp_step_stats) * (size_t)n_iters,
@@ -1657,7 +1739,7 @@
         const int i1 = i0 + kBatch < max_iters ? i0 + kBatch : max_iters;
         hist.clear();
         for (int i = i0; i < i1; ++i) {
-            if ((rc = relax_step_any(ctx, (i % rebuild_every) == 0, d + i))) {
+            if ((rc = relax_step_any(ctx, (i % rebuild_every) == 0, d + i, true))) {
                 ctx->stop_dev = nullptr;
                 return rc;
             }
@@ -2062,7 +2144,7 @@
     if (!stats || !counts) return fail(ctx, WTP_ERR_ARG, "stats/counts is NULL");
     WTP_HIP(ctx, hipSetDevice(ctx->device));
     if ((rc = ensure(ctx, ctx->stats, sizeof(wtp_step_stats)))) return rc;
-    if ((rc = relax_step_any(ctx, rebuild, (wtp_step_stats*)ctx->stats.p))) return rc;
+    if ((rc = relax_step_any(ctx, rebuild, (wtp_step_stats*)ctx->stats.p, false))) return rc;
     int32_t* d_tot = nullptr;
     if ((rc = enqueue_layers(ctx, axis, lo_in, hi_in, lo_out, hi_out, d_lo4, d_hi4, cap, &d_tot))) return rc;
     return read_step(ctx, stats, 1, &d_tot, counts);
@@ -2174,7 +2256,7 @@
         return fail(ctx, WTP_ERR_ARG, "NULL argument");
     WTP_HIP(ctx, hipSetDevice(ctx->device));
     if ((rc = ensure(ctx, ctx->stats, sizeof(wtp_step_stats)))) return rc;
-    if ((rc = relax_step_any(ctx, rebuild, (wtp_step_stats*)ctx->stats.p))) return rc;
+    if ((rc = relax_step_any(ctx, rebuild, (wtp_step_stats*)ctx->stats.p, false))) return rc;
     int32_t* d_tot[3] = {nullptr, nullptr, nullptr};
     for (int ax = 0; ax < 3; ++ax)
         if (axes_mask & (1 << ax))
diff --git a/whatsthepoint.jl_amd/csrc/wtp_cs2.hip b/whatsthepoint.jl_amd/csrc/wtp_cs2.hip
--- a/whatsthepoint.jl_amd/csrc/wtp_cs2.hip
+++ b/whatsthepoint.jl_amd/csrc/wtp_cs2.hip
@@ -737,6 +737,7 @@
             } else {
                 const int pos = atomicAdd(a.fb_count, 1);
                 a.fb_list[pos] = gslot;
+                if (a.fb_total) atomicAdd(a.fb_total, 1);
             }
         }
     }
diff --git a/whatsthepoint.jl_amd/csrc/wtp_generic.hip b/whatsthepoint.jl_amd/csrc/wtp_generic.hip
--- a/whatsthepoint.jl_amd/csrc/wtp_generic.hip
+++ b/whatsthepoint.jl_amd/csrc/wtp_generic.hip
@@ -24,7 +24,7 @@
         const Pt<T> q = a.query[slot];
         const int32_t id = w_to_id(q.w);
         if (MODE == 1 && id < a.n_fixed) {
-            a.out[slot] = q;
+            if (!a.keep_out) a.out[slot] = q;
             a.forces[slot] = (T)0;
             a.nn_dist[slot] = Lim<T>::inf();
             a.nn_id[slot] = -1;
@@ -88,7 +88,7 @@
             Pt<T> o;
             const T f = step_point<T>(a, s, q.x, q.y, q.z, Fx, Fy, Fz, o.x, o.y, o.z);
             o.w = q.w;
-            a.out[slot] = o;
+            if (!a.keep_out) a.out[slot] = o;
             a.forces[slot] = f;
             a.nn_dist[slot] = nd;
             a.nn_id[slot] = nid;
@@ -183,11 +183,12 @@
 
 
 template <typename T> int launch_generic_sweep(wtp_ctx* ctx, SearchArgs<T>& a, bool all) {
-    const int part_base = a.n_partials - kGenericPartials;
+    const int part_base = a.n_partials - kGenericPartials + a.used_generic;
     int rc = launch_wave_sweep<T>(ctx, a, all);
     if (rc) return rc;
-    a.used_generic = grid_for(a.n / 16, kThreads, 256);
-    hipLaunchKernelGGL((generic_kernel<T, 1>), dim3(a.used_generic), dim3(kThreads), 0, ctx->stream, a, a.fb2_list,
+    const int nb = grid_for(a.n / 16, kThreads, 256);
+    a.used_generic += nb;
+    hipLaunchKernelGGL((generic_kernel<T, 1>), dim3(nb), dim3(kThreads), 0, ctx->stream, a, a.fb2_list,
                        a.fb2_count, 0, part_base);
     WTP_HIP(ctx, hipGetLastError());
     return WTP_OK;
diff --git a/whatsthepoint.jl_amd/csrc/wtp_hash.hip b/whatsthepoint.jl_amd/csrc/wtp_hash.hip
--- a/whatsthepoint.jl_amd/csrc/wtp_hash.hip
+++ b/whatsthepoint.jl_amd/csrc/wtp_hash.hip
@@ -612,6 +612,7 @@
     }
     ctx->hash_scratch_clean = false;
     ctx->preranked_builds += half_done ? 1 : 0;
+    if (b.readers && !b.keep_grid) WTP_HIP(ctx, hipStreamWaitEvent(st, b.readers, 0));
     if (!b.keep_grid) {
         hipLaunchKernelGGL(bbox_kernel<T>, dim3(nbb), dim3(kThreads), 0, st, in, n_in, part, v_old, v_fixed_old);
         hipLaunchKernelGGL(grid_setup_kernel<T>, dim3(1), dim3(64), 0, st, part, nbb, g, n, b.dim, rho_k, b.radius, b.min_cell,
@@ -627,6 +628,7 @@
                            ctx->stop_dev);
     }
     hipLaunchKernelGGL(scan_reduce_kernel<T>, dim3(nscan), dim3(kThreads), 0, st, cnt, g, bs);
+    if (b.readers && b.keep_grid) WTP_HIP(ctx, hipStreamWaitEvent(st, b.readers, 0));
     hipLaunchKernelGGL(scan_apply_kernel<T>, dim3(nscan), dim3(kThreads), 0, st, cnt, bs, g, start, ctx->stop_dev);
     hipLaunchKernelGGL(scatter_kernel<T>, dim3(nb), dim3(kThreads), 0, st, in, n_in, cr, g, start, out, v_old, v_fixed_old,
                        v_shift, ctx->stop_dev);
diff --git a/whatsthepoint.jl_amd/csrc/wtp_internal.hpp b/whatsthepoint.jl_amd/csrc/wtp_internal.hpp
--- a/whatsthepoint.jl_amd/csrc/wtp_internal.hpp
+++ b/whatsthepoint.jl_amd/csrc/wtp_internal.hpp
@@ -137,6 +137,8 @@
     int32_t fb_r0;
     int32_t ksel_bx;
     unsigned long long* diag;
+    int32_t* fb_total;
+    int32_t keep_out;
 };
 
 struct DevBuf {
@@ -181,6 +183,7 @@
     bool keep_grid = false;
     bool canonical = true;
     const double* box = nullptr;
+    hipEvent_t readers = nullptr;
     HashBuild(const Pt<T>* in_, Pt<T>* out_, int64_t n_, int dim_, int k_) : in(in_), out(out_), n(n_), dim(dim_), k(k_) {}
     int64_t n_in() const { return view.active ? view.n_in : n; }
 };
@@ -291,6 +294,7 @@
     wtp::DevBuf grid_b, cell_start_b, box_b, f64k_s64, f64k_slot, f64k_lists, f64k_cnt;
     wtp::DevBuf forces, nn_dist, nn_id, spacing_pp;
     wtp::DevBuf partials, stats, fb_list, fb_count, fb2_list, fb2_count, nn_list;
+    wtp::DevBuf nn_rest;
     wtp::DevBuf rad_pos;
     wtp::DevBuf rad_bricks;
     bool rad_dense_attr[2] = {false, false};
@@ -302,6 +306,8 @@
     int64_t preranked_builds = 0;
     hipStream_t comm_stream = nullptr;
     hipEvent_t ev_comm_a = nullptr, ev_comm_b = nullptr;
+    hipEvent_t ev_tail_pos = nullptr, ev_tail_nn = nullptr;
+    bool tail_pending = false;
     bool hash_scratch_clean = false;
     bool counters_clean = false;
     wtp::DevBuf stop_state;
@@ -373,6 +379,7 @@
 int span_begin(wtp_ctx* ctx, int kind);
 void span_end(wtp_ctx* ctx, int span);
 void spans_collect(wtp_ctx* ctx);
+int tail_join(wtp_ctx* ctx);
 
 template <typename T> int build_hash(wtp_ctx* ctx, const HashBuild<T>& b);
 template <typename T> int prerank_old_snapshot(wtp_ctx* ctx, const HashBuild<T>& next);
diff --git a/whatsthepoint.jl_amd/csrc/wtp_wave.hip b/whatsthepoint.jl_amd/csrc/wtp_wave.hip
--- a/whatsthepoint.jl_amd/csrc/wtp_wave.hip
+++ b/whatsthepoint.jl_amd/csrc/wtp_wave.hip
@@ -72,7 +72,7 @@
         const int32_t id = w_to_id(q.w);
         if (MODE == 1 && id < a.n_fixed) {
             if (lane == 0) {
-                a.out[slot] = q;
+                if (!a.keep_out) a.out[slot] = q;
                 a.forces[slot] = (T)0;
                 a.nn_dist[slot] = Lim<T>::inf();
                 a.nn_id[slot] = -1;
@@ -308,7 +308,7 @@
                 Pt<T> o;
                 const T f = step_point<T>(a, s, q.x, q.y, q.z, Fx, Fy, Fz, o.x, o.y, o.z);
                 o.w = q.w;
-                a.out[slot] = o;
+                if (!a.keep_out) a.out[slot] = o;
                 a.forces[slot] = f;
                 a.nn_dist[slot] = nd;
                 a.nn_id[slot] = nid;
@@ -539,7 +539,11 @@
     if (!all && want > 2048) want = 2048;
     if (!all && want < 64) want = 64;
     int nb = (int)(want > kWavePartials ? kWavePartials : (want < 1 ? 1 : want));
-    if (MODE == 1) a.used_wave = nb;
+    if (MODE == 1) {
+        part_base += a.used_wave;
+        if (nb > kWavePartials - a.used_wave) nb = kWavePartials - a.used_wave;
+        a.used_wave += nb;
+    }
     const size_t smem_bytes = wave_smem<T, MODE>();
     hipLaunchKernelGGL((wave_kernel<T, MODE>), dim3(nb), dim3(kThreads), smem_bytes, ctx->stream, a, a.fb_list,
                        a.fb_count, all ? 1 : 0, part_base);
```

Result: slower. 11940 (-5.4%).
